# AiRyunn/BoT

Hardware: AMD Instinct MI355X
Metric: edges/sec full-batch GAT fwd+bwd on ogbn-arxiv; achieved HBM GB/s vs peak (higher is better)
Workload: dtype f32

## Files before the change

### bot_amd/_C.py

```python
from __future__ import annotations

import ctypes
import os
from ctypes import c_char_p, c_double, c_float, c_int32, c_int64, c_uint64, c_void_p

import torch

_HERE = os.path.dirname(os.path.abspath(__file__))
LIB_PATH = os.environ.get("BOT_AMD_LIB") or os.path.join(_HERE, "lib", "libbot_gnn.so")
ABI_VERSION = 19

if not os.path.exists(LIB_PATH):
    raise ImportError(
        f"{LIB_PATH} is missing: build the gfx950 kernels first "
        "(`make -C bot_amd/csrc` or `python -c 'import __graft_entry__ as g; g.build()'`). "
        "bot_amd has no CPU / PyTorch fallback."
    )
_lib = ctypes.CDLL(LIB_PATH)

_P = c_void_p
_SIGS = {
    "bot_abi_version": (ctypes.c_int, []),
    "bot_last_error": (c_char_p, []),
    "bot_last_kernel": (c_char_p, []),
    "bot_debug_abort_trace": (ctypes.c_int, [c_char_p]),
    "bot_row_plan_default_chunk": (c_int32, [c_int64]),
    "bot_row_plan_size_host": (ctypes.c_int, [_P, c_int64, c_int32, _P, _P, _P]),
    "bot_row_plan_fill_host": (ctypes.c_int, [_P, c_int64, c_int32, _P, _P, _P]),
    "bot_degrees_i64": (ctypes.c_int, [_P, c_int64, _P, _P]),
    "bot_spmm_workspace_floats": (c_int64, [c_int64, c_int32, c_int32]),
    "bot_spmm_set_layout": (ctypes.c_int, [c_int32]),
    "bot_spmm_set_zero_skip": (ctypes.c_int, [c_int32]),
    "bot_spmm_f32": (ctypes.c_int, [_P, _P, c_int64, c_int64, _P, c_int64, _P, _P, c_int64, _P, c_int64, c_int64, _P, _P,
                                    c_int32, c_int32, _P, c_int64, c_int64, _P, c_int64, c_int64, _P, _P]),
    "bot_spmm_blocked_f32": (ctypes.c_int, [_P, _P, _P, _P, _P, c_int32, c_int32, c_int32, c_int32, c_int32, c_int32, _P, c_int64, _P,
                                            c_int32, c_int32, _P, c_int64, _P, c_int64, _P]),
    "bot_spmm_dot_f32": (ctypes.c_int, [_P, _P, c_int64, c_int64, _P, c_int64, _P, _P, c_int64, _P, c_int64, c_int64, _P, _P,
                                        _P, c_int64, c_int64, c_int32, c_int32, _P, c_int64, c_int64, _P, _P, _P, _P]),
    "bot_spmm_bcast_f32": (ctypes.c_int, [_P, _P, c_int64, c_int64, _P, c_int64, _P, _P, c_int64, _P, c_int64, _P, _P, c_int32,
                                          c_int32, _P, c_int64, c_int64, _P, _P]),
    "bot_spmm_bcast_halves_f16": (ctypes.c_int, [_P, _P, c_int64, c_int64, _P, c_int64, _P, _P, c_int64, _P, c_int64, _P, _P, c_int32, c_int32, _P, _P,
                                                 c_int64, c_int64, c_int32, c_int32, _P, _P]),
    "bot_spmm_dot_bcast_f32": (ctypes.c_int, [_P, _P, c_int64, c_int64, _P, c_int64, _P, _P, c_int64, _P, c_int64, c_int64, _P,
                                              _P, _P, c_int64, c_int32, c_int32, _P, c_int64, _P, _P, _P]),
    "bot_sddmm_dot_f32": (ctypes.c_int, [_P, _P, c_int64, c_int64, _P, c_int64, _P, c_int64, c_int64, _P, c_int64, c_int64,
                                         c_int32, c_int32, _P, _P, c_int32, _P]),
    "bot_sddmm_dot_bcast_f32": (ctypes.c_int, [_P, _P, c_int64, c_int64, _P, c_int64, _P, c_int64, _P, c_int64, c_int64, c_int32,
                                               c_int32, _P, _P, _P]),
    "bot_sddmm_u_add_v_f32": (ctypes.c_int, [_P, _P, c_int64, _P, _P, c_int32, _P, _P]),
    "bot_gat_attn_fwd_f32": (ctypes.c_int, [_P, _P, c_int64, c_int64, _P, c_int64, c_int32, _P, _P, _P, _P, _P, c_float,
                                            c_int32, _P, _P, _P, c_float, c_uint64, _P, _P, _P]),
    "bot_gat_attn_bwd_f32": (ctypes.c_int, [_P, _P, c_int64, c_int64, _P, c_int64, c_int32, _P, _P, _P, _P, c_float, c_int32,
                                            _P, _P, _P, _P, _P, _P, _P, c_float, c_uint64, _P, _P]),
    "bot_gat_infer_workspace_floats": (c_int64, [c_int64, c_int32, c_int32]),
    "bot_gat_infer_f32": (ctypes.c_int, [_P, _P, c_int64, c_int64, _P, c_int64, _P, _P, c_int64, c_int64, _P, c_int64, c_int64,
                                         _P, c_int64, _P, c_int64, _P, _P, c_float, c_int32, c_int32, _P, c_int64, c_int64, _P, _P,
                                         c_int32, _P, c_int64, c_int64, _P, _P, _P]),
    "bot_segment_sum_f32": (ctypes.c_int, [_P, c_int64, c_int64, _P, c_int64, c_int32, _P, _P, c_int32, _P, _P]),
    "bot_gather_rows_f32": (ctypes.c_int, [_P, c_int64, _P, c_int64, c_int32, _P, c_int64, _P]),
    "bot_scatter_add_rows_f32": (ctypes.c_int, [_P, c_int64, _P, c_int64, c_int32, _P, c_int64, _P]),
    "bot_merge_weight_fwd_f32": (ctypes.c_int, [_P, _P, _P, _P, c_int32, c_int32, c_int32, c_int32, c_int32, c_int32, _P, _P]),
    "bot_merge_weight_bwd_f32": (ctypes.c_int, [_P, _P, _P, c_int32, c_int32, c_int32, c_int32, c_int32, c_int32, _P, _P, _P, _P, _P, _P]),
    "bot_edge_mlp_workspace_floats": (c_int64, []),
    "bot_edge_mlp_fwd_f32": (ctypes.c_int, [_P, c_int32, _P, _P, c_int32, _P, c_int32, c_int64, _P, _P]),
    "bot_edge_mlp_bwd_f32": (ctypes.c_int, [_P, c_int32, _P, _P, c_int32, _P, c_int32, _P, c_int64, _P, _P, _P, _P, _P]),
    "bot_random_keep_workspace_bytes": (c_int64, []),
    "bot_random_keep_u8": (ctypes.c_int, [c_int64, c_int64, c_uint64, _P, _P, _P]),
    "bot_halves_workspace_floats": (c_int64, []),
    "bot_halves_scale_f32": (ctypes.c_int, [_P, c_int64, c_int64, c_int32, _P, _P, _P]),
    "bot_halves_split_f16": (ctypes.c_int, [_P, c_int64, c_int64, c_int32, _P, c_int32, _P, c_int64, c_int32, _P]),
    "bot_halves_split_cols_f16": (ctypes.c_int, [_P, c_int64, c_int64, c_int32, _P, c_int32, _P, c_int64, c_int32, c_int32, _P]),
    "bot_halves_split_heads_f16": (ctypes.c_int, [_P, c_int64, c_int64, c_int32, c_int32, _P, _P, c_int64, c_int32, c_int32, _P]),
    "bot_gemm_halves_f32": (ctypes.c_int, [c_int32, c_int32, c_int64, c_int64, c_int64, _P, _P, c_int64, _P, c_int64, _P, c_int64,
                                           c_int32, c_int64, c_int64, c_int64, c_float, _P, c_int64, c_int32, c_int32, _P]),
    "bot_gemm_halves3_nt_f32": (ctypes.c_int, [c_int64, c_int64, c_int64, _P, _P, _P, c_int64, c_int64, _P, c_int64, c_int64, _P, c_int64,
                                               c_int32, _P]),
    "bot_gemm_halves3_tn_workspace_floats": (c_int64, [c_int64, c_int64, c_int64]),
    "bot_gemm_halves3_tn_f32": (ctypes.c_int, [c_int64, c_int64, c_int64, c_int64, c_int64, _P, _P, _P, c_int64, c_int64, _P, c_int64, c_int64, _P,
                                               c_int64, _P, c_int32, _P]),
    "bot_gemm_halves3_nt_grouped_f32": (ctypes.c_int, [c_int64, c_int64, _P, _P, _P, c_int64, c_int64, _P, c_int64, c_int64, _P, c_int64, c_int32, _P,
                                                       c_int32, _P, _P, c_int32, _P, c_int32, _P]),
    "bot_gemm_halves3_tn_grouped_workspace_floats": (c_int64, [c_int64, c_int32]),
    "bot_gemm_halves3_tn_grouped_f32": (ctypes.c_int, [c_int64, _P, _P, _P, c_int64, c_int64, _P, c_int64, c_int64, _P, c_int32, _P, _P, c_int32, _P]),
    "bot_tn_narrow_workspace_floats": (c_int64, [c_int64, c_int32, c_int32]),
    "bot_tn_narrow_f32": (ctypes.c_int, [_P, c_int64, _P, c_int64, c_int64, c_int32, c_int32, _P, c_int64, c_int32, _P, _P]),
    "bot_bn_act_bwd_reduce_max_f32": (ctypes.c_int, [_P, c_int64, _P, c_int64, c_int64, c_int32, _P, _P, _P, _P, c_int32, c_float, c_uint64, _P, _P, _P, _P, _P]),
    "bot_bn_bwd_bound_f32": (ctypes.c_int, [c_int32, c_int64, _P, _P, _P, c_double, _P, _P, _P, _P]),
    "bot_bn_act_bwd_apply_halves_f32": (ctypes.c_int, [_P, c_int64, _P, c_int64, c_int64, c_int32, _P, _P, _P, _P, c_int32, c_float, c_uint64, _P, _P, _P, c_double,
                                                       _P, c_int64, _P, _P, c_int64, c_int32, c_int32, c_int32, _P]),
    "bot_label_split_f32": (ctypes.c_int, [_P, c_int64, _P, c_int64, _P, c_float, c_uint64, _P, c_int32, _P, _P, _P, _P, _P]),
    "bot_build_input_f32": (ctypes.c_int, [_P, c_int64, c_int64, c_int32, c_int32, _P, c_float, c_uint64, _P, _P, c_int64, _P]),
    "bot_build_input_reuse_f32": (ctypes.c_int, [_P, c_int64, c_int64, c_int32, c_int32, _P, _P, _P, c_int64, c_float, c_uint64, _P, _P, c_int64, _P]),
    "bot_node_loss_f32": (ctypes.c_int, [_P, c_int64, c_int64, c_int32, _P, c_int64, _P, _P, c_int32, c_float, _P, c_int64, _P, c_int64, _P]),
    "bot_rmsprop_step_f32": (ctypes.c_int, [c_int32, _P, _P, _P, _P, c_float, _P, c_float, c_float, c_float, _P]),
    "bot_gemm_halves_last_algo": (ctypes.c_int, [_P, _P]),
    "bot_gemm_halves_library_version": (ctypes.c_int, [_P, _P]),
    "bot_tn_gemm_workspace_floats": (c_int64, [c_int64, c_int32, c_int32, c_int32]),
    "bot_tn_gemm_f32": (ctypes.c_int, [_P, c_int64, _P, c_int64, c_int64, c_int32, c_int32, _P, c_int64, c_int32, c_int32, c_int64, c_int64,
                                       c_int64, _P, _P]),
    "bot_skinny_gemm_f32": (ctypes.c_int, [_P, c_int64, _P, c_int64, c_int32, _P, c_int64, c_int64, c_int32, c_int32, c_int32, c_int32,
                                           c_int64, c_int64, c_int64, _P]),
    "bot_bn_workspace_floats": (c_int64, [c_int32]),
    "bot_colstats_f32": (ctypes.c_int, [_P, c_int64, c_int64, c_int32, _P, _P, _P, _P]),
    "bot_colsum_f32": (ctypes.c_int, [_P, c_int64, c_int64, c_int32, _P, _P, _P]),
    "bot_bn_stats_f32": (ctypes.c_int, [_P, c_int64, c_int64, c_int32, c_float, c_float, _P, _P, _P, _P, _P, _P, _P]),
    "bot_bn_stats_halves_f32": (ctypes.c_int, [_P, c_int64, c_int64, c_int32, c_float, c_float, _P, _P, _P, _P, _P, _P, _P, c_float, _P, _P, _P]),
    "bot_bn_act_fwd_halves_f32": (ctypes.c_int, [_P, c_int64, c_int64, c_int32, _P, _P, _P, _P, c_int32, c_float, c_uint64, _P, _P, c_int64,
                                                 _P, _P, c_int64, c_int32, c_int32, _P]),
    "bot_bn_act_fwd_f32": (ctypes.c_int, [_P, c_int64, c_int64, c_int32, _P, _P, _P, _P, c_int32, c_float, c_uint64, _P, _P, c_int64, _P]),
    "bot_bn_act_bwd_reduce_f32": (ctypes.c_int, [_P, c_int64, _P, c_int64, c_int64, c_int32, _P, _P, _P, _P, c_int32, c_float,
                                                 c_uint64, _P, _P, _P, _P, _P]),
    "bot_bn_act_bwd_apply_f32": (ctypes.c_int, [_P, c_int64, _P, c_int64, c_int64, c_int32, _P, _P, _P, _P, c_int32, c_float,
                                                c_uint64, _P, _P, _P, c_double, _P, c_int64, _P, _P]),
    "bot_halves_tn_combine_f32": (ctypes.c_int, [_P, _P, c_int32, c_int32, c_int32, c_int32, _P, _P, _P, c_int64, _P]),
    "bot_halves_scale_from_slots2_f32": (ctypes.c_int, [_P, c_float, _P, c_float, _P, _P]),
    "bot_halves_tail_f16": (ctypes.c_int, [c_int64, c_int32, _P, _P, _P, _P, _P, c_int64, c_int32, _P]),
    "bot_spmm_dot_halves_fits": (ctypes.c_int, [_P, c_int64, c_int64, _P, c_int64, c_int64, c_int32, c_int32, _P, c_int64, c_int64, c_int32]),
    "bot_spmm_dot_halves_f16": (ctypes.c_int, [_P, _P, c_int64, c_int64, _P, c_int64, _P, _P, c_int64, _P, c_int64, c_int64, _P, _P, _P, c_int64, c_int64,
                                               c_int32, c_int32, _P, _P, c_int64, c_int64, c_int32, _P, _P, _P]),
    "bot_gemm_halves3_nt_bn_rows": (c_int32, [c_int64]),
    "bot_gemm_halves3_nt3_f32": (ctypes.c_int, [c_int64, c_int64, c_int64, _P, _P, c_int64, _P, _P, c_int64, c_int64, _P, c_int64, c_int64, c_int32, _P, c_int64,
                                                _P, c_int32, _P]),
    "bot_gemm_halves3_nt_bn_deferred_max_k": (c_int32, []),
    "bot_gemm_halves3_nt_bn_reduce_f32": (ctypes.c_int, [c_int64, c_int64, c_int64, _P, _P, c_int64, _P, _P, c_int64, c_int64, _P, c_int64, c_int64, c_int32, _P, c_int64,
                                                         _P, _P]),
    "bot_gemm_halves3_nt_bn_apply_f32": (ctypes.c_int, [c_int64, c_int64, c_int64, _P, _P, c_int64, _P, _P, c_int64, c_int64, _P, c_int64, c_int64, c_int32, _P,
                                                        _P, _P, c_double, _P, c_int64, _P, _P, c_int64, c_int32, c_int32, c_int32, _P, _P]),
    "bot_bn_act_bwd_reduce_partials_f32": (ctypes.c_int, [_P, c_int32, c_int32, _P, _P, _P]),
    "bot_bn_bwd_bound_partials_f32": (ctypes.c_int, [c_int32, _P, c_int32, _P, _P, c_double, _P, _P, _P, _P]),
    "bot_bn_bwd_partials_finish_f32": (ctypes.c_int, [_P, _P, c_int32, c_int32, _P, _P, c_int32, c_double, _P, _P, _P, _P]),
    "bot_gemm_halves3_nt2_f32": (ctypes.c_int, [c_int64, c_int64, c_int64, _P, _P, c_int64, _P, _P, c_int64, c_int64, _P, c_int64, c_int64, c_int32, _P, c_int64,
                                                c_int32, _P]),
    "bot_halves_split_frag_f16": (ctypes.c_int, [_P, c_int64, c_int64, c_int32, _P, _P, c_int32, _P]),
    "bot_gemm_halves3_tn2_f32": (ctypes.c_int, [c_int64, c_int64, c_int64, c_int64, c_int64, _P, _P, _P, c_int64, _P, c_int64, c_int64, _P, c_int64, c_int64, _P,
                                                c_int64, _P, c_int32, _P]),
    "bot_stream_create": (ctypes.c_int, [c_int32, _P]),
    "bot_gemm_halves3_nt_grouped2_f32": (ctypes.c_int, [c_int64, c_int64, _P, _P, _P, c_int64, c_int64, _P, c_int64, c_int64, _P, c_int64, c_int32, _P,
                                                        c_int32, _P, _P, c_int32, _P, _P, _P, _P, c_int32, c_int32, _P]),
    "bot_bn_stats_halves_partials_f32": (ctypes.c_int, [_P, _P, c_int32, _P, c_int64, c_int32, c_float, c_float, _P, _P, _P, _P, _P, _P, _P, c_float, _P, _P, _P]),
    "bot_absmax_slots": (c_int32, []),
    "bot_absmax_slots_f32": (ctypes.c_int, [_P, c_int64, c_int64, c_int32, _P, _P]),
    "bot_halves_scale_from_slots_f32": (ctypes.c_int, [_P, _P, _P]),
    "bot_sample_neighbors_count_i32": (ctypes.c_int, [_P, c_int64, _P, c_int64, c_int32, _P, _P]),
    "bot_sample_neighbors_i32": (ctypes.c_int, [_P, c_int64, _P, c_int64, c_int32, c_uint64, _P, _P, _P]),
# ... 303 lines not shown

def spmm_dot(d, x, w, wperm, y, out=None, dot=None, absmax=None):
    _dev(x, w, y, d.indptr)
    x, ldx, hsx = _slab(x, "x")
    y, ldy, hsy = _slab(y, "y")
    H, D = x.shape[1], x.shape[2]
    w = _f32(w, "w").contiguous()
    if out is None:
        out = torch.empty((d.n_rows, H, D), dtype=torch.float32, device=x.device)
    out_, ldo, hso = _slab(out, "out")
    assert out_ is out
    if dot is None:
        dot = torch.empty((d.nnz, H), dtype=torch.float32, device=x.device)
    elif dot.dtype != torch.float32 or not dot.is_contiguous() or dot.dim() != 2 or dot.shape[1] != H:
        raise BotKernelError(f"spmm_dot: dot must be a contiguous float32 [E,{H}] array")
    partial = None
    if d.n_long:
        partial = torch.empty(int(_lib.bot_spmm_workspace_floats(d.n_slots, H, D)), dtype=torch.float32, device=x.device)
    _check(_timed("spmm_dot", (H, D), lambda: _lib.bot_spmm_dot_f32(
        d.indptr.data_ptr(), d.indices.data_ptr(), d.n_rows, d.nnz, d.items.data_ptr(), d.n_items, _ptr(d.long_rows),
        _ptr(d.long_ptr), d.n_long, x.data_ptr(), ldx, hsx, w.data_ptr(), _ptr(_i32(wperm, "wperm")), y.data_ptr(), ldy, hsy,
        H, D, out.data_ptr(), ldo, hso, dot.data_ptr(), _ptr(partial), _ptr(absmax), _stream())), "spmm_dot")
    return out, dot


def spmm_dot_halves_fits(x, y, hout, hsh, h2_off) -> bool:
    x, ldx, hsx = _slab(x, "x")
    y, ldy, hsy = _slab(y, "y")
    return bool(_lib.bot_spmm_dot_halves_fits(x.data_ptr(), ldx, hsx, y.data_ptr(), ldy, hsy, x.shape[1], x.shape[2], hout.data_ptr(), hout.stride(0),
                                              int(hsh), int(h2_off)))


def spmm_dot_halves(d, x, w, wperm, y, hscale, hout, hsh, h2_off, dot=None):
    _dev(x, w, y, d.indptr, hout, hscale)
    x, ldx, hsx = _slab(x, "x")
    y, ldy, hsy = _slab(y, "y")
    H, D = x.shape[1], x.shape[2]
    w = _f32(w, "w").contiguous()
    assert hout.dtype == torch.float16 and hout.stride(1) == 1 and hout.shape[0] == d.n_rows
    if dot is None:
        dot = torch.empty((d.nnz, H), dtype=torch.float32, device=x.device)
    elif dot.dtype != torch.float32 or not dot.is_contiguous() or dot.dim() != 2 or dot.shape[1] != H:
        raise BotKernelError(f"spmm_dot_halves: dot must be a contiguous float32 [E,{H}] array")
    partial = None
    if d.n_long:
        partial = torch.empty(int(_lib.bot_spmm_workspace_floats(d.n_slots, H, D)), dtype=torch.float32, device=x.device)
    _check(_timed("spmm_dot", (H, D), lambda: _lib.bot_spmm_dot_halves_f16(
        d.indptr.data_ptr(), d.indices.data_ptr(), d.n_rows, d.nnz, d.items.data_ptr(), d.n_items, _ptr(d.long_rows),
        _ptr(d.long_ptr), d.n_long, x.data_ptr(), ldx, hsx, w.data_ptr(), _ptr(_i32(wperm, "wperm")), y.data_ptr(), ldy, hsy,
        H, D, hscale.data_ptr(), hout.data_ptr(), hout.stride(0), int(hsh), int(h2_off), dot.data_ptr(), _ptr(partial), _stream())), "spmm_dot_halves")
    return dot


def spmm_bcast(d, x, w, wperm=None, head_outer=True):
    _dev(x, w, d.indptr)
    _f32(x, "x")
    if x.stride(1) != 1:
        x = x.contiguous()
    w = _f32(w, "w").contiguous()
    H, D = w.shape[1], x.shape[1]
    if head_outer:
        out = torch.empty((H, d.n_rows, D), dtype=torch.float32, device=x.device)
        ldo, hso = D, d.n_rows * D
    else:
        out = torch.empty((d.n_rows, H, D), dtype=torch.float32, device=x.device)
        ldo, hso = H * D, D
    partial = None
    if d.n_long:
        partial = torch.empty(int(_lib.bot_spmm_workspace_floats(d.n_slots, H, D)), dtype=torch.float32, device=x.device)
    _check(_timed("spmm_bcast", (H, D), lambda: _lib.bot_spmm_bcast_f32(
        d.indptr.data_ptr(), d.indices.data_ptr(), d.n_rows, d.nnz, d.items.data_ptr(), d.n_items, _ptr(d.long_rows),
        _ptr(d.long_ptr), d.n_long, x.data_ptr(), x.stride(0), w.data_ptr(), _ptr(_i32(wperm, "wperm")), H, D, out.data_ptr(),
        ldo, hso, _ptr(partial), _stream())), "spmm_bcast")
    return out


def spmm_bcast_halves(d, x, w, wperm, hscale, hout, col0, hsh, h2_off, hpiece):
    _dev(x, w, d.indptr, hout, hscale)
    _f32(x, "x")
    if x.stride(1) != 1:
        x = x.contiguous()
    w = _f32(w, "w").contiguous()
    H, D = w.shape[1], x.shape[1]
    assert hout.dtype == torch.float16 and hout.dim() == 2 and hout.shape[0] == d.n_rows and hout.stride(1) == 1 and col0 % 4 == 0
    assert col0 + h2_off + (H - 1) * hsh + hpiece <= hout.shape[1]
    partial = None
    if d.n_long:
        partial = torch.empty(int(_lib.bot_spmm_workspace_floats(d.n_slots, H, D)), dtype=torch.float32, device=x.device)
    _check(_timed("spmm_bcast", (H, D), lambda: _lib.bot_spmm_bcast_halves_f16(
        d.indptr.data_ptr(), d.indices.data_ptr(), d.n_rows, d.nnz, d.items.data_ptr(), d.n_items, _ptr(d.long_rows),
        _ptr(d.long_ptr), d.n_long, x.data_ptr(), x.stride(0), w.data_ptr(), _ptr(_i32(wperm, "wperm")), H, D, hscale.data_ptr(),
        hout.data_ptr() + 2 * col0, hout.stride(0), hsh, h2_off, hpiece, _ptr(partial), _stream())), "spmm_bcast_halves")
    return hout


def spmm_dot_bcast(d, x, w, wperm, y, out=None):
    _dev(x, w, y, d.indptr)
    _f32(x, "x"), _f32(y, "y")
    assert x.dim() == 3 and x.is_contiguous()
    if y.stride(1) != 1:
        y = y.contiguous()
    H, n, D = x.shape
    w = _f32(w, "w").contiguous()
    if out is None:
        out = torch.empty((d.n_rows, D), dtype=torch.float32, device=x.device)
    assert out.stride(1) == 1 and out.shape == (d.n_rows, D)
    dot = torch.empty((d.nnz, H), dtype=torch.float32, device=x.device)
    partial = None
    if d.n_long:
        partial = torch.empty(int(_lib.bot_spmm_workspace_floats(d.n_slots, 1, D)), dtype=torch.float32, device=x.device)
    _check(_timed("spmm_dot_bcast", (H, D), lambda: _lib.bot_spmm_dot_bcast_f32(
        d.indptr.data_ptr(), d.indices.data_ptr(), d.n_rows, d.nnz, d.items.data_ptr(), d.n_items, _ptr(d.long_rows),
        _ptr(d.long_ptr), d.n_long, x.data_ptr(), D, n * D, w.data_ptr(), _ptr(_i32(wperm, "wperm")), y.data_ptr(), y.stride(0),
        H, D, out.data_ptr(), out.stride(0), dot.data_ptr(), _ptr(partial), _stream())), "spmm_dot_bcast")
    return out, dot


def sddmm_dot(d, x, y, operm=None, out=None):
    _dev(x, y, d.indptr)
    x, ldx, hsx = _slab(x, "x")
    y, ldy, hsy = _slab(y, "y")
    H, D = x.shape[1], x.shape[2]
    if out is None:
        out = torch.empty((d.nnz, H), dtype=torch.float32, device=x.device)
    _check(_timed("sddmm_dot", (H, D), lambda: _lib.bot_sddmm_dot_f32(
        d.indptr.data_ptr(), d.indices.data_ptr(), d.n_rows, d.nnz, d.items.data_ptr(), d.n_items, x.data_ptr(), ldx, hsx,
        y.data_ptr(), ldy, hsy, H, D, out.data_ptr(), _ptr(_i32(operm, "operm")), 0, _stream())), "sddmm_dot")
    return out


def sddmm_dot_bcast(d, x, y, operm=None):
    _dev(x, y, d.indptr)
    _f32(x, "x"), _f32(y, "y")
    if x.stride(1) != 1:
        x = x.contiguous()
    assert y.dim() == 3 and y.is_contiguous()
    H, n, D = y.shape
    out = torch.empty((d.nnz, H), dtype=torch.float32, device=x.device)
    _check(_timed("sddmm_dot_bcast", (H, D), lambda: _lib.bot_sddmm_dot_bcast_f32(
        d.indptr.data_ptr(), d.indices.data_ptr(), d.n_rows, d.nnz, d.items.data_ptr(), d.n_items, x.data_ptr(), x.stride(0),
        y.data_ptr(), D, n * D, H, D, out.data_ptr(), _ptr(_i32(operm, "operm")), _stream())), "sddmm_dot_bcast")
    return out


def u_add_v(src, dst, x, y=None):
    _dev(x, y, src)
    x = _f32(x, "x").contiguous()
    y = None if y is None else _f32(y, "y").contiguous()
    E, W = src.numel(), x.shape[1]
    out = torch.empty((E, W), dtype=torch.float32, device=x.device)
    _check(_lib.bot_sddmm_u_add_v_f32(_i32(src, "src").data_ptr(), _ptr(_i32(dst, "dst")), E, x.data_ptr(), _ptr(y), W,
                                      out.data_ptr(), _stream()), "u_add_v")
    return out


def zsign_buffer(d, H, slope):
    if os.environ.get("BOT_NO_ZSIGN"):
        return None
    return torch.empty(d.nnz, dtype=torch.uint8, device=d.indptr.device) if (H <= 8 and slope != 1.0 and d.indptr.is_cuda) else None


def gat_attn_fwd(d, el, er, ee, eperm, keep, slope, H, aperm, zsign=None, drop=None):
    _dev(el, er, ee, d.indptr)
    el = None if el is None else _f32(el, "el").contiguous()
    er = None if er is None else _f32(er, "er").contiguous()
    ee = None if ee is None else _f32(ee, "ee").contiguous()
    if keep is not None and (keep.dtype != torch.uint8 or not keep.is_contiguous()):
        raise BotKernelError("keep must be contiguous uint8")
    a = torch.empty((d.nnz, H), dtype=torch.float32, device=d.indptr.device)
    p, seed = drop if drop is not None else (0.0, 0)
    a_drop = torch.empty_like(a) if p > 0 else None
    _check(_lib.bot_gat_attn_fwd_f32(d.indptr.data_ptr(), d.indices.data_ptr(), d.n_rows, d.nnz, _ptr(d.long_rows), d.n_long,
                                     d.chunk, _ptr(el), _ptr(er), _ptr(ee), _ptr(_i32(eperm, "eperm")), _ptr(keep),
                                     float(slope), H, a.data_ptr(), _ptr(_i32(aperm, "aperm")), _ptr(zsign), float(p),
                                     int(seed) & 0xFFFFFFFFFFFFFFFF, _seed_off(p), _ptr(a_drop), _stream()), "gat_attn_fwd")
    return a if drop is None else (a, a_drop if a_drop is not None else a)


def gat_attn_bwd(d, el, er, ee, eperm, slope, H, a, da, aperm, zperm, want_der, zsign=None, drop=None):
    _dev(a, da, d.indptr)
    el = None if el is None else _f32(el, "el").contiguous()
    er = None if er is None else _f32(er, "er").contiguous()
    ee = None if ee is None else _f32(ee, "ee").contiguous()
    a = _f32(a, "a").contiguous()
    da = _f32(da, "da").contiguous()
    dz = torch.empty((d.nnz, H), dtype=torch.float32, device=a.device)
    der = torch.empty((d.n_rows, H), dtype=torch.float32, device=a.device) if want_der else None
    _check(_lib.bot_gat_attn_bwd_f32(d.indptr.data_ptr(), d.indices.data_ptr(), d.n_rows, d.nnz, _ptr(d.long_rows), d.n_long,
                                     d.chunk, _ptr(el), _ptr(er), _ptr(ee), _ptr(_i32(eperm, "eperm")), float(slope), H,
                                     a.data_ptr(), da.data_ptr(), _ptr(_i32(aperm, "aperm")), dz.data_ptr(),
                                     _ptr(_i32(zperm, "zperm")), _ptr(der), _ptr(zsign), float(drop[0]) if drop else 0.0,
                                     (int(drop[1]) & 0xFFFFFFFFFFFFFFFF) if drop else 0, _seed_off(drop[0]) if drop else None,
                                     _stream()), "gat_attn_bwd")
    return dz, der
# ... 466 lines not shown
    n = x.shape[0]
    out = torch.empty((k, p), dtype=torch.float32, device=x.device)
    ws = torch.empty(int(_lib.bot_gemm_halves3_tn_workspace_floats(n, piece_x, piece_d)), dtype=torch.float32, device=x.device)
    _check(_timed("gemm_halves", (k, p, 3 * n, 1), lambda: _lib.bot_gemm_halves3_tn2_f32(
        n, k, p, piece_x, piece_d, scale_x.data_ptr(), scale_d.data_ptr(), _ptr(scale_d2), int(p_split), x.data_ptr(), _ld(x),
        2 * piece_x if x2_off is None else x2_off, d.data_ptr(), _ld(d), 2 * piece_d if d2_off is None else d2_off,
        out.data_ptr(), _ld(out), ws.data_ptr(), int(mode), _stream())), "gemm_halves3_tn")
    return out


def _idx64(t, name):
    if t.dtype != torch.int64 or not t.is_contiguous() or t.dim() != 1:
        raise BotKernelError(f"{name} must be a contiguous 1-D int64 tensor (got {t.dtype}, stride {tuple(t.stride())})")


def _labels64(labels):
    if labels.dtype != torch.int64:
        raise BotKernelError(f"labels must be int64 (got {labels.dtype})")
    lab = labels.reshape(labels.shape[0], -1)
    if lab.shape[1] > 1 and lab.stride(1) != 1:
        lab = lab.contiguous()
    return lab


def label_split(train_idx, labels, mask, mask_rate, seed, use_labels, code, wn):
    _dev(train_idx, labels, wn)
    _idx64(train_idx, "train_idx")
    count = torch.empty(1, dtype=torch.float32, device=wn.device)
    ws = torch.empty(128, dtype=torch.int32, device=wn.device)
    lab = _labels64(labels)
    if wn.dtype != torch.float32 or not wn.is_contiguous() or (code is not None and (code.dtype != torch.int32 or not code.is_contiguous())):
        raise BotKernelError("label_split: wn must be contiguous float32, code contiguous int32")
    m = None
    if mask is not None:
        _dev(mask)
        m = mask.to(torch.bool).contiguous().view(torch.uint8)
        if m.numel() != train_idx.numel():
            raise BotKernelError("label_split: mask must have one entry per training node")
    _check(_lib.bot_label_split_f32(train_idx.data_ptr(), train_idx.numel(), lab.data_ptr(), lab.stride(0), _ptr(m), float(mask_rate), int(seed),
                                    _seed_off(1.0), int(bool(use_labels)), _ptr(code), wn.data_ptr(), count.data_ptr(), ws.data_ptr(), _stream()), "label_split")
    return count


def build_input(feat, code, n_classes, p, seed):
    _dev(feat)
    _f32(feat, "feat")
    n, F = feat.shape
    out = torch.empty((n, F + n_classes), dtype=torch.float32, device=feat.device)
    _check(_lib.bot_build_input_f32(feat.data_ptr(), _ld(feat), n, F, n_classes, _ptr(code), float(p), int(seed), _seed_off(p), out.data_ptr(), _ld(out),
                                    _stream()), "build_input")
    return out


REUSE_CALLS = 0


def build_input_reuse(feat, code, reuse, pred, n_classes, p, seed, out=None):
    global REUSE_CALLS
    _dev(feat, code, reuse, pred, out)
    _f32(feat, "feat"), _f32(pred, "pred"), _f32(out, "out")
    n, F = feat.shape
    if feat.stride(1) != 1 and F > 1:
        feat = feat.contiguous()
    if pred.dim() != 2 or pred.shape[0] != n or pred.shape[1] < n_classes or (pred.stride(1) != 1 and pred.shape[1] > 1):
        raise BotKernelError(f"build_input_reuse: pred must be [{n}, >= {n_classes}] with unit column stride, got {tuple(pred.shape)}")
    if code is None or code.dtype != torch.int32 or not code.is_contiguous() or code.numel() != n:
        raise BotKernelError(f"build_input_reuse: code must be contiguous int32 [{n}]")
    if reuse is not None and (reuse.dtype != torch.uint8 or not reuse.is_contiguous() or reuse.numel() != n):
        raise BotKernelError(f"build_input_reuse: reuse must be contiguous uint8 [{n}]")
    if out is None:
        out = torch.empty((n, F + n_classes), dtype=torch.float32, device=feat.device)
    elif out.shape != (n, F + n_classes) or out.stride(1) != 1:
        raise BotKernelError(f"build_input_reuse: out must be [{n}, {F + n_classes}] with unit column stride")
    _check(_lib.bot_build_input_reuse_f32(feat.data_ptr(), _ld(feat), n, F, n_classes, code.data_ptr(), _ptr(reuse), pred.data_ptr(), _ld(pred), float(p),
                                          int(seed), _seed_off(p), out.data_ptr(), _ld(out), _stream()), "build_input_reuse")
    REUSE_CALLS += 1
    torch.autograd.graph.increment_version(out)
    return out


LOSS_KINDS = {"logit": 0, "loge": 1, "savage": 2}


def node_loss(x, labels, wn, count, kind, eps, want_grad=True):
    _dev(x, labels, wn, count)
    _f32(x, "x")
    n, C = x.shape
    n_pad = (n + 63) // 64 * 64
    y = torch.empty(n_pad, dtype=torch.float32, device=x.device)
    dx = torch.empty((n, C), dtype=torch.float32, device=x.device) if want_grad else None
    lab = _labels64(labels)
    if wn.dtype != torch.float32 or not wn.is_contiguous() or count.dtype != torch.float32:
        raise BotKernelError("node_loss: wn / count must be contiguous float32")
    _check(_lib.bot_node_loss_f32(x.data_ptr(), _ld(x), n, C, lab.data_ptr(), lab.stride(0), wn.data_ptr(), count.data_ptr(), LOSS_KINDS[kind], float(eps),
                                  y.data_ptr(), n_pad, _ptr(dx), C, _stream()), "node_loss")
    return y, dx


def node_loss_weighted(x, labels, wn, lw, wsum, kind, eps, want_grad=True):
    _dev(x, labels, wn, lw, wsum)
    _f32(x, "x")
    n, C = x.shape
    n_pad = (n + 63) // 64 * 64
    y = torch.empty(n_pad, dtype=torch.float32, device=x.device)
    dx = torch.empty((n, C), dtype=torch.float32, device=x.device) if want_grad else None
    lab = _labels64(labels)
# ... 922 lines not shown
```

### bot_amd/csrc/common.h

```cpp
#pragma once
#include <hip/hip_runtime.h>
#include <stdint.h>
#include <stdio.h>

#include "../../include/bot_gnn.h"

namespace bot {

void set_error(const char* fmt, ...);
void set_kernel(const char* fmt, ...);
void launch_halves_scale(const float* part, int n, float* scale, hipStream_t st);

inline int hip_status(const char* what) {
    hipError_t e = hipGetLastError();
    if (e != hipSuccess) {
        set_error("%s: %s", what, hipGetErrorString(e));
        return (int)e;
    }
    return 0;
}

#define BOT_REQUIRE(cond, code, ...)    \
    do {                                \
        if (!(cond)) {                  \
            bot::set_error(__VA_ARGS__); \
            return (code);              \
        }                               \
    } while (0)

inline bool aligned(const void* p, size_t a) { return (reinterpret_cast<uintptr_t>(p) % a) == 0; }

inline unsigned launch_grid(int64_t n, int64_t per_block, int64_t cap = 4096) {
    int64_t b = (n + per_block - 1) / per_block;
    return (unsigned)(b < 1 ? 1 : (b > cap ? cap : b));
}

constexpr int kBlock = 256;
constexpr int kWave = 64;

template <int VEC> struct Vec;
template <> struct Vec<1> { using type = float; };
template <> struct Vec<2> { using type = float2; };
template <> struct Vec<4> { using type = float4; };

template <int VEC>
__device__ __forceinline__ void vload(float (&r)[VEC], const float* p) {
    using T = typename Vec<VEC>::type;
    T v = *reinterpret_cast<const T*>(p);
    if constexpr (VEC == 1) { r[0] = v; }
    if constexpr (VEC == 2) { r[0] = v.x; r[1] = v.y; }
    if constexpr (VEC == 4) { r[0] = v.x; r[1] = v.y; r[2] = v.z; r[3] = v.w; }
}

template <int VEC>
__device__ __forceinline__ void vstore_nt(float* p, const float (&r)[VEC]) {
    typedef float nv __attribute__((ext_vector_type(VEC)));
    nv v;
#pragma unroll
    for (int t = 0; t < VEC; ++t) v[t] = r[t];
    __builtin_nontemporal_store(v, reinterpret_cast<nv*>(p));
}

template <int VEC>
__device__ __forceinline__ void vstore(float* p, const float (&r)[VEC]) {
    using T = typename Vec<VEC>::type;
    T v;
    if constexpr (VEC == 1) { v = r[0]; }
    if constexpr (VEC == 2) { v.x = r[0]; v.y = r[1]; }
    if constexpr (VEC == 4) { v.x = r[0]; v.y = r[1]; v.z = r[2]; v.w = r[3]; }
    *reinterpret_cast<T*>(p) = v;
}

template <int LANES>
__device__ __forceinline__ int group_bcast(int v, int j) {
    if constexpr (LANES == 64) return __builtin_amdgcn_readlane(v, j);
    else return __shfl(v, j, LANES);
}
template <int LANES>
__device__ __forceinline__ float group_bcast(float v, int j) {
    return __int_as_float(group_bcast<LANES>(__float_as_int(v), j));
}

template <int LANES>
// ... 114 lines not shown
```

### bot_amd/csrc/halves.hip

```cpp
#include <hip/hip_fp16.h>

#include "common.h"

namespace bot {

constexpr int kMaxBlocks = 1024;

__global__ __launch_bounds__(kBlock) void absmax_partial_kernel(const float* x, int64_t ldx, int64_t n, int32_t F, float* part) {
    __shared__ float lds[kBlock / kWave];
    float m = 0.f;
    const int64_t total = n * (int64_t)F;
    if (ldx == F && (reinterpret_cast<uintptr_t>(x) & 15) == 0) {
        const int64_t nq = total >> 2;
        const float4* x4 = reinterpret_cast<const float4*>(x);
        const int64_t stride = (int64_t)gridDim.x * kBlock;
        int64_t i = (int64_t)blockIdx.x * kBlock + threadIdx.x;
        for (; i + 3 * stride < nq; i += 4 * stride) {
            const float4 a = x4[i], b = x4[i + stride], c = x4[i + 2 * stride], d = x4[i + 3 * stride];
            m = fmaxf(m, fmaxf(fmaxf(fmaxf(fabsf(a.x), fabsf(a.y)), fmaxf(fabsf(a.z), fabsf(a.w))),
                               fmaxf(fmaxf(fabsf(b.x), fabsf(b.y)), fmaxf(fabsf(b.z), fabsf(b.w)))));
            m = fmaxf(m, fmaxf(fmaxf(fmaxf(fabsf(c.x), fabsf(c.y)), fmaxf(fabsf(c.z), fabsf(c.w))),
                               fmaxf(fmaxf(fabsf(d.x), fabsf(d.y)), fmaxf(fabsf(d.z), fabsf(d.w)))));
        }
        for (; i < nq; i += stride) {
            const float4 a = x4[i];
            m = fmaxf(m, fmaxf(fmaxf(fabsf(a.x), fabsf(a.y)), fmaxf(fabsf(a.z), fabsf(a.w))));
        }
        for (int64_t j = (nq << 2) + (int64_t)blockIdx.x * kBlock + threadIdx.x; j < total; j += stride) m = fmaxf(m, fabsf(x[j]));
    } else if (ldx == F) {
        for (int64_t i = (int64_t)blockIdx.x * kBlock + threadIdx.x; i < total; i += (int64_t)gridDim.x * kBlock) m = fmaxf(m, fabsf(x[i]));
    } else {
        for (int64_t i = (int64_t)blockIdx.x * kBlock + threadIdx.x; i < total; i += (int64_t)gridDim.x * kBlock) {
            const int64_t r = i / F;
            m = fmaxf(m, fabsf(x[r * ldx + (i - r * F)]));
        }
    }
#pragma unroll
    for (int o = 32; o > 0; o >>= 1) m = fmaxf(m, __shfl_xor(m, o));
    if ((threadIdx.x & 63) == 0) lds[threadIdx.x >> 6] = m;
    __syncthreads();
    if (threadIdx.x == 0) {
        for (int w = 1; w < kBlock / kWave; ++w) m = fmaxf(m, lds[w]);
        part[blockIdx.x] = m;
    }
}

__global__ __launch_bounds__(kWave) void halves_scale_kernel(const float* part, int nblk, float* scale) {
    float m = 0.f;
    for (int i = threadIdx.x; i < nblk; i += kWave) m = fmaxf(m, part[i]);
#pragma unroll
    for (int o = 32; o > 0; o >>= 1) m = fmaxf(m, __shfl_xor(m, o));
    if (threadIdx.x == 0) {
        float s = 1.f;
        if (m > 0.f && m < INFINITY) {
            int e;
            const float f = frexpf(m, &e);
            if (f == 0.5f) e -= 1;
            s = ldexpf(1.f, min(60, 14 - e));
        }
        scale[0] = s;
        scale[1] = 1.f / s;
    }
}

template <int ORDER>
__global__ __launch_bounds__(128) void halves_split_kernel(const float* x, int64_t ldx, int32_t F, const float* scale, __half* out,
                                                           int64_t ldo, int32_t piece, bool wide, int32_t width) {
    const int64_t r = blockIdx.x;
    const int c = (blockIdx.y * 128 + threadIdx.x) * 2;
    if (c >= width) return;
    const float s = scale ? scale[0] : 1.f;
    float v0 = 0.f, v1 = 0.f;
    const float* xr = x + r * ldx;
    if (c + 1 < F) {
        if (wide) {
            const float2 v = *reinterpret_cast<const float2*>(xr + c);
            v0 = v.x * s, v1 = v.y * s;
        } else {
            v0 = xr[c] * s, v1 = xr[c + 1] * s;
        }
    } else if (c < F) {
        v0 = xr[c] * s;
    }
// ... 304 lines not shown
```

### bot_amd/csrc/sddmm.hip

```cpp
#include "common.h"

namespace bot {

struct DotArgs {
    const int32_t* indices;
    const int4* items;
    int64_t n_items;
    const float* x;
    int64_t ldx, hsx;
    const float* y;
    int64_t ldy, hsy;
    int32_t H, D;
    float* out;
    const int32_t* operm;
    int32_t accumulate;
};

template <int LANES, int U>
__device__ __forceinline__ float transpose_reduce(float (&p)[U], int lane) {
    static_assert(U == 4 || U == 8, "U");
    if constexpr (U == 8) {
        const bool hi = lane & 4;
        float q[4];
#pragma unroll
        for (int i = 0; i < 4; ++i) {
            const float keep = hi ? p[i + 4] : p[i];
            const float send = hi ? p[i] : p[i + 4];
            q[i] = keep + __shfl_xor(send, 4, LANES);
        }
        const bool h2 = lane & 2;
        float r[2];
#pragma unroll
        for (int i = 0; i < 2; ++i) {
            const float keep = h2 ? q[i + 2] : q[i];
            const float send = h2 ? q[i] : q[i + 2];
            r[i] = keep + __shfl_xor(send, 2, LANES);
        }
        const bool h1 = lane & 1;
        float s = (h1 ? r[1] : r[0]) + __shfl_xor(h1 ? r[0] : r[1], 1, LANES);
#pragma unroll
        for (int m = 8; m < LANES; m <<= 1) s += __shfl_xor(s, m, LANES);
        return s;
    } else {
        const bool h2 = lane & 2;
        float r[2];
#pragma unroll
        for (int i = 0; i < 2; ++i) {
            const float keep = h2 ? p[i + 2] : p[i];
            const float send = h2 ? p[i] : p[i + 2];
            r[i] = keep + __shfl_xor(send, 2, LANES);
        }
        const bool h1 = lane & 1;
        float s = (h1 ? r[1] : r[0]) + __shfl_xor(h1 ? r[0] : r[1], 1, LANES);
#pragma unroll
        for (int m = 4; m < LANES; m <<= 1) s += __shfl_xor(s, m, LANES);
        return s;
    }
}

template <int VEC, int LANES, int NCHUNK>
__global__ __launch_bounds__(kBlock) void sddmm_dot_kernel(DotArgs a) {
    constexpr int U = 8;
    const int lane = threadIdx.x % LANES;
    const int64_t gid = ((int64_t)blockIdx.x * kBlock + threadIdx.x) / LANES;
    if (gid >= a.n_items * a.H) return;
    int head = (int)(gid / a.n_items);
    const int64_t item = gid - (int64_t)head * a.n_items;
    const int4 it = a.items[item];
// ... 24 lines not shown
    for (int k0 = beg; k0 < end; k0 += LANES) {
        const int k = k0 + lane;
        const int idx = k < end ? a.indices[k] : 0;
        const int cnt = min(LANES, end - k0);
        for (int i = 0; i < cnt; i += U) {
            float p[U];
            float v[U][NCHUNK][VEC];
#pragma unroll
            for (int u = 0; u < U; ++u) {
                const int s = group_bcast<LANES>(idx, min(i + u, cnt - 1));
                const float* px = xb + (int64_t)s * a.ldx;
#pragma unroll
                for (int c = 0; c < NCHUNK; ++c) vload<VEC>(v[u][c], px + off[c]);
            }
#pragma unroll
            for (int u = 0; u < U; ++u) {
                float s = 0.f;
#pragma unroll
                for (int c = 0; c < NCHUNK; ++c)
#pragma unroll
                    for (int t = 0; t < VEC; ++t) s = fmaf(v[u][c][t], yv[c][t], s);
                p[u] = s;
            }
            const float tot = transpose_reduce<LANES, U>(p, lane);
            if (lane < U && i + lane < cnt) {
                const int pos = k0 + i + lane;
                const int64_t o = (int64_t)(a.operm ? a.operm[pos] : pos) * a.H + head;
                a.out[o] = a.accumulate ? a.out[o] + tot : tot;
            }
        }
    }
}

template <int VEC, int LANES, int NCHUNK>
static void launch_dot(const DotArgs& a, hipStream_t st) {
    const int64_t groups = a.n_items * a.H;
    const int64_t blocks = (groups * LANES + kBlock - 1) / kBlock;
    if (blocks == 0) return;
    hipLaunchKernelGGL((sddmm_dot_kernel<VEC, LANES, NCHUNK>), dim3((unsigned)blocks), dim3(kBlock), 0, st, a);
}

template <int VEC>
static void dispatch_dot(const DotArgs& a, hipStream_t st) {
    const int L = (a.D + VEC - 1) / VEC;
    if (L <= 8) launch_dot<VEC, 8, 1>(a, st);
    else if (L <= 16) launch_dot<VEC, 16, 1>(a, st);
    else if (L <= 32) launch_dot<VEC, 32, 1>(a, st);
    else if (L <= 64) launch_dot<VEC, 64, 1>(a, st);
    else if (L <= 128) launch_dot<VEC, 64, 2>(a, st);
    else if (L <= 192) launch_dot<VEC, 64, 3>(a, st);
    else launch_dot<VEC, 64, 4>(a, st);
}

template <int VEC, int LANES, int NCHUNK, int HB>
__global__ __launch_bounds__(kBlock) void sddmm_dot_bcast_kernel(DotArgs a) {
    static_assert(LANES >= 16 && HB <= 4, "butterfly layout");
    constexpr int U = 4;
    const int lane = threadIdx.x % LANES;
    const int64_t item = ((int64_t)blockIdx.x * kBlock + threadIdx.x) / LANES;
    if (item >= a.n_items) return;
    const int4 it = a.items[item];
    int row = it.x, beg = it.y, end = it.z;
    if constexpr (LANES == 64) {
        row = __builtin_amdgcn_readfirstlane(row);
        beg = __builtin_amdgcn_readfirstlane(beg);
        end = __builtin_amdgcn_readfirstlane(end);
    }
    int off[NCHUNK];
    float yv[HB][NCHUNK][VEC];
#pragma unroll
    for (int c = 0; c < NCHUNK; ++c) {
        const int e = (c * LANES + lane) * VEC;
        const bool act = e < a.D;
        off[c] = act ? e : 0;
#pragma unroll
        for (int h = 0; h < HB; ++h) {
            vload<VEC>(yv[h][c], a.y + (int64_t)row * a.ldy + (int64_t)h * a.hsy + off[c]);
            if (!act) {
#pragma unroll
                for (int t = 0; t < VEC; ++t) yv[h][c][t] = 0.f;
            }
        }
    }
    for (int k0 = beg; k0 < end; k0 += LANES) {
        const int k = k0 + lane;
        const int idx = k < end ? a.indices[k] : 0;
        const int cnt = min(LANES, end - k0);
        for (int i = 0; i < cnt; i += U) {
            float p[16], v[U][NCHUNK][VEC];
#pragma unroll
            for (int q = 0; q < 16; ++q) p[q] = 0.f;
#pragma unroll
            for (int u = 0; u < U; ++u) {
                const int s = group_bcast<LANES>(idx, min(i + u, cnt - 1));
                const float* px = a.x + (int64_t)s * a.ldx;
#pragma unroll
                for (int c = 0; c < NCHUNK; ++c) vload<VEC>(v[u][c], px + off[c]);
            }
#pragma unroll
            for (int u = 0; u < U; ++u)
#pragma unroll
                for (int h = 0; h < HB; ++h) {
                    float d = 0.f;
#pragma unroll
                    for (int c = 0; c < NCHUNK; ++c)
#pragma unroll
                        for (int t = 0; t < VEC; ++t) d = fmaf(v[u][c][t], yv[h][c][t], d);
                    p[u * 4 + h] = d;
                }
            const float tot = transpose_reduce16<LANES>(p, lane);
            const int slot16 = lane & 15, u = slot16 >> 2, h = slot16 & 3;
            if (lane < 16 && h < HB && i + u < cnt) {
                const int pos = k0 + i + u;
                a.out[(int64_t)(a.operm ? a.operm[pos] : pos) * HB + h] = tot;
            }
        }
    }
}

template <int VEC, int HB>
static void dispatch_dot_bcast(const DotArgs& a, hipStream_t st) {
    const int L = (a.D + VEC - 1) / VEC;
#define BOT_DOTB(LN, NC)                                                                                                    \
    do {                                                                                                                    \
        const int64_t blocks = (a.n_items * LN + kBlock - 1) / kBlock;                                                      \
        if (blocks == 0) break;                                                                                             \
        set_kernel("bot::sddmm_dot_bcast_kernel<%d,%d,%d,%d>", VEC, LN, NC, HB);                                           \
        hipLaunchKernelGGL((sddmm_dot_bcast_kernel<VEC, LN, NC, HB>), dim3((unsigned)blocks), dim3(kBlock), 0, st, a);      \
    } while (0)
    if (L <= 16) BOT_DOTB(16, 1);
    else if (L <= 32) BOT_DOTB(32, 1);
    else if (L <= 64) BOT_DOTB(64, 1);
    else if (L <= 128) BOT_DOTB(64, 2);
    else BOT_DOTB(64, 4);
#undef BOT_DOTB
}

__global__ __launch_bounds__(kBlock) void u_add_v_kernel(const int32_t* src, const int32_t* dst, int64_t n_edges,
                                                        const float* x, const float* y, int32_t W, float* out) {
    const int64_t total = n_edges * W;
    for (int64_t g = (int64_t)blockIdx.x * kBlock + threadIdx.x; g < total; g += (int64_t)gridDim.x * kBlock) {
        const int64_t e = g / W;
        const int j = (int)(g - e * W);
        float v = x[(int64_t)src[e] * W + j];
        if (y) v += y[(int64_t)dst[e] * W + j];
        out[g] = v;
    }
}

}

extern "C" {

int bot_sddmm_dot_f32(const int32_t* indptr, const int32_t* indices, int64_t n_rows, int64_t nnz, const int32_t* items,
                      int64_t n_items, const float* x, int64_t ldx, int64_t hsx, const float* y, int64_t ldy, int64_t hsy,
                      int32_t H, int32_t D, float* out, const int32_t* operm, int32_t accumulate, bot_stream_t stream) {
    using namespace bot;
    (void)indptr;
    BOT_REQUIRE(n_rows >= 0 && nnz >= 0 && n_items >= 0, BOT_E_RANGE, "sddmm_dot: negative size");
    BOT_REQUIRE(nnz < INT32_MAX && n_rows < INT32_MAX, BOT_E_RANGE, "sddmm_dot: int32 index range exceeded");
    BOT_REQUIRE(H >= 1 && D >= 1, BOT_E_RANGE, "sddmm_dot: H=%d D=%d must be >= 1", H, D);
    if (nnz == 0 || n_rows == 0) return 0;
    BOT_REQUIRE(indices && items && x && y && out, BOT_E_NULL, "sddmm_dot: NULL pointer");
    BOT_REQUIRE(hsx >= D && hsy >= D && ldx >= (int64_t)(H - 1) * hsx + D && ldy >= (int64_t)(H - 1) * hsy + D, BOT_E_RANGE,
                "sddmm_dot: strides smaller than the slab");
    hipStream_t st = (hipStream_t)stream;
    const int vec = pick_vec(D, {ldx, hsx, ldy, hsy}, {x, y});
    const int cap = vec * 256;
    for (int d0 = 0; d0 < D; d0 += cap) {
        DotArgs a{indices, reinterpret_cast<const int4*>(items), n_items, x + d0, ldx, hsx, y + d0, ldy, hsy, H,
                  (int32_t)(D - d0 < cap ? D - d0 : cap), out, operm, (d0 > 0 || accumulate) ? 1 : 0};
        if (vec == 4) dispatch_dot<4>(a, st);
        else if (vec == 2) dispatch_dot<2>(a, st);
        else dispatch_dot<1>(a, st);
    }
    return hip_status("sddmm_dot launch");
}

int bot_sddmm_dot_bcast_f32(const int32_t* indptr, const int32_t* indices, int64_t n_rows, int64_t nnz, const int32_t* items,
                            int64_t n_items, const float* x, int64_t ldx, const float* y, int64_t ldy, int64_t hsy, int32_t H,
                            int32_t D, float* out, const int32_t* operm, bot_stream_t stream) {
    using namespace bot;
    (void)indptr;
    BOT_REQUIRE(n_rows >= 0 && nnz >= 0 && n_items >= 0 && nnz < INT32_MAX && n_rows < INT32_MAX, BOT_E_RANGE, "sddmm_dot_bcast: bad size");
    BOT_REQUIRE(H >= 1 && H <= 4 && D >= 1 && D <= 1024, BOT_E_RANGE, "sddmm_dot_bcast: H=%d (1..4) D=%d (1..1024)", H, D);
    if (nnz == 0 || n_rows == 0) return 0;
    BOT_REQUIRE(indices && items && x && y && out, BOT_E_NULL, "sddmm_dot_bcast: NULL pointer");
    BOT_REQUIRE(ldx >= D && ldy >= D && (hsy >= D || H == 1), BOT_E_RANGE, "sddmm_dot_bcast: strides smaller than the slab");
    hipStream_t st = (hipStream_t)stream;
    const int vec = pick_vec(D, {ldx, ldy, H > 1 ? hsy : 0}, {x, y});
    BOT_REQUIRE(D <= vec * 256, BOT_E_RANGE, "sddmm_dot_bcast: D=%d exceeds one launch tile", D);
    DotArgs a{indices, reinterpret_cast<const int4*>(items), n_items, x, ldx, 0, y, ldy, hsy, H, D, out, operm, 0};
#define BOT_DOTB_H(V)                                       \
    switch (H) {                                            \
        case 1: dispatch_dot_bcast<V, 1>(a, st); break;     \
        case 2: dispatch_dot_bcast<V, 2>(a, st); break;     \
        case 3: dispatch_dot_bcast<V, 3>(a, st); break;     \
        default: dispatch_dot_bcast<V, 4>(a, st); break;    \
    }
    if (vec == 4) { BOT_DOTB_H(4) } else if (vec == 2) { BOT_DOTB_H(2) } else { BOT_DOTB_H(1) }
#undef BOT_DOTB_H
    return hip_status("sddmm_dot_bcast launch");
}

int bot_sddmm_u_add_v_f32(const int32_t* src, const int32_t* dst, int64_t n_edges, const float* x, const float* y,
                          int32_t W, float* out, bot_stream_t stream) {
    using namespace bot;
    BOT_REQUIRE(n_edges >= 0 && W >= 1, BOT_E_RANGE, "u_add_v: n_edges=%lld W=%d", (long long)n_edges, W);
    if (n_edges == 0) return 0;
    BOT_REQUIRE(src && x && out && (y == nullptr || dst), BOT_E_NULL, "u_add_v: NULL pointer");
    const int64_t total = n_edges * W;
    int64_t blocks = (total + kBlock - 1) / kBlock;
    if (blocks > 256 * 8) blocks = 256 * 8;
    hipLaunchKernelGGL(u_add_v_kernel, dim3((unsigned)blocks), dim3(kBlock), 0, (hipStream_t)stream, src, dst, n_edges, x, y,
                       W, out);
    return hip_status("u_add_v launch");
}

}
```

### bot_amd/csrc/spmm.hip

```cpp
#include <hip/hip_fp16.h>

#include "sweep.h"

#include <stdlib.h>
#include <algorithm>
#include <atomic>
#include <string.h>

namespace bot {

struct SpmmArgs {
    const int32_t* indices;
    const int4* items;
    int64_t n_items;
    const float* x;
    int64_t ldx, hsx;
    const float* w;
    const int32_t* wperm;
    int32_t H, D, n_tiles;
    float* out;
    int64_t ldo, hso;
    float* partial;
    int64_t ldp;
    const float* y;
    int64_t ldy, hsy;
    float* dot_out;
    const float* addend;
    int64_t lda, hsa;
    uint32_t* absmax;
    __half* hout;
    int64_t ldh, hsh;
    int32_t h2_off, hpiece;
    const float* hscale;
    int32_t skip;
};

__device__ __forceinline__ bool is_zero_weight(float w) { return (__float_as_uint(w) << 1) == 0u; }
__device__ __forceinline__ bool wants_row(float w, uint32_t force) { return ((__float_as_uint(w) << 1) | force) != 0u; }
__device__ __forceinline__ void settle(float& v) { asm volatile("" : "+v"(v)); }
__device__ __forceinline__ void settle(int& v) { asm volatile("" : "+v"(v)); }

template <int VEC>
__device__ __forceinline__ void store_halves(__half* p, int32_t h2_off, const float (&v)[VEC], float s) {
    __half a[VEC], b[VEC];
#pragma unroll
    for (int t = 0; t < VEC; ++t) {
        const float z = v[t] * s;
        a[t] = __float2half_rn(z);
        b[t] = __float2half_rn((z - __half2float(a[t])) * 2048.0f);
    }
    if constexpr (VEC == 4) {
        *reinterpret_cast<uint2*>(p) = *reinterpret_cast<const uint2*>(a);
        *reinterpret_cast<uint2*>(p + h2_off) = *reinterpret_cast<const uint2*>(b);
    } else if constexpr (VEC == 2) {
        *reinterpret_cast<uint32_t*>(p) = *reinterpret_cast<const uint32_t*>(a);
        *reinterpret_cast<uint32_t*>(p + h2_off) = *reinterpret_cast<const uint32_t*>(b);
    } else {
        p[0] = a[0], p[h2_off] = b[0];
    }
}

template <int VEC, int LANES, int NCHUNK>
__global__ __launch_bounds__(kBlock) void spmm_dot_kernel(SpmmArgs a) {
    constexpr int U = 4;
    const int lane = threadIdx.x % LANES;
    const int64_t gid = ((int64_t)blockIdx.x * kBlock + threadIdx.x) / LANES;
    if (gid >= a.n_items * a.H) return;
    int head = (int)(gid / a.n_items);
    const int64_t item = gid - (int64_t)head * a.n_items;
    const int4 it = a.items[item];
    int row = it.x, beg = it.y, end = it.z, slot = it.w;
    if constexpr (LANES == 64) {
        row = __builtin_amdgcn_readfirstlane(row);
        beg = __builtin_amdgcn_readfirstlane(beg);
        end = __builtin_amdgcn_readfirstlane(end);
        slot = __builtin_amdgcn_readfirstlane(slot);
        head = __builtin_amdgcn_readfirstlane(head);
    }
    const float* xb = a.x + (int64_t)head * a.hsx;
    const float* yb = a.y + (int64_t)row * a.ldy + (int64_t)head * a.hsy;
    int off[NCHUNK];
    bool act[NCHUNK];
    float acc[NCHUNK][VEC], yv[NCHUNK][VEC];
#pragma unroll
    for (int c = 0; c < NCHUNK; ++c) {
        const int e = (c * LANES + lane) * VEC;
        act[c] = e < a.D;
        off[c] = act[c] ? e : 0;
        vload<VEC>(yv[c], yb + off[c]);
// ... 543 lines not shown
#pragma unroll
        for (int h = 0; h < HB; ++h) wv[h] = 0.f;
        if (k < end) {
            idx = a.indices[k];
            const int wp = a.wperm ? a.wperm[k] : k;
#pragma unroll
            for (int h = 0; h < HB; ++h) wv[h] = a.w[(int64_t)wp * HB + h];
        }
        const int cnt = min(LANES, end - k0);
        for (int i = 0; i < cnt; i += U) {
            float v[U][NCHUNK][VEC], ww[U][HB];
#pragma unroll
            for (int u = 0; u < U; ++u) {
                const int j = min(i + u, cnt - 1);
                const int s = group_bcast<LANES>(idx, j);
#pragma unroll
                for (int h = 0; h < HB; ++h) ww[u][h] = i + u < cnt ? group_bcast<LANES>(wv[h], j) : 0.f;
                const float* px = a.x + (int64_t)s * a.ldx;
#pragma unroll
                for (int c = 0; c < NCHUNK; ++c) vload<VEC>(v[u][c], px + off[c]);
            }
#pragma unroll
            for (int u = 0; u < U; ++u)
#pragma unroll
                for (int h = 0; h < HB; ++h)
#pragma unroll
                    for (int c = 0; c < NCHUNK; ++c)
#pragma unroll
                        for (int t = 0; t < VEC; ++t) acc[h][c][t] = fmaf(ww[u][h], v[u][c][t], acc[h][c][t]);
        }
    }
    if (a.hout && slot < 0) {
        const float s = a.hscale[0];
#pragma unroll
        for (int h = 0; h < HB; ++h) {
            __half* ob = a.hout + (int64_t)row * a.ldh + (int64_t)h * a.hsh;
#pragma unroll
            for (int c = 0; c < NCHUNK; ++c) {
                const int e = (c * LANES + lane) * VEC;
                if (e < a.hpiece) store_halves<VEC>(ob + e, a.h2_off, acc[h][c], act[c] ? s : 0.f);
            }
        }
        return;
    }
#pragma unroll
    for (int h = 0; h < HB; ++h) {
        float* ob = slot < 0 ? a.out + (int64_t)row * a.ldo + (int64_t)h * a.hso : a.partial + (int64_t)slot * a.ldp + (int64_t)h * a.D;
#pragma unroll
        for (int c = 0; c < NCHUNK; ++c)
            if (act[c]) vstore<VEC>(ob + off[c], acc[h][c]);
    }
}

__global__ __launch_bounds__(kBlock) void spmm_combine_halves_kernel(const int32_t* long_rows, const int32_t* long_ptr, int64_t n_long, int32_t H,
                                                                    int32_t D, const float* partial, int64_t ldp, __half* hout, int64_t ldh,
                                                                    int64_t hsh, int32_t h2_off, int32_t hpiece, const float* hscale) {
    const int64_t gid = (int64_t)blockIdx.x * kBlock + threadIdx.x;
    const int64_t hp = (int64_t)H * hpiece;
    if (gid >= n_long * hp) return;
    const int64_t i = gid / hp;
    const int e2 = (int)(gid - i * hp);
    const int h = e2 / hpiece, d = e2 - h * hpiece;
    float v[1] = {0.f};
    if (d < D) {
        const int e = h * D + d;
        for (int p = long_ptr[i]; p < long_ptr[i + 1]; ++p) v[0] += partial[(int64_t)p * ldp + e];
    }
    store_halves<1>(hout + (int64_t)long_rows[i] * ldh + (int64_t)h * hsh + d, h2_off, v, hscale[0]);
}

template <int VEC, int LANES, int NCHUNK, int HB>
__global__ __launch_bounds__(kBlock) void spmm_dot_bcast_kernel(SpmmArgs a) {
    static_assert(LANES >= 16 && HB <= 4, "butterfly layout");
    constexpr int U = 4;
    const int lane = threadIdx.x % LANES;
    const int64_t item = ((int64_t)blockIdx.x * kBlock + threadIdx.x) / LANES;
    if (item >= a.n_items) return;
    const int4 it = a.items[item];
    int row = it.x, beg = it.y, end = it.z, slot = it.w;
    if constexpr (LANES == 64) {
        row = __builtin_amdgcn_readfirstlane(row);
        beg = __builtin_amdgcn_readfirstlane(beg);
        end = __builtin_amdgcn_readfirstlane(end);
        slot = __builtin_amdgcn_readfirstlane(slot);
    }
    const float* yb = a.y + (int64_t)row * a.ldy;
    int off[NCHUNK];
    bool act[NCHUNK];
    float acc[NCHUNK][VEC], yv[NCHUNK][VEC];
#pragma unroll
    for (int c = 0; c < NCHUNK; ++c) {
        const int e = (c * LANES + lane) * VEC;
        act[c] = e < a.D;
        off[c] = act[c] ? e : 0;
        vload<VEC>(yv[c], yb + off[c]);
#pragma unroll
        for (int t = 0; t < VEC; ++t) {
            acc[c][t] = 0.f;
            if (!act[c]) yv[c][t] = 0.f;
        }
    }
    for (int k0 = beg; k0 < end; k0 += LANES) {
        const int k = k0 + lane;
        int idx = 0, wp = 0;
        float wv[HB];
#pragma unroll
        for (int h = 0; h < HB; ++h) wv[h] = 0.f;
        if (k < end) {
            idx = a.indices[k];
            wp = a.wperm ? a.wperm[k] : k;
#pragma unroll
            for (int h = 0; h < HB; ++h) wv[h] = a.w[(int64_t)wp * HB + h];
        }
        const int cnt = min(LANES, end - k0);
        for (int i = 0; i < cnt; i += U) {
            float p[16];
#pragma unroll
            for (int q = 0; q < 16; ++q) p[q] = 0.f;
#pragma unroll
            for (int u = 0; u < U; ++u) {
                const int j = min(i + u, cnt - 1);
                const int s = group_bcast<LANES>(idx, j);
                const float* px = a.x + (int64_t)s * a.ldx;
                float v[HB][NCHUNK][VEC];
#pragma unroll
                for (int h = 0; h < HB; ++h)
#pragma unroll
                    for (int c = 0; c < NCHUNK; ++c) vload<VEC>(v[h][c], px + (int64_t)h * a.hsx + off[c]);
#pragma unroll
                for (int h = 0; h < HB; ++h) {
                    const float ww = i + u < cnt ? group_bcast<LANES>(wv[h], j) : 0.f;
                    float d = 0.f;
#pragma unroll
                    for (int c = 0; c < NCHUNK; ++c)
#pragma unroll
                        for (int t = 0; t < VEC; ++t) {
                            acc[c][t] = fmaf(ww, v[h][c][t], acc[c][t]);
                            d = fmaf(v[h][c][t], yv[c][t], d);
                        }
                    p[u * 4 + h] = d;
                }
            }
            const float tot = transpose_reduce16<LANES>(p, lane);
            const int slot16 = lane & 15, u = slot16 >> 2, h = slot16 & 3;
            const int mywp = __shfl(wp, min(i + u, LANES - 1), LANES);
            if (lane < 16 && h < HB && i + u < cnt) a.dot_out[(int64_t)mywp * HB + h] = tot;
        }
    }
    float* ob = slot < 0 ? a.out + (int64_t)row * a.ldo : a.partial + (int64_t)slot * a.ldp;
#pragma unroll
    for (int c = 0; c < NCHUNK; ++c)
        if (act[c]) vstore<VEC>(ob + off[c], acc[c]);
}

template <int VEC, int HB, bool DOT>
static void dispatch_bcast(SpmmArgs& a, hipStream_t st) {
    const int L = (std::max(a.D, a.hout ? a.hpiece : 0) + VEC - 1) / VEC;
#define BOT_BCAST(LN, NC)                                                                                                     \
    do {                                                                                                                      \
        const int64_t blocks = (a.n_items * LN + kBlock - 1) / kBlock;                                                        \
        if (blocks == 0) break;                                                                                               \
        set_kernel(DOT ? "bot::spmm_dot_bcast_kernel<%d,%d,%d,%d>" : "bot::spmm_bcast_kernel<%d,%d,%d,%d>", VEC, LN, NC, HB);        \
        if constexpr (DOT) hipLaunchKernelGGL((spmm_dot_bcast_kernel<VEC, LN, NC, HB>), dim3((unsigned)blocks), dim3(kBlock), 0, st, a); \
        else hipLaunchKernelGGL((spmm_bcast_kernel<VEC, LN, NC, HB>), dim3((unsigned)blocks), dim3(kBlock), 0, st, a);        \
    } while (0)
    if (L <= 16) BOT_BCAST(16, 1);
    else if (L <= 32) BOT_BCAST(32, 1);
    else if (L <= 64) BOT_BCAST(64, 1);
    else if (L <= 128) BOT_BCAST(64, 2);
    else BOT_BCAST(64, 4);
#undef BOT_BCAST
}

template <bool DOT>
static int run_bcast(SpmmArgs& a, int vec, int H, hipStream_t st) {
#define BOT_BCAST_H(V)                                \
    switch (H) {                                      \
        case 1: dispatch_bcast<V, 1, DOT>(a, st); break; \
        case 2: dispatch_bcast<V, 2, DOT>(a, st); break; \
        case 3: dispatch_bcast<V, 3, DOT>(a, st); break; \
        default: dispatch_bcast<V, 4, DOT>(a, st); break; \
    }
    if (vec == 4) { BOT_BCAST_H(4) } else if (vec == 2) { BOT_BCAST_H(2) } else { BOT_BCAST_H(1) }
#undef BOT_BCAST_H
    return hip_status(DOT ? "spmm_dot_bcast launch" : "spmm_bcast launch");
}

template <int VEC, int LANES, int NCHUNK>
static void launch_spmm(const SpmmArgs& a, hipStream_t st) {
    const int64_t groups = a.n_items * a.H * a.n_tiles;
    const int64_t blocks = (groups * LANES + kBlock - 1) / kBlock;
    if (blocks == 0) return;
    set_kernel("bot::spmm_kernel<%d,%d,%d,%s>", VEC, LANES, NCHUNK, a.w ? "true" : "false");
    if (a.w) hipLaunchKernelGGL((spmm_kernel<VEC, LANES, NCHUNK, true>), dim3((unsigned)blocks), dim3(kBlock), 0, st, a);
    else hipLaunchKernelGGL((spmm_kernel<VEC, LANES, NCHUNK, false>), dim3((unsigned)blocks), dim3(kBlock), 0, st, a);
}

template <int VEC, int LANES, int NCHUNK>
static void launch_spmm_dot(const SpmmArgs& a, hipStream_t st) {
    const int64_t groups = a.n_items * a.H;
    const int64_t blocks = (groups * LANES + kBlock - 1) / kBlock;
    if (blocks == 0) return;
    set_kernel("bot::spmm_dot_kernel<%d,%d,%d>", VEC, LANES, NCHUNK);
    hipLaunchKernelGGL((spmm_dot_kernel<VEC, LANES, NCHUNK>), dim3((unsigned)blocks), dim3(kBlock), 0, st, a);
}

template <int VEC>
static void dispatch_spmm_dot(SpmmArgs& a, hipStream_t st) {
    const int L = (a.D + VEC - 1) / VEC;
    if (L <= 8) launch_spmm_dot<VEC, 8, 1>(a, st);
    else if (L <= 16) launch_spmm_dot<VEC, 16, 1>(a, st);
    else if (L <= 32) launch_spmm_dot<VEC, 32, 1>(a, st);
    else if (L <= 64) launch_spmm_dot<VEC, 64, 1>(a, st);
    else if (L <= 128) launch_spmm_dot<VEC, 64, 2>(a, st);
    else if (L <= 192) launch_spmm_dot<VEC, 64, 3>(a, st);
    else launch_spmm_dot<VEC, 64, 4>(a, st);
}

static bool spmm_dot_rows_wanted() {
    static const bool wanted = [] {
        const char* e = getenv("BOT_SPMM_DOT_LAYOUT");
        return !(e && !strcmp(e, "heads"));
    }();
    return wanted;
}

static bool spmm_rows_wanted() {
    static const bool wanted = [] {
        const char* e = getenv("BOT_SPMM_LAYOUT");
        return !(e && !strcmp(e, "heads"));
    }();
    return wanted;
}

// ... 173 lines not shown
    if (n_long > 0) {
        const int64_t n = n_long * H * D;
        hipLaunchKernelGGL(spmm_combine_kernel, dim3((unsigned)((n + kBlock - 1) / kBlock)), dim3(kBlock), 0, st, long_rows,
                           long_ptr, n_long, H, D, partial, (int64_t)H * D, out, ldo, hso, addend, lda, hsa);
        if (int rc = hip_status("spmm combine launch")) return rc;
    }
    return 0;
}

int bot_spmm_dot_f32(const int32_t* indptr, const int32_t* indices, int64_t n_rows, int64_t nnz, const int32_t* items,
                     int64_t n_items, const int32_t* long_rows, const int32_t* long_ptr, int64_t n_long, const float* x,
                     int64_t ldx, int64_t hsx, const float* w, const int32_t* wperm, const float* y, int64_t ldy, int64_t hsy,
                     int32_t H, int32_t D, float* out, int64_t ldo, int64_t hso, float* dot_out, float* partial,
                     uint32_t* absmax_slots, bot_stream_t stream) {
    using namespace bot;
    (void)indptr;
    BOT_REQUIRE(n_rows >= 0 && nnz >= 0 && n_items >= 0 && n_long >= 0, BOT_E_RANGE, "spmm_dot: negative size");
    BOT_REQUIRE(nnz < INT32_MAX && n_rows < INT32_MAX, BOT_E_RANGE, "spmm_dot: int32 index range exceeded");
    BOT_REQUIRE(H >= 1 && D >= 1, BOT_E_RANGE, "spmm_dot: H=%d D=%d must be >= 1", H, D);
    if (n_rows == 0) return 0;
    BOT_REQUIRE(items && x && out && y && (nnz == 0 || (indices && w && dot_out)), BOT_E_NULL, "spmm_dot: NULL pointer");
    BOT_REQUIRE(n_long == 0 || (long_rows && long_ptr && partial), BOT_E_NULL, "spmm_dot: long rows need long_rows/long_ptr/partial");
    BOT_REQUIRE(hsx >= D && hso >= D && hsy >= D && ldx >= (int64_t)(H - 1) * hsx + D && ldo >= (int64_t)(H - 1) * hso + D &&
                    ldy >= (int64_t)(H - 1) * hsy + D, BOT_E_RANGE, "spmm_dot: strides smaller than the slab");
    hipStream_t st = (hipStream_t)stream;
    SpmmArgs a{indices, reinterpret_cast<const int4*>(items), n_items, x, ldx, hsx, w, wperm, H, D, 1, out, ldo, hso, partial,
               (int64_t)H * D, y, ldy, hsy, dot_out, nullptr, 0, 0};
    const int vec = pick_vec(D, {ldx, hsx, ldo, hso, ldy, hsy}, {x, out, partial, y});
    BOT_REQUIRE(D <= vec * 256, BOT_E_RANGE, "spmm_dot: D=%d exceeds the %d floats one launch tile covers (use bot_spmm_f32 + bot_sddmm_dot_f32)",
                D, vec * 256);
    a.absmax = absmax_slots;
    a.skip = g_zero_skip.load(std::memory_order_relaxed);
    const bool rows = vec == 4 ? dispatch_spmm_dot_rows<4>(a, st) : (vec == 2 ? dispatch_spmm_dot_rows<2>(a, st) : dispatch_spmm_dot_rows<1>(a, st));
    if (!rows) {
        if (vec == 4) dispatch_spmm_dot<4>(a, st);
        else if (vec == 2) dispatch_spmm_dot<2>(a, st);
        else dispatch_spmm_dot<1>(a, st);
    }
    if (int rc = hip_status("spmm_dot launch")) return rc;
    if (n_long > 0) {
        const int64_t n = n_long * H * D;
        hipLaunchKernelGGL(spmm_combine_kernel, dim3((unsigned)((n + kBlock - 1) / kBlock)), dim3(kBlock), 0, st, long_rows,
                           long_ptr, n_long, H, D, partial, (int64_t)H * D, out, ldo, hso, (const float*)nullptr, (int64_t)0, (int64_t)0,
                           rows ? absmax_slots : (uint32_t*)nullptr);
        if (int rc = hip_status("spmm_dot combine launch")) return rc;
    }
    if (absmax_slots && !rows) {
        for (int h = 0; h < H; ++h) launch_absmax_slots(out + (int64_t)h * hso, ldo, n_rows, D, absmax_slots, st);
        if (int rc = hip_status("spmm_dot absmax launch")) return rc;
    }
    return 0;
}

int bot_spmm_bcast_f32(const int32_t* indptr, const int32_t* indices, int64_t n_rows, int64_t nnz, const int32_t* items,
                       int64_t n_items, const int32_t* long_rows, const int32_t* long_ptr, int64_t n_long, const float* x,
                       int64_t ldx, const float* w, const int32_t* wperm, int32_t H, int32_t D, float* out, int64_t ldo,
                       int64_t hso, float* partial, bot_stream_t stream) {
    using namespace bot;
    (void)indptr;
    BOT_REQUIRE(n_rows >= 0 && nnz >= 0 && n_items >= 0 && n_long >= 0 && nnz < INT32_MAX, BOT_E_RANGE, "spmm_bcast: bad size");
    BOT_REQUIRE(H >= 1 && H <= 4 && D >= 1 && D <= 1024, BOT_E_RANGE, "spmm_bcast: H=%d (1..4) D=%d (1..1024)", H, D);
    if (n_rows == 0) return 0;
    BOT_REQUIRE(items && x && out && (nnz == 0 || (indices && w)), BOT_E_NULL, "spmm_bcast: NULL pointer");
    BOT_REQUIRE(n_long == 0 || (long_rows && long_ptr && partial), BOT_E_NULL, "spmm_bcast: long rows need long_rows/long_ptr/partial");
    BOT_REQUIRE(ldx >= D && (hso >= D || H == 1) && ldo >= D, BOT_E_RANGE, "spmm_bcast: strides smaller than the slab");
    hipStream_t st = (hipStream_t)stream;
    SpmmArgs a{indices, reinterpret_cast<const int4*>(items), n_items, x, ldx, 0, w, wperm, H, D, 1, out, ldo, hso, partial,
               (int64_t)H * D, nullptr, 0, 0, nullptr, nullptr, 0, 0};
    const int vec = pick_vec(D, {ldx, ldo, hso}, {x, out, partial});
    BOT_REQUIRE(D <= vec * 256, BOT_E_RANGE, "spmm_bcast: D=%d exceeds one launch tile", D);
    if (int rc = run_bcast<false>(a, vec, H, st)) return rc;
    if (n_long > 0) {
        const int64_t n = n_long * H * D;
        hipLaunchKernelGGL(spmm_combine_kernel, dim3((unsigned)((n + kBlock - 1) / kBlock)), dim3(kBlock), 0, st, long_rows,
                           long_ptr, n_long, H, D, partial, (int64_t)H * D, out, ldo, hso, (const float*)nullptr, (int64_t)0, (int64_t)0);
        if (int rc = hip_status("spmm_bcast combine launch")) return rc;
    }
    return 0;
}

int bot_spmm_bcast_halves_f16(const int32_t* indptr, const int32_t* indices, int64_t n_rows, int64_t nnz, const int32_t* items, int64_t n_items,
                              const int32_t* long_rows, const int32_t* long_ptr, int64_t n_long, const float* x, int64_t ldx, const float* w,
                              const int32_t* wperm, int32_t H, int32_t D, const float* hscale, uint16_t* hout, int64_t ldh, int64_t hsh, int32_t h2_off,
                              int32_t hpiece, float* partial, bot_stream_t stream) {
    using namespace bot;
    (void)indptr;
    BOT_REQUIRE(n_rows >= 0 && nnz >= 0 && n_items >= 0 && n_long >= 0 && nnz < INT32_MAX, BOT_E_RANGE, "spmm_bcast_halves: bad size");
    BOT_REQUIRE(H >= 1 && H <= 4 && D >= 1 && D <= 1024, BOT_E_RANGE, "spmm_bcast_halves: H=%d (1..4) D=%d (1..1024)", H, D);
    if (n_rows == 0) return 0;
    BOT_REQUIRE(items && x && hout && hscale && (nnz == 0 || (indices && w)), BOT_E_NULL, "spmm_bcast_halves: NULL pointer");
    BOT_REQUIRE(n_long == 0 || (long_rows && long_ptr && partial), BOT_E_NULL, "spmm_bcast_halves: long rows need long_rows/long_ptr/partial");
    BOT_REQUIRE(ldx >= D && hpiece >= D && hpiece % 4 == 0 && (hsh >= hpiece || H == 1) && h2_off % 4 == 0 && hsh % 4 == 0 && ldh % 4 == 0 &&
                    h2_off >= (int64_t)(H - 1) * hsh + hpiece && ldh >= h2_off + (int64_t)(H - 1) * hsh + hpiece && aligned(hout, 8),
                BOT_E_RANGE, "spmm_bcast_halves: D=%d hpiece=%d hsh=%lld h2_off=%d ldh=%lld", D, hpiece, (long long)hsh, h2_off, (long long)ldh);
    hipStream_t st = (hipStream_t)stream;
    SpmmArgs a{indices, reinterpret_cast<const int4*>(items), n_items, x, ldx, 0, w, wperm, H, D, 1, nullptr, 0, 0, partial,
               (int64_t)H * D, nullptr, 0, 0, nullptr, nullptr, 0, 0};
    a.hout = reinterpret_cast<__half*>(hout), a.ldh = ldh, a.hsh = hsh, a.h2_off = h2_off, a.hpiece = hpiece, a.hscale = hscale;
    const int vec = pick_vec(D, {ldx}, {x, partial});
    BOT_REQUIRE(hpiece <= vec * 256, BOT_E_RANGE, "spmm_bcast_halves: hpiece=%d exceeds one launch tile", hpiece);
    a.D = D;
    if (int rc = run_bcast<false>(a, vec, H, st)) return rc;
    if (n_long > 0) {
        const int64_t n = n_long * H * hpiece;
        hipLaunchKernelGGL(spmm_combine_halves_kernel, dim3((unsigned)((n + kBlock - 1) / kBlock)), dim3(kBlock), 0, st, long_rows, long_ptr, n_long, H, D,
                           (const float*)partial, (int64_t)H * D, a.hout, ldh, hsh, h2_off, hpiece, hscale);
        if (int rc = hip_status("spmm_bcast_halves combine launch")) return rc;
    }
    return 0;
}

int bot_spmm_dot_halves_fits(const float* x, int64_t ldx, int64_t hsx, const float* y, int64_t ldy, int64_t hsy, int32_t H, int32_t D, const uint16_t* hout,
                             int64_t ldh, int64_t hsh, int32_t h2_off) {
    using namespace bot;
    if (H < 2 || D < 1 || !spmm_dot_rows_wanted()) return 0;
    const int vec = pick_vec(D, {ldx, hsx, ldy, hsy}, {x, y});
    if (!(hsh >= D && h2_off >= (int64_t)(H - 1) * hsh + D && ldh >= h2_off + (int64_t)(H - 1) * hsh + D && hsh % vec == 0 && h2_off % vec == 0 && ldh % vec == 0 &&
          aligned(hout, 2 * vec) && D <= vec * 256))
        return 0;
    const int L = (D + vec - 1) / vec;
    if (L <= 8) return 0;
    if (L > 64) return (L <= 128 && vec != 4 && H <= 3) ? 1 : 0;
    const int HL = L <= 16 ? 16 : (L <= 32 ? 32 : 64);
    return (H * HL + 63) / 64 <= 4 ? 1 : 0;
}

int bot_spmm_dot_halves_f16(const int32_t* indptr, const int32_t* indices, int64_t n_rows, int64_t nnz, const int32_t* items,
                            int64_t n_items, const int32_t* long_rows, const int32_t* long_ptr, int64_t n_long, const float* x,
                            int64_t ldx, int64_t hsx, const float* w, const int32_t* wperm, const float* y, int64_t ldy, int64_t hsy,
                            int32_t H, int32_t D, const float* hscale, uint16_t* hout, int64_t ldh, int64_t hsh, int32_t h2_off, float* dot_out,
                            float* partial, bot_stream_t stream) {
    using namespace bot;
    (void)indptr;
    BOT_REQUIRE(n_rows >= 0 && nnz >= 0 && n_items >= 0 && n_long >= 0 && nnz < INT32_MAX && n_rows < INT32_MAX, BOT_E_RANGE, "spmm_dot_halves: bad size");
    BOT_REQUIRE(H >= 2 && D >= 1, BOT_E_RANGE, "spmm_dot_halves: H=%d D=%d (the all-heads layout needs H >= 2)", H, D);
    if (n_rows == 0) return 0;
    BOT_REQUIRE(items && x && hout && hscale && y && (nnz == 0 || (indices && w && dot_out)), BOT_E_NULL, "spmm_dot_halves: NULL pointer");
    BOT_REQUIRE(n_long == 0 || (long_rows && long_ptr && partial), BOT_E_NULL, "spmm_dot_halves: long rows need long_rows/long_ptr/partial");
    BOT_REQUIRE(hsx >= D && hsy >= D && ldx >= (int64_t)(H - 1) * hsx + D && ldy >= (int64_t)(H - 1) * hsy + D, BOT_E_RANGE,
                "spmm_dot_halves: strides smaller than the slab");
    hipStream_t st = (hipStream_t)stream;
    SpmmArgs a{indices, reinterpret_cast<const int4*>(items), n_items, x, ldx, hsx, w, wperm, H, D, 1, nullptr, 0, 0, partial,
               (int64_t)H * D, y, ldy, hsy, dot_out, nullptr, 0, 0};
    const int vec = pick_vec(D, {ldx, hsx, ldy, hsy}, {x, partial, y});
    BOT_REQUIRE(hsh >= D && h2_off >= (int64_t)(H - 1) * hsh + D && ldh >= h2_off + (int64_t)(H - 1) * hsh + D && hsh % vec == 0 && h2_off % vec == 0 &&
                    ldh % vec == 0 && aligned(hout, 2 * vec), BOT_E_RANGE, "spmm_dot_halves: D=%d hsh=%lld h2_off=%d ldh=%lld vec=%d", D, (long long)hsh, h2_off,
                (long long)ldh, vec);
    BOT_REQUIRE(D <= vec * 256, BOT_E_RANGE, "spmm_dot_halves: D=%d exceeds one launch tile", D);
    a.hout = reinterpret_cast<__half*>(hout), a.ldh = ldh, a.hsh = hsh, a.h2_off = h2_off, a.hpiece = D, a.hscale = hscale;
    a.skip = g_zero_skip.load(std::memory_order_relaxed);
    const bool rows = vec == 4 ? dispatch_spmm_dot_rows<4>(a, st) : (vec == 2 ? dispatch_spmm_dot_rows<2>(a, st) : dispatch_spmm_dot_rows<1>(a, st));
    BOT_REQUIRE(rows, BOT_E_RANGE, "spmm_dot_halves: H=%d D=%d does not fit the all-heads layout", H, D);
    if (int rc = hip_status("spmm_dot_halves launch")) return rc;
    if (n_long > 0) {
        const int64_t n = n_long * H * D;
        hipLaunchKernelGGL(spmm_combine_halves_kernel, dim3((unsigned)((n + kBlock - 1) / kBlock)), dim3(kBlock), 0, st, long_rows, long_ptr, n_long, H, D,
                           (const float*)partial, (int64_t)H * D, a.hout, ldh, hsh, h2_off, D, hscale);
        if (int rc = hip_status("spmm_dot_halves combine launch")) return rc;
    }
    return 0;
}

// ... 30 lines not shown
```

### bot_amd/csrc/step.hip

```cpp
#include <algorithm>

#include "common.h"

namespace bot {
namespace {

__device__ __forceinline__ uint64_t eff_seed(uint64_t seed, const uint64_t* off) {
    return off ? seed + off[0] * 0x9E3779B97F4A7C15ull : seed;
}

__device__ __forceinline__ float uniform01(uint32_t w) { return (w >> 8) * (1.0f / 16777216.0f); }

constexpr int kSplitBlocks = 128;
__global__ __launch_bounds__(256) void label_split_kernel(const int64_t* train_idx, int64_t n_train, const int64_t* labels, int64_t ldl, const uint8_t* mask,
                                                          float mask_rate, uint64_t seed, const uint64_t* seed_offset, int use_labels, int32_t* code,
                                                          float* wn, int32_t* partial) {
    __shared__ int part[4];
    const uint64_t s = eff_seed(seed, seed_offset);
    int mine = 0;
    for (int64_t i = (int64_t)blockIdx.x * 256 + threadIdx.x; i < n_train; i += (int64_t)gridDim.x * 256) {
        bool keep;
        if (mask) {
            keep = mask[i] != 0;
        } else {
            uint32_t w[4];
            Philox::gen(s, (uint64_t)(i >> 2), w);
            keep = uniform01(w[i & 3]) < mask_rate;
        }
        const int64_t n = train_idx[i];
        const bool pred = use_labels ? !keep : keep;
        if (code) code[n] = (use_labels && keep) ? (int32_t)labels[n * ldl] : -1;
        wn[n] = pred ? 1.f : 0.f;
        mine += pred ? 1 : 0;
    }
#pragma unroll
    for (int o = 32; o > 0; o >>= 1) mine += __shfl_xor(mine, o);
    if ((threadIdx.x & 63) == 0) part[threadIdx.x >> 6] = mine;
    __syncthreads();
    if (threadIdx.x == 0) partial[blockIdx.x] = part[0] + part[1] + part[2] + part[3];
}

__global__ __launch_bounds__(64) void label_count_kernel(const int32_t* partial, int nb, float* count) {
    int t = 0;
    for (int i = threadIdx.x; i < nb; i += 64) t += partial[i];
#pragma unroll
    for (int o = 32; o > 0; o >>= 1) t += __shfl_xor(t, o);
    if (threadIdx.x == 0) count[0] = (float)t;
}

__global__ __launch_bounds__(256) void build_input_kernel(const float* feat, int64_t ldf, int64_t n, int F, int C, const int32_t* code, float p,
                                                          uint64_t seed, const uint64_t* seed_offset, float* out, int64_t ldo) {
    const int W = F + C, nquad = (W + 3) >> 2;
    const uint64_t s = eff_seed(seed, seed_offset);
    const float scale = p > 0.f ? 1.f / (1.f - p) : 1.f;
    const int64_t total = n * (int64_t)nquad;
    for (int64_t q = (int64_t)blockIdx.x * 256 + threadIdx.x; q < total; q += (int64_t)gridDim.x * 256) {
        const int64_t r = q / nquad;
        const int c0 = (int)(q - r * nquad) * 4;
        const int lab = code ? code[r] : -1;
        uint32_t w[4] = {0u, 0u, 0u, 0u};
        if (p > 0.f) Philox::gen(s, (uint64_t)q, w);
        float v[4];
#pragma unroll
        for (int t = 0; t < 4; ++t) {
            const int c = c0 + t;
            float x = 0.f;
            if (c < F) x = feat[r * ldf + c];
            else if (c < W) x = (c - F == lab) ? 1.f : 0.f;
            v[t] = (p > 0.f && uniform01(w[t]) < p) ? 0.f : x * scale;
        }
        float* o = out + r * ldo + c0;
        if (c0 + 3 < W && (ldo & 3) == 0 && (reinterpret_cast<uintptr_t>(out) & 15) == 0) {
            *reinterpret_cast<float4*>(o) = make_float4(v[0], v[1], v[2], v[3]);
        } else {
#pragma unroll
            for (int t = 0; t < 4; ++t)
                if (c0 + t < W) o[t] = v[t];
        }
    }
}

constexpr int kReuseMaxPerLane = 8;
__global__ __launch_bounds__(256) void build_input_reuse_kernel(const float* feat, int64_t ldf, int64_t n, int F, int C, const int32_t* code,
                                                                const uint8_t* reuse, const float* pred, int64_t ldp, float p, uint64_t seed,
                                                                const uint64_t* seed_offset, float* out, int64_t ldo) {
    __shared__ float prob[16][16 * kReuseMaxPerLane + 16];
    const int W = F + C, nquad = (W + 3) >> 2;
    const uint64_t s = eff_seed(seed, seed_offset);
    const float scale = p > 0.f ? 1.f / (1.f - p) : 1.f;
    const int l16 = threadIdx.x & 15, g = threadIdx.x >> 4;
    const bool vec_out = (ldo & 3) == 0 && (reinterpret_cast<uintptr_t>(out) & 15) == 0;
    const bool vec_in = (ldf & 3) == 0 && (reinterpret_cast<uintptr_t>(feat) & 15) == 0;
    for (int64_t base = (int64_t)blockIdx.x * 16; base < n; base += (int64_t)gridDim.x * 16) {
        const int64_t r = base + g;
        const bool live = r < n;
        const int lab = live ? code[r] : 0;
        const bool soft = live && lab < 0 && (!reuse || reuse[r] != 0);
        const float* xr = pred + (soft ? r : 0) * ldp;
        float v[kReuseMaxPerLane];
        float m = -INFINITY;
#pragma unroll
        for (int k = 0; k < kReuseMaxPerLane; ++k) {
            const int c = l16 + 16 * k;
            v[k] = (soft && c < C) ? xr[c] : -INFINITY;
            m = fmaxf(m, v[k]);
        }
#pragma unroll
        for (int o = 8; o > 0; o >>= 1) m = fmaxf(m, __shfl_xor(m, o, 16));
        float se = 0.f;
#pragma unroll
        for (int k = 0; k < kReuseMaxPerLane; ++k) {
            v[k] = (soft && l16 + 16 * k < C) ? expf(v[k] - m) : 0.f;
            se += v[k];
        }
#pragma unroll
        for (int o = 8; o > 0; o >>= 1) se += __shfl_xor(se, o, 16);
        if (soft) {
            const float inv = 1.f / se;
#pragma unroll
            for (int k = 0; k < kReuseMaxPerLane; ++k) {
                const int c = l16 + 16 * k;
                if (c < C) prob[g][c] = v[k] * inv;
            }
        }
        __syncthreads();
        if (live) {
            const float* fr = feat + r * ldf;
            float* orow = out + r * ldo;
            for (int quad = l16; quad < nquad; quad += 16) {
                const int c0 = quad * 4;
                uint32_t w[4] = {0u, 0u, 0u, 0u};
                if (p > 0.f) Philox::gen(s, (uint64_t)(r * nquad + quad), w);
// ... 102 lines not shown
    int n_tensors;
    float lr, alpha, eps, weight_decay;
    const float* lr_dev;
};

__global__ __launch_bounds__(256) void rmsprop_kernel(RmsArgs a) {
    int t = 0;
    while (t + 1 < a.n_tensors && (int)blockIdx.x >= a.first_block[t + 1]) ++t;
    const int64_t i0 = ((int64_t)(blockIdx.x - a.first_block[t]) * 256 + threadIdx.x) * 4;
    const float lr = a.lr_dev ? a.lr_dev[0] : a.lr;
    float* p = a.p[t];
    const float* g = a.g[t];
    float* sq = a.sq[t];
#pragma unroll
    for (int e = 0; e < 4; ++e) {
        const int64_t i = i0 + e;
        if (i < a.numel[t]) {
            float gi = g[i];
            if (a.weight_decay != 0.f) gi = fmaf(a.weight_decay, p[i], gi);
            const float s = a.alpha * sq[i] + (1.f - a.alpha) * gi * gi;
            sq[i] = s;
            p[i] = p[i] - lr * (gi / (sqrtf(s) + a.eps));
        }
    }
}

}
}

extern "C" int bot_label_split_f32(const int64_t* train_idx, int64_t n_train, const int64_t* labels, int64_t ldl, const uint8_t* mask, float mask_rate,
                                   uint64_t seed, const uint64_t* seed_offset, int32_t use_labels, int32_t* code, float* wn, float* count,
                                   int32_t* workspace, bot_stream_t stream) {
    using namespace bot;
    BOT_REQUIRE(n_train >= 0 && train_idx && wn && count && workspace && (!use_labels || (code && labels)), -1, "label_split: null pointer");
    const int nb = (int)std::max<int64_t>(1, std::min<int64_t>(kSplitBlocks, (n_train + 255) / 256));
    hipLaunchKernelGGL(label_split_kernel, dim3(nb), dim3(256), 0, (hipStream_t)stream, train_idx, n_train, labels, ldl, mask, mask_rate, seed, seed_offset,
                       (int)use_labels, code, wn, workspace);
    hipLaunchKernelGGL(label_count_kernel, dim3(1), dim3(64), 0, (hipStream_t)stream, workspace, nb, count);
    return hip_status("label_split");
}

extern "C" int bot_build_input_f32(const float* feat, int64_t ldf, int64_t n, int32_t F, int32_t C, const int32_t* code, float p, uint64_t seed,
                                   const uint64_t* seed_offset, float* out, int64_t ldo, bot_stream_t stream) {
    using namespace bot;
    BOT_REQUIRE(n >= 0 && F >= 0 && C >= 0 && F + C > 0 && feat && out && ldo >= F + C && ldf >= F && p >= 0.f && p < 1.f && (C == 0 || code), -1,
                "build_input: bad arguments");
    if (n == 0) return 0;
    const int64_t total = n * (int64_t)((F + C + 3) / 4);
    hipLaunchKernelGGL(build_input_kernel, dim3((unsigned)std::min<int64_t>((total + 255) / 256, 65536)), dim3(256), 0, (hipStream_t)stream, feat, ldf, n, (int)F,
                       (int)C, code, p, seed, seed_offset, out, ldo);
    return hip_status("build_input");
}

extern "C" int bot_build_input_reuse_f32(const float* feat, int64_t ldf, int64_t n, int32_t F, int32_t C, const int32_t* code, const uint8_t* reuse,
                                         const float* pred, int64_t ldp, float p, uint64_t seed, const uint64_t* seed_offset, float* out, int64_t ldo,
                                         bot_stream_t stream) {
    using namespace bot;
    BOT_REQUIRE(C >= 1 && C <= 16 * kReuseMaxPerLane, BOT_E_RANGE, "build_input_reuse: C=%d (1 <= C <= %d)", (int)C, 16 * kReuseMaxPerLane);
    BOT_REQUIRE(n >= 0 && F >= 0 && ldo >= F + C && ldf >= F && ldp >= C && p >= 0.f && p < 1.f, BOT_E_RANGE,
                "build_input_reuse: n=%lld F=%d ldf=%lld ldp=%lld ldo=%lld p=%f", (long long)n, (int)F, (long long)ldf, (long long)ldp, (long long)ldo, (double)p);
    BOT_REQUIRE(out && code && pred && (F == 0 || feat), BOT_E_NULL, "build_input_reuse: NULL pointer (feat, code, pred, out)");
    if (n == 0) return 0;
    hipLaunchKernelGGL(build_input_reuse_kernel, dim3((unsigned)std::min<int64_t>((n + 15) / 16, 65536)), dim3(256), 0, (hipStream_t)stream, feat, ldf, n, (int)F,
                       (int)C, code, reuse, pred, ldp, p, seed, seed_offset, out, ldo);
    return hip_status("build_input_reuse");
}

extern "C" int bot_node_loss_f32(const float* x, int64_t ldx, int64_t n, int32_t C, const int64_t* labels, int64_t ldl, const float* wn, const float* count,
                                 int32_t kind, float eps, float* y, int64_t n_pad, float* dx, int64_t lddx, bot_stream_t stream) {
    using namespace bot;
    BOT_REQUIRE(n >= 0 && C > 0 && C <= 16 * kLossMaxPerLane && x && labels && wn && count && y && n_pad >= n && kind >= 0 && kind <= 2 && (!dx || lddx >= C),
                -1, "node_loss: bad arguments (1 <= C <= %d)", 16 * kLossMaxPerLane);
    if (n_pad == 0) return 0;
    hipLaunchKernelGGL(node_loss_kernel<false>, dim3((unsigned)((n_pad * 16 + 255) / 256)), dim3(256), 0, (hipStream_t)stream, x, ldx, n, (int)C, labels, ldl,
                       wn, nullptr, count, (int)kind, eps, y, dx, lddx, n_pad);
    return hip_status("node_loss");
}

extern "C" int bot_node_loss_weighted_f32(const float* x, int64_t ldx, int64_t n, int32_t C, const int64_t* labels, int64_t ldl, const float* wn,
                                          const float* lw, const float* wsum, int32_t kind, float eps, float* y, int64_t n_pad, float* dx, int64_t lddx,
                                          bot_stream_t stream) {
    using namespace bot;
    BOT_REQUIRE(n >= 0 && C > 0 && C <= 16 * kLossMaxPerLane && n_pad >= n && kind >= 0 && kind <= 2 && (!dx || lddx >= C) && ldx >= C, BOT_E_RANGE,
                "node_loss_weighted: n=%lld n_pad=%lld C=%d kind=%d ldx=%lld lddx=%lld (1 <= C <= %d)", (long long)n, (long long)n_pad, (int)C, (int)kind,
                (long long)ldx, (long long)lddx, 16 * kLossMaxPerLane);
    BOT_REQUIRE(x && labels && wn && lw && wsum && y, BOT_E_NULL, "node_loss_weighted: NULL pointer (x, labels, wn, lw, wsum, y)");
    if (n_pad == 0) return 0;
    hipLaunchKernelGGL(node_loss_kernel<true>, dim3((unsigned)((n_pad * 16 + 255) / 256)), dim3(256), 0, (hipStream_t)stream, x, ldx, n, (int)C, labels, ldl,
                       wn, lw, wsum, (int)kind, eps, y, dx, lddx, n_pad);
    return hip_status("node_loss_weighted");
}

extern "C" int bot_rmsprop_step_f32(int32_t n_tensors, float* const* params, const float* const* grads, float* const* square_avg, const int64_t* numel,
                                    float lr, const float* lr_dev, float alpha, float eps, float weight_decay, bot_stream_t stream) {
    using namespace bot;
    BOT_REQUIRE(n_tensors >= 0 && n_tensors <= kMaxTensors, -1, "rmsprop_step: at most %d tensors per call (got %d)", kMaxTensors, n_tensors);
    if (n_tensors == 0) return 0;
    RmsArgs a;
    int blocks = 0;
    for (int t = 0; t < n_tensors; ++t) {
        BOT_REQUIRE(params[t] && grads[t] && square_avg[t] && numel[t] >= 0, -1, "rmsprop_step: null pointer in tensor %d", t);
        a.p[t] = params[t], a.g[t] = grads[t], a.sq[t] = square_avg[t], a.numel[t] = numel[t];
        a.first_block[t] = blocks;
        blocks += (int)((numel[t] + 1023) / 1024);
    }
    a.first_block[n_tensors] = blocks;
// ... 6 lines not shown
```

### bot_amd/nn/fused.py

```python
from __future__ import annotations

import os
from types import SimpleNamespace

import torch
import torch.nn as nn
import torch.nn.functional as F

from .. import _C, gemm, halo, side
from ..graph import take_rows
from ..ops import bn_epilogue_forward, bn_epilogue_sums, new_dropout_seed, stats_partials_for


ABSMAX_BYPRODUCT = os.environ.get("BOT_ABSMAX_BYPRODUCT", "1") != "0"
SKIP_Y = os.environ.get("BOT_SKIP_Y", "1") != "0"
HANDLES = 0
SKINNY = os.environ.get("BOT_SKINNY", "1") != "0"
FORCE = False
CALLS = 0
AGG_CALLS = 0
L0_CALLS = 0


def can_fuse(conv, norm, activation, graph, training, stack_residual) -> bool:
# ... 477 lines not shown


def _small_mm(a, b, b_is_kn, out):
    if a.is_cuda and SKINNY:
        return _C.skinny_gemm(a, b, b_is_kn=b_is_kn, out=out)
    out.copy_(a @ (b if b_is_kn else b.t()))
    return out


def use_agg_first(conv) -> bool:
    return AGG_FIRST and conv._in_src_feats <= conv._out_feats and conv._num_heads <= 4 and conv._in_src_feats <= 256


class _GATHiddenAggFirst(torch.autograd.Function):

    @staticmethod
    def forward(ctx, h, W, Wr, bn_w, bn_b, graph, bn, H, D, has_res, has_er, slope, attn_p, drop_p, bn_training, kp, sym, y_needed=True):
        N, Fin, HD = h.shape[0], h.shape[1], H * D
        Nd = graph.number_of_dst_nodes()
        csc = graph.csc
        ctx.cfg, ctx.graph = (H, D, has_res, has_er, slope), graph
        ctx.sym = sym
        ctx.kp = kp
        skinny = SKINNY and h.is_cuda and Fin <= 256 and N >= 4096
        l0h = _l0_halves_ok(h, H, D, Fin, has_res, sym, attn_p, graph) and not ctx.needs_input_grad[0]
        ctx.l0h = l0h
        if l0h:
            P2 = Wr.shape[1 if kp else 0]
            out2 = torch.empty((N, P2), dtype=h.dtype, device=h.device)
            _small_mm(h, Wr[:, HD:] if kp else Wr[HD:], kp, out2[:, HD:])
        elif skinny:
            out2 = _C.skinny_gemm(h, Wr, b_is_kn=kp, out=torch.empty((N, Wr.shape[1 if kp else 0]), dtype=h.dtype, device=h.device))
        else:
            out2 = torch.mm(h, Wr) if kp else torch.mm(h, Wr.t())
        ctx.skinny = skinny
        c = HD if has_res else 0
        ext = None
        if graph.halo is not None:
            import torch.distributed as dist
            plan = graph.halo
            Wd = _ext_width(Fin, H)
            ext = torch.empty((N + plan.n_halo, Wd), dtype=h.dtype, device=h.device)
            ext[:N, :Fin] = h
            ext[:N, Fin:Fin + H] = out2[:, c:c + H]
            if Wd > Fin + H:
                ext[:N, Fin + H:].zero_()
            send = _C.gather_rows(ext[:N], plan.send_rows) if plan.n_send else ext.new_empty((0, Wd))
            halo.a2a(ext[N:], send, plan.recv_splits, plan.send_splits, plan.group)
            xsrc = ext[:, :Fin]
            el = ext[:, Fin:Fin + H].contiguous()
        else:
            xsrc = h
            el = out2[:, c:c + H].contiguous()
        er = out2[:Nd, c + H:c + 2 * H].contiguous() if has_er else None
        if sym:
            s_out, w_e = sym_scales(graph)
            el = el * s_out.unsqueeze(1)
        ctx.zs = _C.zsign_buffer(csc, H, slope)
        ctx.adrop = (attn_p, new_dropout_seed(attn_p)) if attn_p > 0 else None
        a, a_d = _C.gat_attn_fwd(csc, el, er, None, None, None, slope, H, None, ctx.zs, drop=ctx.adrop or (0.0, 0))
        if sym:
            a_d = a_d * w_e
        if l0h:
            global L0_CALLS
            L0_CALLS += 1
            FP, DP, g_fwd, _, _ = _l0_tables(H, D, Fin, out2.shape[1], kp, Nd)
            KA = (1 + H) * FP
            xscale = _C.halves_scale(h) if ext is None else _C.halves_scale_from_slots(_C.absmax_into(xsrc, _C.absmax_slots(h.device)))
            A = torch.empty((Nd, 2 * KA), dtype=torch.float16, device=h.device)
            _C.halves_split_cols(h if Nd == N else h[:Nd], xscale, 2, A, KA, 0, FP)
            _C.spmm_bcast_halves(csc, xsrc, a_d, None, xscale, A, FP, FP, KA, FP)
            Wres = (Wr.t()[:HD] if kp else Wr[:HD]).contiguous()
            slots = _C.absmax_slots(h.device)
            _C.absmax_into(Wres, slots)
            _C.absmax_into(W, slots)
            wscale = _C.halves_scale_from_slots(slots)
            B = torch.empty((HD, 6 * FP), dtype=torch.float16, device=h.device)
            _C.halves_split_cols(Wres, wscale, 1, B, 2 * FP, 0, FP)
            _C.halves_split_cols(W, wscale, 1, B, 2 * FP, FP, FP)
            x = out2[:Nd, :HD]
            partials = None
            if bn is not None and h.is_cuda | FORCE:
                carries = int(_C._lib.bot_gemm_halves3_nt_bn_rows(2 * FP)) == 256
                partials = stats_partials_for(bn, bn_training, Nd, HD, h.device, carries and gemm.epilogue_piece(HD, x) is not None)
            _C.gemm_halves3_nt_grouped(A, B, xscale, wscale, KA, 2 * FP, out2, g_fwd, FP // 32, stats=partials)
            return _finish_forward(ctx, x, bn, bn_w, bn_b, bn_training, drop_p, y_needed, partials, h=h, W=W, Wr=Wr, z=A,
                                   table=ext if ext is not None else h, el=el, er=er, a=a, a_d=a_d, xscale=xscale)
        z = _C.spmm_bcast(csc, xsrc, a_d, None, head_outer=True)
        Wh = W.view(H, D, Fin)
        if has_res and skinny:
            _C.skinny_gemm(z, Wh, b_is_kn=False, out=out2, accumulate=True, batch=H, strides=(Nd * Fin, D * Fin, D), m=Nd, n=D, k=Fin)
            x = out2[:Nd, :HD]
        elif has_res:
            for i in range(H):
                out2[:Nd, i * D:(i + 1) * D].addmm_(z[i], Wh[i].t())
            x = out2[:Nd, :HD]
        elif skinny:
            agg = _C.skinny_gemm(z, Wh, b_is_kn=False, out=torch.empty((H, Nd, D), dtype=h.dtype, device=h.device), batch=H,
                                 strides=(Nd * Fin, D * Fin, Nd * D), m=Nd, n=D, k=Fin)
            x = agg.permute(1, 0, 2).reshape(Nd, HD)
        else:
            agg = torch.empty((H, Nd, D), dtype=h.dtype, device=h.device)
            for i in range(H):
                torch.mm(z[i], Wh[i].t(), out=agg[i])
            x = agg.permute(1, 0, 2).reshape(Nd, HD)
        return _finish_forward(ctx, x, bn, bn_w, bn_b, bn_training, drop_p, y_needed, h=h, W=W, Wr=Wr, z=z,
                               table=ext if ext is not None else h, el=el, er=er, a=a, a_d=a_d)

    @staticmethod
    def backward(ctx, dy):
        H, D, has_res, has_er, slope = ctx.cfg
        g, epi, s = ctx.graph, ctx.epi, _saved(ctx)
        h, W, Wr, z, table, el, er, a, a_d = s.h, s.W, s.Wr, s.z, s.table, s.el, s.er, s.a, s.a_d
        if epi is not None and epi.out_link is not None:
            dy = epi.out_link.stored(dy)
        dy = dy.contiguous()
        d_bn_w = d_bn_b = None
        l0h, kp = ctx.l0h, ctx.kp
        N, Fin, HD, P2 = h.shape[0], h.shape[1], H * D, Wr.shape[1 if kp else 0]
        Nd = g.number_of_dst_nodes()
        dout2 = torch.empty((N, P2), dtype=h.dtype, device=h.device)
        dx = dout2[:Nd, :HD] if has_res else torch.empty((Nd, HD), dtype=h.dtype, device=h.device)
        if has_res and Nd < N:
            dout2[Nd:, :HD].zero_()
        direct = l0h and L0_DIRECT and epi is not None and D % 2 == 0
        slots = _C.absmax_slots(dy.device) if l0h and (ABSMAX_BYPRODUCT or direct) and epi is not None else None
        Dh = dscale = None
        if epi is None:
            dx.copy_(dy)
        else:
            (sg, sgx), (d_bn_b, d_bn_w) = bn_epilogue_sums(epi, dy, s.x, s.mean, s.invstd, s.bn_w, s.bn_b, True, epi.bn_training and epi.sync,
                                                           slots if direct else None)
            if direct:
                DP = (D + 63) // 64 * 64
                dscale = _C.halves_scale_from_slots(slots)
                Dh = _C.bn_act_bwd_apply_halves(dy, s.x, s.mean, s.invstd, s.bn_w, s.bn_b, True, epi.drop_p, epi.seed, sg, sgx, epi.total,
                                                dscale, _l0_dh(dy.device, Nd, H, D, DP), D, DP)
            else:
                _C.bn_act_bwd_apply(dy, s.x, s.mean, s.invstd, s.bn_w, s.bn_b, True, epi.drop_p, epi.seed, sg, sgx, epi.total, out=dx, absmax=slots)
        Wh = W.view(H, D, Fin)
        dz = torch.empty((H, Nd, Fin), dtype=h.dtype, device=h.device)
        dW3 = torch.empty((H, D, Fin), dtype=h.dtype, device=h.device) if ctx.needs_input_grad[1] and not l0h else None
        if l0h:
            FP, DP, _, g_dz, t_tn = _l0_tables(H, D, Fin, P2, kp, Nd)
            if Dh is None:
                dscale = _C.halves_scale_from_slots(slots) if slots is not None else _C.halves_scale(dx)
                Dh = _C.halves_split_heads(dx, dscale, H, D, DP)
            Wt = gemm.split(Wh.transpose(1, 2).reshape(H * Fin, D), 1)
            _C.gemm_halves3_nt_grouped(Dh, Wt.buf, dscale, Wt.scale, H * DP, Wt.piece, dz[0], g_dz, 0)
            flat = torch.empty(HD * Fin + P2 * Fin, dtype=h.dtype, device=h.device)

            def wgrad():
                _C.gemm_halves3_tn_grouped(z, Dh, s.xscale, dscale, (1 + H) * FP, H * DP, flat, t_tn)
                return flat
            if side.usable(flat):
                side.run(wgrad, z, Dh, s.xscale, dscale, flat)
            else:
                wgrad()
        elif ctx.skinny and D <= 256:
            _C.skinny_gemm(dx, Wh, b_is_kn=True, out=dz, batch=H, strides=(D, D * Fin, Nd * Fin), m=Nd, n=Fin, k=D)
        if ctx.skinny and dW3 is not None:
            _C.tn_gemm(dx, z, out=dW3, batch=H, strides=(D, Nd * Fin, 0), n=Nd, kx=D, ky=Fin)
        for i in range(H if not l0h else 0):
            dxi = dx[:, i * D:(i + 1) * D]
            if not (ctx.skinny and D <= 256):
                torch.mm(dxi, Wh[i], out=dz[i])
            if dW3 is not None and not ctx.skinny:
                torch.mm(dxi.t(), z[i], out=dW3[i])
        dW = dW3.view(HD, Fin) if dW3 is not None else None
        halo = g.halo is not None
        c = HD if has_res else 0
        need_dh = ctx.needs_input_grad[0]
        if not need_dh:
            xsrc = table[:, :Fin] if halo else h
            da = _C.sddmm_dot_bcast(g.csc, xsrc, dz)
            dh_g = None
        elif halo:
            dext = torch.empty_like(table)
            _, da = _C.spmm_dot_bcast(g.csr, dz, a_d, g.csr2csc, table[:, :Fin], out=dext[:, :Fin])
        else:
            dh_g, da = _C.spmm_dot_bcast(g.csr, dz, a_d, g.csr2csc, h)
        d_el, der = _attn_backward(ctx, da, el, er, a)
        if halo and not need_dh:
            dsm = d_el.new_zeros((d_el.shape[0], (H + 3) // 4 * 4))
            dsm[:, :H] = d_el
            d_el = _extend_backward(g, dsm, N)[:, :H]
        elif halo:
            _score_columns(dext, Fin, d_el)
            own = _extend_backward(g, dext, N)
            dh_g, d_el = own[:, :Fin], own[:, Fin:Fin + H]
        _score_columns(dout2, c, d_el, der)
        dWr = None
        if l0h:
            dW = flat[:HD * Fin].view(HD, Fin)
            dWr = flat[HD * Fin:].view((Fin, P2) if kp else (P2, Fin))
            tail = dout2[:, HD:]
            if h.is_cuda and tail.shape[1] <= 32:
                _C.tn_narrow(tail, h, dWr[:, HD:] if kp else dWr[HD:], transpose_out=kp)
            elif h.is_cuda:
                _C.tn_gemm(tail, h, out=dWr[:, HD:] if kp else dWr[HD:], transpose_out=kp)
            elif kp:
                dWr[:, HD:] = h.t() @ tail
            else:
                dWr[HD:] = tail.t() @ h
            side.join()
            if not ctx.needs_input_grad[1]:
                dW = None
            if not ctx.needs_input_grad[2]:
                dWr = None
        elif ctx.needs_input_grad[2]:
            dWr = torch.mm(h.t(), dout2) if kp else torch.mm(dout2.t(), h)
        dh = None
        if need_dh:
            dh = torch.addmm(dh_g, dout2, Wr.t() if kp else Wr)
        return (dh, dW, dWr, d_bn_w if ctx.needs_input_grad[3] else None, d_bn_b if ctx.needs_input_grad[4] else None,
                None, None, None, None, None, None, None, None, None, None, None, None, None)


def halves_only_consumer(conv, norm, activation, graph, training, stack_residual, n_rows, on_device) -> bool:
    return (SKIP_Y and (on_device or FORCE) and can_fuse(conv, norm, activation, graph, training, stack_residual) and not use_agg_first(conv)
            and gemm.MODE == "halves" and (gemm.FORCE or (on_device and n_rows >= gemm.MIN_ROWS)))


_INPUT_DROPPED = [False]


class input_already_dropped:

    def __init__(self, on=True):
        self.on = bool(on)

    def __enter__(self):
        _INPUT_DROPPED[0] = self.on
        return self

    def __exit__(self, *exc):
        _INPUT_DROPPED[0] = False
        return False


def take_input_dropped() -> bool:
    v = _INPUT_DROPPED[0]
    _INPUT_DROPPED[0] = False
    return v


def gat_hidden_layer(conv, bn, graph, h, dropout_p, training, y_needed=True):
    from . import has_zero_in_degree
    if not conv._allow_zero_in_degree:
        assert not has_zero_in_degree(graph), "0-in-degree nodes (models.py:477-479)"
    global CALLS
    CALLS += 1
    H, D = conv._num_heads, conv._out_feats
    attn_p = conv.attn_drop.p if training else 0.0
    bn_w = bn.weight if bn is not None and bn.affine else None
    bn_b = bn.bias if bn is not None and bn.affine else None
    bn_training = bn is not None and (bn.training or not bn.track_running_stats)
    if use_agg_first(conv):
        global AGG_CALLS
        AGG_CALLS += 1
        return _GATHiddenAggFirst.apply(h, conv.fc.weight, merged_weight(conv, with_fc=False), bn_w, bn_b, graph, bn, H, D,
                                        conv.res_fc is not None, conv.attn_r is not None, conv.leaky_relu.negative_slope,
                                        attn_p, dropout_p if training and bn is not None else 0.0, bn_training, WEIGHT_KP,
                                        conv._use_symmetric_norm, y_needed)
    if bn is None:
        return _GATHidden.apply(h, merged_weight(conv), None, None, graph, None, H, D, conv.res_fc is not None,
                                conv.attn_r is not None, conv.leaky_relu.negative_slope, attn_p, 0.0, False, WEIGHT_KP,
                                conv._use_symmetric_norm)
    return _GATHidden.apply(h, merged_weight(conv), bn.weight if bn.affine else None, bn.bias if bn.affine else None, graph, bn,
                            H, D, conv.res_fc is not None, conv.attn_r is not None, conv.leaky_relu.negative_slope,
                            conv.attn_drop.p if training else 0.0, dropout_p if training else 0.0, bn_training, WEIGHT_KP,
                            conv._use_symmetric_norm, y_needed)



_GENERATION = [0]


def bump_generation():
    _GENERATION[0] += 1


def _versions(*ts):
    return (_GENERATION[0],) + tuple((t.data_ptr(), t._version) for t in ts if t is not None)


def _cached(owner, slot, key, make):
    c = owner.__dict__.setdefault("_bot_infer_cache", {})
    hit = c.get(slot)
    if hit is None or hit[0] != key:
        hit = c[slot] = (key, make())
    return hit[1]

# ... 67 lines not shown

def count_infer():
    global INFER_CALLS
    INFER_CALLS += 1


L0_INFER = os.environ.get("BOT_L0_INFER", "1") != "0"
L0_INFER_CALLS = 0


L0_INFER_OVER_LABEL_REUSE = os.environ.get("BOT_L0_INFER_LABEL_REUSE", "1") != "0"


def _infer_l0_ok(conv, graph, h, label_reuse_cols) -> bool:
    return (L0_INFER and L0_HALVES and use_agg_first(conv) and (not label_reuse_cols or L0_INFER_OVER_LABEL_REUSE) and graph.halo is None
            and conv.res_fc is not None
            and not conv._use_symmetric_norm and conv._out_feats <= 256 and h.shape[1] <= 192 and (h.is_cuda or FORCE)
            and gemm.MODE == "halves" and gemm.NT_KERNEL == "halves3" and (h.shape[0] >= gemm.MIN_ROWS or gemm.FORCE or FORCE))


def _infer_l0(conv, epi, graph, h, relu):
    global L0_INFER_CALLS
    L0_INFER_CALLS += 1
    H, D = conv._num_heads, conv._out_feats
    HD, N, Fin = H * D, graph.number_of_dst_nodes(), h.shape[1]
    has_er = conv.attn_r is not None
    csc = graph.csc
    Wr = _cached(conv, "wcat_agg", _infer_key(conv), lambda: merged_weight(conv, with_fc=False).detach())
    kp = WEIGHT_KP
    P2 = Wr.shape[1 if kp else 0]
    FP, _, g_fwd, _, _ = _l0_tables(H, D, Fin, P2, kp, N)
    KA = (1 + H) * FP

    def right_operand():
        Wres = (Wr.t()[:HD] if kp else Wr[:HD]).contiguous()
        W = conv.fc.weight.detach()
        slots = _C.absmax_slots(h.device)
        _C.absmax_into(Wres, slots)
        _C.absmax_into(W, slots)
        wscale = _C.halves_scale_from_slots(slots)
        B = torch.empty((HD, 6 * FP), dtype=torch.float16, device=h.device)
        _C.halves_split_cols(Wres, wscale, 1, B, 2 * FP, 0, FP)
        _C.halves_split_cols(W, wscale, 1, B, 2 * FP, FP, FP)
        return B, wscale
    B, wscale = _cached(conv, "infer_l0_halves", _infer_key(conv) + (str(h.device),), right_operand)
    tail = torch.empty((h.shape[0], P2 - HD), dtype=h.dtype, device=h.device)
    _small_mm(h, Wr[:, HD:] if kp else Wr[HD:], kp, tail)
    el = tail[:, :H]
    er = tail[:N, H:2 * H] if has_er else None
    a = _C.gat_attn_fwd(csc, el, er, None, None, None, conv.leaky_relu.negative_slope, H, None)
    xscale = _C.halves_scale(h)
    A = torch.empty((N, 2 * KA), dtype=torch.float16, device=h.device)
    _C.halves_split_cols(h if N == h.shape[0] else h[:N], xscale, 2, A, KA, 0, FP)
    _C.spmm_bcast_halves(csc, h, a, None, xscale, A, FP, FP, KA, FP)
    scale, shift = eval_affine(epi)
    y = torch.empty((N, HD), dtype=h.dtype, device=h.device)
    slots = _C.absmax_slots(h.device) if (relu and ABSMAX_BYPRODUCT and gemm.enabled(h)) else None
    _C.gemm_halves3_nt_grouped(A, B, xscale, wscale, KA, 2 * FP, y, g_fwd, FP // 32, col_scale=scale, col_shift=shift, relu=relu, absmax=slots)
    if slots is not None:
        gemm.stash_scale(y, _C.halves_scale_from_slots(slots))
    return y


@torch.no_grad()
def gat_infer_layer(conv, epi, graph, h, relu, first=False):
    from . import has_zero_in_degree
    if not conv._allow_zero_in_degree:
        assert not has_zero_in_degree(graph), "0-in-degree nodes (models.py:477-479)"
    global INFER_CALLS
    INFER_CALLS += 1
    H, D = conv._num_heads, conv._out_feats
    HD, N = H * D, graph.number_of_dst_nodes()
    has_res, has_er = conv.res_fc is not None, conv.attn_r is not None
    W = infer_weight(conv)
    ctx = _LabelReuse.active
    F0 = ctx.static_cols if (ctx is not None and first and 0 < ctx.static_cols < h.shape[1]) else 0
    if _infer_l0_ok(conv, graph, h, F0):
        return _infer_l0(conv, epi, graph, h, relu)
    if F0:
        Wk = W if WEIGHT_KP else W.t()
        key = (id(conv), h.data_ptr(), tuple(h.shape)) + _versions(W)
        if ctx.store.get("key") != key:
            ctx.store["key"], ctx.store["base"] = key, torch.mm(h[:, :F0], Wk[:F0])
        out = torch.addmm(ctx.store["base"], h[:, F0:], Wk[F0:])
    elif gemm.enabled(h):
        out = gemm.mm_nt(gemm.split_with_stash(h, 0), _cached(conv, "infer_halves", _infer_key(conv),
                                                   lambda: gemm.split_right(W.t().contiguous() if WEIGHT_KP else W)))
    else:
        out = torch.mm(h, W) if WEIGHT_KP else torch.mm(h, W.t())
    B = block_width(HD)
    c = 2 * B if has_res else B
    if graph.halo is not None:
        ext = _extend_forward(graph, out, HD, H, c)
        ft, el = ext[:, :HD], ext[:, HD:HD + H]
    else:
        ft, el = out[:, :HD], out[:, c:c + H]
    er = out[:N, c + H:c + 2 * H] if has_er else None
    ew = None
    if conv._use_symmetric_norm:
        s_out, w_e = sym_scales(graph)
        el = el * s_out.unsqueeze(1)
        ew = w_e
    scale, shift = eval_affine(epi)
    res = out[:N, B:B + HD].unflatten(1, (H, D)) if has_res else None
    slots = _C.absmax_slots(h.device) if (relu and ABSMAX_BYPRODUCT and gemm.enabled(h)) else None
    y = _C.gat_infer(graph.csc, ft.unflatten(1, (H, D)), el, er, None, ew, conv.leaky_relu.negative_slope, addend=res,
                     scale=scale, shift=shift, relu=relu, absmax=slots)
# ... 5 lines not shown
```

### bot_amd/train.py

```python
from __future__ import annotations

import math
import os
import weakref

import torch
import torch.nn.functional as F

EPSILON = 1 - math.log(2)
FUSED_STEP = os.environ.get("BOT_FUSED_STEP", "1") != "0"
FUSED_REUSE = os.environ.get("BOT_FUSED_REUSE", "1") != "0"
FORCE_REUSE = False
DEBUG_KEEP_PREDS = False
DEBUG_PREDS = []
_SPLIT = {}
_REUSE = {}


def _split_buffers(train_idx, n):
    key = (train_idx.device, n, id(train_idx))
    ent = _SPLIT.get(key)
    if ent is None or ent[0]() is not train_idx or ent[3] != train_idx._version:
        ent = (weakref.ref(train_idx), torch.full((n,), -1, dtype=torch.int32, device=train_idx.device),
               torch.zeros(n, dtype=torch.float32, device=train_idx.device), train_idx._version)
# ... 43 lines not shown
class _NodeLossWeighted(torch.autograd.Function):

    @staticmethod
    def forward(ctx, pred, labels, wn, lw, kind):
        from . import _C
        n = pred.shape[0]
        lwp = torch.zeros((n + 63) // 64 * 64, dtype=torch.float32, device=pred.device)
        lwp[:n] = torch.where(wn > 0, lw, torch.zeros_like(lw))
        wsum = _C.colsum(lwp.view(-1, 64)).sum().reshape(1)
        y, dx = _C.node_loss_weighted(pred, labels, wn, lw, wsum, kind, EPSILON, want_grad=pred.requires_grad)
        ctx.save_for_backward(dx)
        return _C.colsum(y.view(-1, 64)).sum() / wsum[0]

    @staticmethod
    def backward(ctx, g):
        (dx,) = ctx.saved_tensors
        return dx * g, None, None, None, None


def weighted_node_loss(pred, labels, wn, lw, kind="logit"):
    from .ops import sum_all
    y = per_node_loss(pred, labels.clamp(0, pred.shape[1] - 1), kind)
    lw = lw.to(y.dtype)
    on = wn > 0
    return sum_all(torch.where(on, lw * y, torch.zeros_like(y))) / sum_all(torch.where(on, lw, torch.zeros_like(lw)))


def _check_loss_weight(loss_weight, n):
    if loss_weight.shape != (n,) or not loss_weight.is_floating_point():
        raise ValueError(f"loss_weight holds one float per node of the graph the step runs on ({n}), got {tuple(loss_weight.shape)} "
                         f"{loss_weight.dtype}")


def _forward(model, graph, feat, edge_weight):
    return model(graph, feat) if edge_weight is None else model(graph, feat, edge_weight=edge_weight)


def _fused_forward_backward(model, graph, feat, labels, train_idx, *, use_labels, mask_rate, loss, n_classes, mask, count_reduce=None,
                            n_label_iters=0, val_idx=None, test_idx=None, loss_weight=None, edge_weight=None):
    from . import _C
    from .nn import fused
    from .ops import new_dropout_seed
    n = feat.shape[0]
    code, wn = _split_buffers(train_idx, n)
    count = _C.label_split(train_idx, labels, mask, mask_rate, new_dropout_seed(1.0) if mask is None else 0, use_labels,
                           code if use_labels else None, wn)
    if count_reduce is not None:
        count_reduce(count)
    from . import nn as bnn
    drop = getattr(model, "input_drop", None) if isinstance(model, (bnn.GAT, bnn.GCN)) else None
    if use_labels:
        p = float(drop.p) if (drop is not None and model.training) else 0.0
        static = feat
        feat = _C.build_input(static, code, n_classes, p, new_dropout_seed(p))
        if n_label_iters > 0:
            reuse = _reuse_members(n, train_idx, val_idx, test_idx)
            with torch.no_grad():
                for _ in range(n_label_iters):
                    with fused.input_already_dropped(drop is not None):
                        prev = _forward(model, graph, feat, edge_weight)
                    if DEBUG_KEEP_PREDS:
                        DEBUG_PREDS.append(prev)
                    feat = _C.build_input_reuse(static, code, reuse, prev, n_classes, p, new_dropout_seed(p), out=feat)
                    del prev
        with fused.input_already_dropped(drop is not None):
            pred = _forward(model, graph, feat, edge_weight)
    else:
        pred = _forward(model, graph, feat, edge_weight)
    if loss_weight is not None:
        _check_loss_weight(loss_weight, n)
        if pred.shape[1] <= 128:
            out = _NodeLossWeighted.apply(pred, labels, wn, loss_weight.to(torch.float32).contiguous(), loss)
        else:
            out = weighted_node_loss(pred, labels, wn, loss_weight, loss)
    elif pred.shape[1] <= 128:
        out = _NodeLoss.apply(pred, labels, wn, count, loss)
    else:
        from .ops import sum_all
        y = per_node_loss(pred, labels.clamp(0, pred.shape[1] - 1), loss)
        out = sum_all(torch.where(wn > 0, y, torch.zeros_like(y))) / count[0]
    out.backward()
    return out, pred, wn if (wn.is_cuda and torch.cuda.is_current_stream_capturing()) else wn.clone()


def add_labels(feat, labels, idx, n_classes):
    onehot = torch.zeros([feat.shape[0], n_classes], device=feat.device, dtype=feat.dtype)
    onehot[idx, labels[idx, 0]] = 1
    return torch.cat([feat, onehot], dim=-1)


def per_node_loss(x, labels, loss="logit"):
    y = F.cross_entropy(x, labels[:, 0], reduction="none")
    if loss == "loge":
        y = torch.log(EPSILON + y) - math.log(EPSILON)
    elif loss == "savage":
        y = (1 - torch.exp(-y)) ** 2
    elif loss != "logit":
        raise ValueError(f"unknown loss {loss!r}")
    return y


def compute_loss(x, labels, loss="logit"):
    return torch.mean(per_node_loss(x, labels, loss))


def adjust_learning_rate(optimizer, lr, epoch):
    if epoch <= 50:
        for group in optimizer.param_groups:
            group["lr"] = lr * epoch / 50


def compute_acc(pred, labels):
    return ((torch.argmax(pred, dim=1) == labels[:, 0]).float().sum() / len(pred)).item()


def forward_backward(model, graph, feat, labels, train_idx, val_idx, test_idx, *, use_labels=True, mask_rate=0.5,
                     n_label_iters=0, loss="logit", n_classes=None, mask=None, loss_weight=None, edge_weight=None):
    reuse = n_label_iters > 0 and use_labels and reuse_path_ok(feat, n_classes)
    if FUSED_STEP and (n_label_iters == 0 or reuse) and feat.dtype == torch.float32 and loss in ("logit", "loge", "savage"):
        return _fused_forward_backward(model, graph, feat, labels, train_idx, use_labels=use_labels, mask_rate=mask_rate, loss=loss,
                                       n_classes=n_classes, mask=mask, n_label_iters=n_label_iters if reuse else 0, val_idx=val_idx,
                                       test_idx=test_idx, loss_weight=loss_weight, edge_weight=edge_weight)
    if mask is None:
        mask = torch.rand(train_idx.shape, device=train_idx.device) < mask_rate
    if use_labels:
        onehot = torch.zeros([feat.shape[0], n_classes], device=feat.device, dtype=feat.dtype)
        onehot[train_idx, labels[train_idx, 0]] = mask.to(feat.dtype)
        feat = torch.cat([feat, onehot], dim=-1)
        w = (~mask).to(feat.dtype)
    else:
        w = mask.to(feat.dtype)
    pred = _forward(model, graph, feat, edge_weight)
    if n_label_iters > 0 and use_labels:
        m = mask.unsqueeze(1)
        for _ in range(n_label_iters):
            pred = pred.detach()
            prob = F.softmax(pred, dim=-1)
            feat[train_idx, -n_classes:] = torch.where(m, feat[train_idx, -n_classes:], prob[train_idx])
            for idx in (val_idx, test_idx):
                feat[idx, -n_classes:] = prob[idx]
            pred = _forward(model, graph, feat, edge_weight)
    wn = torch.zeros(pred.shape[0], device=pred.device, dtype=pred.dtype)
    wn[train_idx] = w
    if loss_weight is not None:
        _check_loss_weight(loss_weight, pred.shape[0])
        out = weighted_node_loss(pred, labels, wn, loss_weight, loss)
        out.backward()
        return out, pred, w
    y = per_node_loss(pred, labels.clamp(0, pred.shape[1] - 1), loss)
    from .ops import sum_all
    out = sum_all(torch.where(wn > 0, y, torch.zeros_like(y))) / sum_all(w)
    out.backward()
    return out, pred, w


def train_step(model, graph, feat, labels, train_idx, val_idx, test_idx, optimizer, **kw):
    model.train()
    optimizer.zero_grad()
    loss, pred, _ = forward_backward(model, graph, feat, labels, train_idx, val_idx, test_idx, **kw)
    optimizer.step()
    return loss, pred


@torch.no_grad()
def evaluate(model, graph, feat, labels, train_idx, val_idx, test_idx, *, use_labels=True, n_label_iters=0, loss="logit",
             n_classes=None):
    import contextlib
    from .nn import fused
    model.eval()
    n_static = feat.shape[1]
    if use_labels:
        feat = add_labels(feat, labels, train_idx, n_classes)
    with (fused.label_reuse(n_static) if (use_labels and n_label_iters > 0) else contextlib.nullcontext()):
        pred = model(graph, feat)
        if n_label_iters > 0:
            unlabel_idx = torch.cat([val_idx, test_idx])
            for _ in range(n_label_iters):
                feat[unlabel_idx, -n_classes:] = F.softmax(pred[unlabel_idx], dim=-1)
                pred = model(graph, feat)
    losses = tuple(compute_loss(pred[i], labels[i], loss) for i in (train_idx, val_idx, test_idx))
    accs = tuple(compute_acc(pred[i], labels[i]) for i in (train_idx, val_idx, test_idx))
    return accs + losses + (pred,)


CAPTURE_DRAIN_S = float(os.environ.get("BOT_CAPTURE_DRAIN_S", "1.0"))


def drain_rccl_watchdog(device=None) -> bool:
    import time
    import torch.distributed as dist
    if not (dist.is_available() and dist.is_initialized()) or not torch.cuda.is_available():
        return False
    if "nccl" not in str(dist.get_backend()).lower():
        return False
    torch.cuda.synchronize(device)
    time.sleep(CAPTURE_DRAIN_S)
    return True


class CapturedTrainStep:

    def __init__(self, step_fn, device, warmup: int = 3):
        from . import _C
        self.device = torch.device(device)
        if _C.SEED_OFFSET is None or _C.SEED_OFFSET.device != self.device:
            _C.SEED_OFFSET = torch.zeros(1, dtype=torch.int64, device=self.device)
        self._off = _C.SEED_OFFSET
        self._step_fn = step_fn

        def body():
            self._off.add_(1)
            return step_fn()

        side = torch.cuda.Stream(device=self.device)
        side.wait_stream(torch.cuda.current_stream(self.device))
        with torch.cuda.stream(side):
            for _ in range(warmup):
                body()
        torch.cuda.current_stream(self.device).wait_stream(side)
        self.graph = torch.cuda.CUDAGraph()
        import torch.distributed as dist
        mode = "thread_local" if dist.is_available() and dist.is_initialized() else "global"
        self.drained = drain_rccl_watchdog(self.device)
        with torch.cuda.graph(self.graph, capture_error_mode=mode):
            self.loss, self.pred = body()

# ... 19 lines not shown
```

### include/bot_gnn.h

```cpp
#ifndef BOT_GNN_H
#define BOT_GNN_H

#include <stdint.h>

#ifdef __cplusplus
extern "C" {
#endif

#define BOT_ABI_VERSION 19

#define BOT_E_NULL (-1)
#define BOT_E_RANGE (-2)
#define BOT_E_ALIGN (-3)
#define BOT_E_PLAN (-4)

typedef void* bot_stream_t;

int bot_abi_version(void);
const char* bot_last_error(void);
int bot_stream_create(int32_t high_priority, bot_stream_t* out);
const char* bot_last_kernel(void);
int bot_debug_abort_trace(const char* path_host);

int bot_row_plan_size_host(const int32_t* indptr_host, int64_t n_rows, int32_t chunk,
// ... 8 lines not shown
                             int64_t* sizes , bot_stream_t stream);
int bot_row_plan_fill_device(const int32_t* indptr, int64_t n_rows, int32_t chunk, const void* workspace, int64_t workspace_bytes,
                             int64_t n_items, int64_t n_long, int64_t n_slots, int32_t* items ,
                             int32_t* long_rows , int32_t* long_ptr , bot_stream_t stream);

int64_t bot_csc_transpose_workspace_bytes(int64_t nnz);
int bot_csc_transpose_i32(const int32_t* indptr, const int32_t* indices, int64_t n_dst, int64_t n_src, int64_t nnz, int32_t* indptr_r,
                          int32_t* indices_r, int32_t* eid_r, int64_t* n_bad, void* workspace, int64_t workspace_bytes,
                          bot_stream_t stream);

int bot_degrees_i64(const int32_t* indptr, int64_t n_rows, int64_t* deg, bot_stream_t stream);

int64_t bot_spmm_workspace_floats(int64_t n_slots, int32_t H, int32_t D);
int bot_spmm_set_layout(int32_t layout);
int bot_spmm_set_zero_skip(int32_t on);
int bot_spmm_f32(const int32_t* indptr, const int32_t* indices, int64_t n_rows, int64_t nnz,
                 const int32_t* items, int64_t n_items,
                 const int32_t* long_rows, const int32_t* long_ptr, int64_t n_long,
                 const float* x, int64_t ldx, int64_t hsx,
                 const float* w, const int32_t* wperm,
                 int32_t H, int32_t D,
                 float* out, int64_t ldo, int64_t hso,
                 const float* addend, int64_t lda, int64_t hsa,
                 float* partial, bot_stream_t stream);

int bot_spmm_blocked_f32(const int32_t* tile_rows, const int32_t* ptr, const int32_t* b_src, const uint8_t* b_lrow,
                         const int32_t* b_pos, int32_t n_tiles, int32_t nblk, int32_t block_rows, int32_t T, int32_t epi,
                         int32_t round_tiles, const float* x, int64_t ldx, const float* w, int32_t H, int32_t D, float* out,
                         int64_t ldo, const float* addend, int64_t lda, bot_stream_t stream);


int bot_spmm_dot_f32(const int32_t* indptr, const int32_t* indices, int64_t n_rows, int64_t nnz,
                     const int32_t* items, int64_t n_items,
                     const int32_t* long_rows, const int32_t* long_ptr, int64_t n_long,
                     const float* x, int64_t ldx, int64_t hsx,
                     const float* w, const int32_t* wperm,
                     const float* y, int64_t ldy, int64_t hsy,
                     int32_t H, int32_t D,
                     float* out, int64_t ldo, int64_t hso,
                     float* dot_out, float* partial, uint32_t* absmax_slots, bot_stream_t stream);

int bot_spmm_bcast_f32(const int32_t* indptr, const int32_t* indices, int64_t n_rows, int64_t nnz,
                       const int32_t* items, int64_t n_items,
                       const int32_t* long_rows, const int32_t* long_ptr, int64_t n_long,
                       const float* x, int64_t ldx, const float* w, const int32_t* wperm,
                       int32_t H, int32_t D, float* out, int64_t ldo, int64_t hso,
                       float* partial, bot_stream_t stream);
int bot_spmm_bcast_halves_f16(const int32_t* indptr, const int32_t* indices, int64_t n_rows, int64_t nnz,
                              const int32_t* items, int64_t n_items,
                              const int32_t* long_rows, const int32_t* long_ptr, int64_t n_long,
                              const float* x, int64_t ldx, const float* w, const int32_t* wperm,
                              int32_t H, int32_t D, const float* hscale, uint16_t* hout, int64_t ldh, int64_t hsh, int32_t h2_off,
                              int32_t hpiece, float* partial, bot_stream_t stream);
int bot_spmm_dot_bcast_f32(const int32_t* indptr, const int32_t* indices, int64_t n_rows, int64_t nnz,
                           const int32_t* items, int64_t n_items,
                           const int32_t* long_rows, const int32_t* long_ptr, int64_t n_long,
                           const float* x, int64_t ldx, int64_t hsx, const float* w, const int32_t* wperm,
                           const float* y, int64_t ldy, int32_t H, int32_t D,
                           float* out, int64_t ldo, float* dot_out, float* partial, bot_stream_t stream);

int bot_sddmm_dot_f32(const int32_t* indptr, const int32_t* indices, int64_t n_rows, int64_t nnz,
                      const int32_t* items, int64_t n_items,
                      const float* x, int64_t ldx, int64_t hsx,
                      const float* y, int64_t ldy, int64_t hsy,
                      int32_t H, int32_t D,
                      float* out, const int32_t* operm, int32_t accumulate, bot_stream_t stream);

int bot_sddmm_dot_bcast_f32(const int32_t* indptr, const int32_t* indices, int64_t n_rows, int64_t nnz,
                            const int32_t* items, int64_t n_items,
                            const float* x, int64_t ldx,
                            const float* y, int64_t ldy, int64_t hsy,
                            int32_t H, int32_t D,
                            float* out, const int32_t* operm, bot_stream_t stream);

int bot_sddmm_u_add_v_f32(const int32_t* src, const int32_t* dst, int64_t n_edges,
                          const float* x, const float* y, int32_t W, float* out, bot_stream_t stream);

int bot_gat_attn_fwd_f32(const int32_t* indptr, const int32_t* indices, int64_t n_rows, int64_t nnz,
                         const int32_t* long_rows, int64_t n_long, int32_t chunk,
                         const float* el, const float* er, const float* ee, const int32_t* eperm,
                         const uint8_t* keep, float slope, int32_t H,
                         float* a, const int32_t* aperm, uint8_t* zsign,
                         float attn_drop, uint64_t drop_seed, const uint64_t* seed_offset, float* a_drop,
                         bot_stream_t stream);

int bot_gat_attn_bwd_f32(const int32_t* indptr, const int32_t* indices, int64_t n_rows, int64_t nnz,
                         const int32_t* long_rows, int64_t n_long, int32_t chunk,
                         const float* el, const float* er, const float* ee, const int32_t* eperm,
                         float slope, int32_t H,
                         const float* a, const float* da, const int32_t* aperm,
                         float* dz, const int32_t* zperm, float* der, const uint8_t* zsign,
                         float attn_drop, uint64_t drop_seed, const uint64_t* seed_offset, bot_stream_t stream);

int64_t bot_gat_infer_workspace_floats(int64_t n_slots, int32_t H, int32_t D);
int bot_gat_infer_f32(const int32_t* indptr, const int32_t* indices, int64_t n_rows, int64_t nnz,
                      const int32_t* items, int64_t n_items,
                      const int32_t* long_rows, const int32_t* long_ptr, int64_t n_long, int64_t n_slots,
                      const float* x, int64_t ldx, int64_t hsx,
                      const float* el, int64_t ldel, const float* er, int64_t lder,
                      const float* ee, const float* ew, float slope, int32_t H, int32_t D,
                      const float* addend, int64_t lda, int64_t hsa,
                      const float* scale, const float* shift, int32_t relu,
                      float* out, int64_t ldo, int64_t hso,
                      float* workspace, uint32_t* absmax_slots , bot_stream_t stream);

int bot_segment_sum_f32(const int32_t* indptr, int64_t n_rows, int64_t nnz,
                        const int32_t* long_rows, int64_t n_long, int32_t chunk,
                        const float* vals, const int32_t* perm, int32_t W,
                        float* out, bot_stream_t stream);

int bot_gather_rows_f32(const float* x, int64_t ldx, const int32_t* rows, int64_t n_sel, int32_t F,
                        float* out, int64_t ldo, bot_stream_t stream);
int bot_scatter_add_rows_f32(float* x, int64_t ldx, const int32_t* rows, int64_t n_sel, int32_t F,
                             const float* vals, int64_t ldv, bot_stream_t stream);

int64_t bot_bn_workspace_floats(int32_t F);
int bot_colstats_f32(const float* x, int64_t ldx, int64_t n, int32_t F, float* mean, float* m2, float* workspace,
                     bot_stream_t stream);
int bot_colsum_f32(const float* x, int64_t ldx, int64_t n, int32_t F, float* sum, float* workspace, bot_stream_t stream);
int bot_bn_stats_f32(const float* x, int64_t ldx, int64_t n, int32_t F, float eps, float momentum, float* mean, float* invstd,
                     float* running_mean, float* running_var, int64_t* num_batches_tracked, float* workspace,
                     bot_stream_t stream);
int bot_bn_act_fwd_f32(const float* x, int64_t ldx, int64_t n, int32_t F, const float* mean, const float* invstd,
                       const float* weight, const float* bias, int32_t relu, float p, uint64_t seed,
                       const uint64_t* seed_offset, float* y, int64_t ldy, bot_stream_t stream);
int bot_bn_stats_halves_f32(const float* x, int64_t ldx, int64_t n, int32_t F, float eps, float momentum, float* mean, float* invstd,
// ... 202 lines not shown
    const float* bias;
    int32_t relu;
    float p;
    uint64_t seed;
    const uint64_t* seed_offset;
    float* part;
    float* pmax;
} bot_bn_bwd_stats_t;
int32_t bot_gemm_halves3_nt_bn_rows(int64_t k);
int bot_gemm_halves3_nt3_f32(int64_t m, int64_t n, int64_t k, const float* scale_a, const float* scale_a2, int64_t k_split, const float* scale_b,
                             const uint16_t* A, int64_t lda, int64_t a2_off, const uint16_t* B, int64_t ldb, int64_t b2_off, int32_t b_layout, float* C,
                             int64_t ldc, const bot_bn_bwd_stats_t* bn, int32_t mode, bot_stream_t stream);
int32_t bot_gemm_halves3_nt_bn_deferred_max_k(void);
int bot_gemm_halves3_nt_bn_reduce_f32(int64_t m, int64_t n, int64_t k, const float* scale_a, const float* scale_a2, int64_t k_split, const float* scale_b,
                                      const uint16_t* A, int64_t lda, int64_t a2_off, const uint16_t* B, int64_t ldb, int64_t b2_off, int32_t b_layout,
                                      float* C, int64_t ldc, const bot_bn_bwd_stats_t* bn, bot_stream_t stream);
int bot_gemm_halves3_nt_bn_apply_f32(int64_t m, int64_t n, int64_t k, const float* scale_a, const float* scale_a2, int64_t k_split, const float* scale_b,
                                     const uint16_t* A, int64_t lda, int64_t a2_off, const uint16_t* B, int64_t ldb, int64_t b2_off, int32_t b_layout,
                                     const bot_bn_bwd_stats_t* bn, const float* sum_g, const float* sum_gx, double total_count, float* dx, int64_t lddx,
                                     const float* hscale, uint16_t* hout, int64_t ldh, int32_t h2_off, int32_t hD, int32_t hDP, uint32_t* absmax_slots,
                                     bot_stream_t stream);
int bot_bn_act_bwd_reduce_partials_f32(const float* part, int32_t nblk, int32_t F, float* sum_g, float* sum_gx, bot_stream_t stream);
int bot_bn_bwd_bound_partials_f32(int32_t F, const float* pmax, int32_t nblk, const float* sum_g, const float* sum_gx, double total_count,
                                  const float* weight, const float* invstd, uint32_t* absmax_slots, bot_stream_t stream);
int bot_bn_bwd_partials_finish_f32(const float* part, const float* pmax, int32_t nblk, int32_t F, float* sum_g, float* sum_gx, int32_t batch_stats,
                                   double total_count, const float* weight, const float* invstd, uint32_t* absmax_slots, bot_stream_t stream);
int bot_halves_split_frag_f16(const float* x, int64_t ldx, int64_t n, int32_t F, const float* scale, uint16_t* out, int32_t piece, bot_stream_t stream);
int bot_gemm_halves3_tn2_f32(int64_t n_rows, int64_t k, int64_t p, int64_t kp, int64_t pp, const float* scale_x, const float* scale_d, const float* scale_d2,
                             int64_t p_split, const uint16_t* X, int64_t ldx, int64_t x2_off, const uint16_t* D, int64_t ldd, int64_t d2_off, float* out,
                             int64_t ldo, float* workspace, int32_t mode, bot_stream_t stream);

int bot_gemm_halves3_nt_grouped_f32(int64_t m, int64_t b_rows, const float* scale_a, const float* scale_b, const uint16_t* A, int64_t lda,
                                    int64_t a2_off, const uint16_t* B, int64_t ldb, int64_t b2_off, float* C, int64_t ldc, int32_t n_groups,
                                    const int64_t* groups, int32_t k_seg, const float* col_scale, const float* col_shift, int32_t relu,
                                    uint32_t* absmax_slots, int32_t mode, bot_stream_t stream);
int bot_gemm_halves3_nt_grouped2_f32(int64_t m, int64_t b_rows, const float* scale_a, const float* scale_b, const uint16_t* A, int64_t lda,
                                     int64_t a2_off, const uint16_t* B, int64_t ldb, int64_t b2_off, float* C, int64_t ldc, int32_t n_groups,
                                     const int64_t* groups, int32_t k_seg, const float* col_scale, const float* col_shift, int32_t relu,
                                     uint32_t* absmax_slots, float* stats_part, float* stats_minmax, float* stats_pivot, int32_t stats_F,
                                     int32_t mode, bot_stream_t stream);
int bot_bn_stats_halves_partials_f32(const float* part, const float* minmax, int32_t nblk, const float* pivot, int64_t n, int32_t F, float eps, float momentum,
                                     float* mean, float* invstd, float* running_mean, float* running_var, int64_t* num_batches_tracked,
                                     const float* weight, const float* bias, float p, float* hscale, float* bound_workspace, bot_stream_t stream);
int64_t bot_gemm_halves3_tn_grouped_workspace_floats(int64_t n_rows, int32_t n_tiles);
int bot_gemm_halves3_tn_grouped_f32(int64_t n_rows, const float* scale_x, const float* scale_d, const uint16_t* X, int64_t ldx, int64_t x2_off,
                                    const uint16_t* D, int64_t ldd, int64_t d2_off, float* out, int32_t n_tiles, const int64_t* tiles,
                                    float* workspace, int32_t mode, bot_stream_t stream);

int bot_label_split_f32(const int64_t* train_idx, int64_t n_train, const int64_t* labels, int64_t ldl, const uint8_t* mask, float mask_rate,
                        uint64_t seed, const uint64_t* seed_offset, int32_t use_labels, int32_t* code, float* wn, float* count, int32_t* workspace,
                        bot_stream_t stream);
int bot_build_input_f32(const float* feat, int64_t ldf, int64_t n, int32_t F, int32_t C, const int32_t* code, float p, uint64_t seed,
                        const uint64_t* seed_offset, float* out, int64_t ldo, bot_stream_t stream);
int bot_build_input_reuse_f32(const float* feat, int64_t ldf, int64_t n, int32_t F, int32_t C, const int32_t* code, const uint8_t* reuse,
                              const float* pred, int64_t ldp, float p, uint64_t seed, const uint64_t* seed_offset, float* out, int64_t ldo,
                              bot_stream_t stream);
int bot_node_loss_f32(const float* x, int64_t ldx, int64_t n, int32_t C, const int64_t* labels, int64_t ldl, const float* wn, const float* count,
                      int32_t kind, float eps, float* y, int64_t n_pad, float* dx, int64_t lddx, bot_stream_t stream);
int bot_node_loss_weighted_f32(const float* x, int64_t ldx, int64_t n, int32_t C, const int64_t* labels, int64_t ldl, const float* wn, const float* lw,
                               const float* wsum, int32_t kind, float eps, float* y, int64_t n_pad, float* dx, int64_t lddx, bot_stream_t stream);
int bot_rmsprop_step_f32(int32_t n_tensors, float* const* params, const float* const* grads, float* const* square_avg, const int64_t* numel,
                         float lr, const float* lr_dev, float alpha, float eps, float weight_decay, bot_stream_t stream);

int bot_gemm_halves_last_algo(int32_t* index, float* ms);
int bot_gemm_halves_library_version(int32_t* compiled, int32_t* runtime);

int bot_skinny_gemm_f32(const float* A, int64_t lda, const float* B, int64_t ldb, int32_t b_is_kn, float* C, int64_t ldc, int64_t m,
                        int32_t n, int32_t k, int32_t accumulate, int32_t batch, int64_t stride_a, int64_t stride_b, int64_t stride_c,
                        bot_stream_t stream);

int64_t bot_tn_narrow_workspace_floats(int64_t n, int32_t kx, int32_t ky);
int bot_tn_narrow_f32(const float* X, int64_t ldx, const float* Y, int64_t ldy, int64_t n, int32_t kx, int32_t ky, float* out, int64_t ldo,
                      int32_t transpose_out, float* workspace, bot_stream_t stream);
int64_t bot_tn_gemm_workspace_floats(int64_t n, int32_t kx, int32_t ky, int32_t batch);
int bot_tn_gemm_f32(const float* X, int64_t ldx, const float* Y, int64_t ldy, int64_t n, int32_t kx, int32_t ky, float* out, int64_t ldo,
                    int32_t transpose_out, int32_t batch, int64_t stride_x, int64_t stride_y, int64_t stride_out, float* workspace,
                    bot_stream_t stream);

#ifdef __cplusplus
}
#endif
#endif
```

Before: 249.1 million.

## Gather only feature columns plus a compact label pair in layer-0 sparse kernels

When labels are appended to input features, the new input builder also emits a per-node (class, value) pair table. The layer-0 SpMM and SDDMM kernels then read only the dense feature columns and rebuild the one-hot label part from that pair, instead of gathering the full one-hot label block for every edge. This cuts gather traffic on the widest input layer. In exchange it adds a context-managed pairing mechanism with version checks, extra kernel variants and a row pitch padded to 32 columns. It also adds a vectorised absmax path for strided inputs.

```diff
diff --git a/bot_amd/_C.py b/bot_amd/_C.py
--- a/bot_amd/_C.py
+++ b/bot_amd/_C.py
@@ -41,12 +41,18 @@
                                           c_int32, _P, c_int64, c_int64, _P, _P]),
     "bot_spmm_bcast_halves_f16": (ctypes.c_int, [_P, _P, c_int64, c_int64, _P, c_int64, _P, _P, c_int64, _P, c_int64, _P, _P, c_int32, c_int32, _P, _P,
                                                  c_int64, c_int64, c_int32, c_int32, _P, _P]),
+    "bot_spmm_bcast_pairs_f32": (ctypes.c_int, [_P, _P, c_int64, c_int64, _P, c_int64, _P, _P, c_int64, _P, c_int64, _P, c_int32, _P, _P, c_int32,
+                                                c_int32, _P, c_int64, c_int64, _P, _P]),
+    "bot_spmm_bcast_halves_pairs_f16": (ctypes.c_int, [_P, _P, c_int64, c_int64, _P, c_int64, _P, _P, c_int64, _P, c_int64, _P, c_int32, _P, _P, c_int32,
+                                                       c_int32, _P, _P, c_int64, c_int64, c_int32, c_int32, _P, _P]),
     "bot_spmm_dot_bcast_f32": (ctypes.c_int, [_P, _P, c_int64, c_int64, _P, c_int64, _P, _P, c_int64, _P, c_int64, c_int64, _P,
                                               _P, _P, c_int64, c_int32, c_int32, _P, c_int64, _P, _P, _P]),
     "bot_sddmm_dot_f32": (ctypes.c_int, [_P, _P, c_int64, c_int64, _P, c_int64, _P, c_int64, c_int64, _P, c_int64, c_int64,
                                          c_int32, c_int32, _P, _P, c_int32, _P]),
     "bot_sddmm_dot_bcast_f32": (ctypes.c_int, [_P, _P, c_int64, c_int64, _P, c_int64, _P, c_int64, _P, c_int64, c_int64, c_int32,
                                                c_int32, _P, _P, _P]),
+    "bot_sddmm_dot_bcast_pairs_f32": (ctypes.c_int, [_P, _P, c_int64, c_int64, _P, c_int64, _P, c_int64, _P, c_int32, _P, c_int64, c_int64, c_int32,
+                                                     c_int32, _P, _P, _P]),
     "bot_sddmm_u_add_v_f32": (ctypes.c_int, [_P, _P, c_int64, _P, _P, c_int32, _P, _P]),
     "bot_gat_attn_fwd_f32": (ctypes.c_int, [_P, _P, c_int64, c_int64, _P, c_int64, c_int32, _P, _P, _P, _P, _P, c_float,
                                             c_int32, _P, _P, _P, c_float, c_uint64, _P, _P, _P]),
@@ -90,6 +96,7 @@
                                                        _P, c_int64, _P, _P, c_int64, c_int32, c_int32, c_int32, _P]),
     "bot_label_split_f32": (ctypes.c_int, [_P, c_int64, _P, c_int64, _P, c_float, c_uint64, _P, c_int32, _P, _P, _P, _P, _P]),
     "bot_build_input_f32": (ctypes.c_int, [_P, c_int64, c_int64, c_int32, c_int32, _P, c_float, c_uint64, _P, _P, c_int64, _P]),
+    "bot_build_input_pairs_f32": (ctypes.c_int, [_P, c_int64, c_int64, c_int32, c_int32, _P, c_float, c_uint64, _P, _P, c_int64, _P, _P]),
     "bot_build_input_reuse_f32": (ctypes.c_int, [_P, c_int64, c_int64, c_int32, c_int32, _P, _P, _P, c_int64, c_float, c_uint64, _P, _P, c_int64, _P]),
     "bot_node_loss_f32": (ctypes.c_int, [_P, c_int64, c_int64, c_int32, _P, c_int64, _P, _P, c_int32, c_float, _P, c_int64, _P, c_int64, _P]),
     "bot_rmsprop_step_f32": (ctypes.c_int, [c_int32, _P, _P, _P, _P, c_float, _P, c_float, c_float, c_float, _P]),
@@ -499,7 +506,33 @@
     return dot
 
 
-def spmm_bcast(d, x, w, wperm=None, head_outer=True):
+PAIR_CALLS = 0
+PAIR_DECLINES = 0
+_E_RANGE = -2
+
+
+def _label_pairs(pairs, x, label_col):
+    if pairs is None:
+        return None
+    if pairs.dtype != torch.int32 or pairs.dim() != 2 or pairs.shape != (x.shape[0], 2) or not pairs.is_contiguous() or pairs.device != x.device:
+        raise BotKernelError(f"label pairs must be contiguous int32 [{x.shape[0]}, 2] on {x.device}, got {pairs.dtype} {tuple(pairs.shape)}")
+    if not 0 <= int(label_col) <= x.shape[1]:
+        raise BotKernelError(f"label_col={label_col} outside the {x.shape[1]} columns of x")
+    return pairs
+
+
+def _pairs_or_full(name, key, with_pairs, full, what):
+    global PAIR_CALLS, PAIR_DECLINES
+    if with_pairs is not None:
+        rc = _timed(name, key, with_pairs)
+        if rc != _E_RANGE:
+            PAIR_CALLS += 1
+            return _check(rc, what + "_pairs")
+        PAIR_DECLINES += 1
+    _check(_timed(name, key, full), what)
+
+
+def spmm_bcast(d, x, w, wperm=None, head_outer=True, pairs=None, label_col=0):
     _dev(x, w, d.indptr)
     _f32(x, "x")
     if x.stride(1) != 1:
@@ -515,14 +548,16 @@
     partial = None
     if d.n_long:
         partial = torch.empty(int(_lib.bot_spmm_workspace_floats(d.n_slots, H, D)), dtype=torch.float32, device=x.device)
-    _check(_timed("spmm_bcast", (H, D), lambda: _lib.bot_spmm_bcast_f32(
-        d.indptr.data_ptr(), d.indices.data_ptr(), d.n_rows, d.nnz, d.items.data_ptr(), d.n_items, _ptr(d.long_rows),
-        _ptr(d.long_ptr), d.n_long, x.data_ptr(), x.stride(0), w.data_ptr(), _ptr(_i32(wperm, "wperm")), H, D, out.data_ptr(),
-        ldo, hso, _ptr(partial), _stream())), "spmm_bcast")
-    return out
-
-
-def spmm_bcast_halves(d, x, w, wperm, hscale, hout, col0, hsh, h2_off, hpiece):
+    pairs = _label_pairs(pairs, x, label_col)
+    head = (d.indptr.data_ptr(), d.indices.data_ptr(), d.n_rows, d.nnz, d.items.data_ptr(), d.n_items, _ptr(d.long_rows), _ptr(d.long_ptr), d.n_long,
+            x.data_ptr(), x.stride(0))
+    tail = (w.data_ptr(), _ptr(_i32(wperm, "wperm")), H, D, out.data_ptr(), ldo, hso, _ptr(partial), _stream())
+    _pairs_or_full("spmm_bcast", (H, D), None if pairs is None else lambda: _lib.bot_spmm_bcast_pairs_f32(*head, pairs.data_ptr(), int(label_col), *tail),
+                   lambda: _lib.bot_spmm_bcast_f32(*head, *tail), "spmm_bcast")
+    return out
+
+
+def spmm_bcast_halves(d, x, w, wperm, hscale, hout, col0, hsh, h2_off, hpiece, pairs=None, label_col=0):
     _dev(x, w, d.indptr, hout, hscale)
     _f32(x, "x")
     if x.stride(1) != 1:
@@ -534,10 +569,14 @@
     partial = None
     if d.n_long:
         partial = torch.empty(int(_lib.bot_spmm_workspace_floats(d.n_slots, H, D)), dtype=torch.float32, device=x.device)
-    _check(_timed("spmm_bcast", (H, D), lambda: _lib.bot_spmm_bcast_halves_f16(
-        d.indptr.data_ptr(), d.indices.data_ptr(), d.n_rows, d.nnz, d.items.data_ptr(), d.n_items, _ptr(d.long_rows),
-        _ptr(d.long_ptr), d.n_long, x.data_ptr(), x.stride(0), w.data_ptr(), _ptr(_i32(wperm, "wperm")), H, D, hscale.data_ptr(),
-        hout.data_ptr() + 2 * col0, hout.stride(0), hsh, h2_off, hpiece, _ptr(partial), _stream())), "spmm_bcast_halves")
+    pairs = _label_pairs(pairs, x, label_col)
+    head = (d.indptr.data_ptr(), d.indices.data_ptr(), d.n_rows, d.nnz, d.items.data_ptr(), d.n_items, _ptr(d.long_rows), _ptr(d.long_ptr), d.n_long,
+            x.data_ptr(), x.stride(0))
+    tail = (w.data_ptr(), _ptr(_i32(wperm, "wperm")), H, D, hscale.data_ptr(), hout.data_ptr() + 2 * col0, hout.stride(0), hsh, h2_off, hpiece,
+            _ptr(partial), _stream())
+    _pairs_or_full("spmm_bcast", (H, D),
+                   None if pairs is None else lambda: _lib.bot_spmm_bcast_halves_pairs_f16(*head, pairs.data_ptr(), int(label_col), *tail),
+                   lambda: _lib.bot_spmm_bcast_halves_f16(*head, *tail), "spmm_bcast_halves")
     return hout
 
 
@@ -576,7 +615,7 @@
     return out
 
 
-def sddmm_dot_bcast(d, x, y, operm=None):
+def sddmm_dot_bcast(d, x, y, operm=None, pairs=None, label_col=0):
     _dev(x, y, d.indptr)
     _f32(x, "x"), _f32(y, "y")
     if x.stride(1) != 1:
@@ -584,9 +623,12 @@
     assert y.dim() == 3 and y.is_contiguous()
     H, n, D = y.shape
     out = torch.empty((d.nnz, H), dtype=torch.float32, device=x.device)
-    _check(_timed("sddmm_dot_bcast", (H, D), lambda: _lib.bot_sddmm_dot_bcast_f32(
-        d.indptr.data_ptr(), d.indices.data_ptr(), d.n_rows, d.nnz, d.items.data_ptr(), d.n_items, x.data_ptr(), x.stride(0),
-        y.data_ptr(), D, n * D, H, D, out.data_ptr(), _ptr(_i32(operm, "operm")), _stream())), "sddmm_dot_bcast")
+    pairs = _label_pairs(pairs, x, label_col)
+    head = (d.indptr.data_ptr(), d.indices.data_ptr(), d.n_rows, d.nnz, d.items.data_ptr(), d.n_items, x.data_ptr(), x.stride(0))
+    tail = (y.data_ptr(), D, n * D, H, D, out.data_ptr(), _ptr(_i32(operm, "operm")), _stream())
+    _pairs_or_full("sddmm_dot_bcast", (H, D),
+                   None if pairs is None else lambda: _lib.bot_sddmm_dot_bcast_pairs_f32(*head, pairs.data_ptr(), int(label_col), *tail),
+                   lambda: _lib.bot_sddmm_dot_bcast_f32(*head, *tail), "sddmm_dot_bcast")
     return out
 
 
@@ -1159,6 +1201,23 @@
     return out
 
 
+def build_input_pairs(feat, code, n_classes, p, seed, pitch=None):
+    _dev(feat, code)
+    _f32(feat, "feat")
+    n, F = feat.shape
+    W = F + n_classes
+    if code is None or code.dtype != torch.int32 or code.shape != (n,) or not code.is_contiguous():
+        raise BotKernelError(f"build_input_pairs: code must be contiguous int32 [{n}]")
+    pitch = W if pitch is None else int(pitch)
+    if pitch < W:
+        raise BotKernelError(f"build_input_pairs: pitch {pitch} below the {W} columns")
+    out = torch.empty((n, pitch), dtype=torch.float32, device=feat.device)[:, :W]
+    pairs = torch.empty((n, 2), dtype=torch.int32, device=feat.device)
+    _check(_lib.bot_build_input_pairs_f32(feat.data_ptr(), _ld(feat), n, F, n_classes, code.data_ptr(), float(p), int(seed), _seed_off(p), out.data_ptr(),
+                                          pitch, pairs.data_ptr(), _stream()), "build_input_pairs")
+    return out, pairs
+
+
 REUSE_CALLS = 0
 
 
diff --git a/bot_amd/csrc/common.h b/bot_amd/csrc/common.h
--- a/bot_amd/csrc/common.h
+++ b/bot_amd/csrc/common.h
@@ -29,6 +29,14 @@
     } while (0)
 
 inline bool aligned(const void* p, size_t a) { return (reinterpret_cast<uintptr_t>(p) % a) == 0; }
+
+#define BOT_REQUIRE_PAIRS(what)                                                                                                            \
+    do {                                                                                                                                   \
+        BOT_REQUIRE(F > 0 && F < D && F % 4 == 0, BOT_E_RANGE, what ": F=%d must be a multiple of 4 inside (0, D=%d): keep the full gather", \
+                    (int)F, (int)D);                                                                                                       \
+        BOT_REQUIRE(pairs, BOT_E_NULL, what ": NULL pair table");                                                                         \
+        BOT_REQUIRE(bot::aligned(pairs, 8), BOT_E_ALIGN, what ": pair table not 8-byte aligned");                                        \
+    } while (0)
 
 inline unsigned launch_grid(int64_t n, int64_t per_block, int64_t cap = 4096) {
     int64_t b = (n + per_block - 1) / per_block;
diff --git a/bot_amd/csrc/halves.hip b/bot_amd/csrc/halves.hip
--- a/bot_amd/csrc/halves.hip
+++ b/bot_amd/csrc/halves.hip
@@ -29,6 +29,15 @@
         for (int64_t j = (nq << 2) + (int64_t)blockIdx.x * kBlock + threadIdx.x; j < total; j += stride) m = fmaxf(m, fabsf(x[j]));
     } else if (ldx == F) {
         for (int64_t i = (int64_t)blockIdx.x * kBlock + threadIdx.x; i < total; i += (int64_t)gridDim.x * kBlock) m = fmaxf(m, fabsf(x[i]));
+    } else if (((F | ldx) & 3) == 0 && (reinterpret_cast<uintptr_t>(x) & 15) == 0) {
+        const int Fq = F >> 2;
+        const int64_t nq = n * (int64_t)Fq, ldq = ldx >> 2;
+        const float4* x4 = reinterpret_cast<const float4*>(x);
+        for (int64_t i = (int64_t)blockIdx.x * kBlock + threadIdx.x; i < nq; i += (int64_t)gridDim.x * kBlock) {
+            const int64_t r = i / Fq;
+            const float4 a = x4[r * ldq + (i - r * Fq)];
+            m = fmaxf(m, fmaxf(fmaxf(fabsf(a.x), fabsf(a.y)), fmaxf(fabsf(a.z), fabsf(a.w))));
+        }
     } else {
         for (int64_t i = (int64_t)blockIdx.x * kBlock + threadIdx.x; i < total; i += (int64_t)gridDim.x * kBlock) {
             const int64_t r = i / F;
diff --git a/bot_amd/csrc/sddmm.hip b/bot_amd/csrc/sddmm.hip
--- a/bot_amd/csrc/sddmm.hip
+++ b/bot_amd/csrc/sddmm.hip
@@ -14,6 +14,11 @@
     float* out;
     const int32_t* operm;
     int32_t accumulate;
+};
+
+struct DotLabelPairs {
+    const int2* pairs;
+    int32_t F;
 };
 
 template <int LANES, int U>
@@ -144,8 +149,8 @@
     else launch_dot<VEC, 64, 4>(a, st);
 }
 
-template <int VEC, int LANES, int NCHUNK, int HB>
-__global__ __launch_bounds__(kBlock) void sddmm_dot_bcast_kernel(DotArgs a) {
+template <int VEC, int LANES, int NCHUNK, int HB, bool PAIRS>
+__device__ __forceinline__ void sddmm_dot_bcast_sweep(const DotArgs& a, const DotLabelPairs& lp) {
     static_assert(LANES >= 16 && HB <= 4, "butterfly layout");
     constexpr int U = 4;
     const int lane = threadIdx.x % LANES;
@@ -158,13 +163,16 @@
         beg = __builtin_amdgcn_readfirstlane(beg);
         end = __builtin_amdgcn_readfirstlane(end);
     }
-    int off[NCHUNK];
+    int off[NCHUNK], rel[NCHUNK];
+    bool lab[NCHUNK];
     float yv[HB][NCHUNK][VEC];
 #pragma unroll
     for (int c = 0; c < NCHUNK; ++c) {
         const int e = (c * LANES + lane) * VEC;
         const bool act = e < a.D;
         off[c] = act ? e : 0;
+        lab[c] = PAIRS && act && e >= lp.F;
+        rel[c] = lab[c] ? e - lp.F : INT32_MIN / 2;
 #pragma unroll
         for (int h = 0; h < HB; ++h) {
             vload<VEC>(yv[h][c], a.y + (int64_t)row * a.ldy + (int64_t)h * a.hsy + off[c]);
@@ -177,6 +185,7 @@
     for (int k0 = beg; k0 < end; k0 += LANES) {
         const int k = k0 + lane;
         const int idx = k < end ? a.indices[k] : 0;
+        int2 pr = make_int2(-1, 0);
         const int cnt = min(LANES, end - k0);
         for (int i = 0; i < cnt; i += U) {
             float p[16], v[U][NCHUNK][VEC];
@@ -184,10 +193,33 @@
             for (int q = 0; q < 16; ++q) p[q] = 0.f;
 #pragma unroll
             for (int u = 0; u < U; ++u) {
-                const int s = group_bcast<LANES>(idx, min(i + u, cnt - 1));
+                const int j = min(i + u, cnt - 1);
+                const int s = group_bcast<LANES>(idx, j);
                 const float* px = a.x + (int64_t)s * a.ldx;
-#pragma unroll
-                for (int c = 0; c < NCHUNK; ++c) vload<VEC>(v[u][c], px + off[c]);
+                if constexpr (PAIRS) {
+#pragma unroll
+                    for (int c = 0; c < NCHUNK; ++c) {
+#pragma unroll
+                        for (int t = 0; t < VEC; ++t) v[u][c][t] = 0.f;
+                        if (!lab[c]) vload<VEC>(v[u][c], px + off[c]);
+                    }
+                } else {
+#pragma unroll
+                    for (int c = 0; c < NCHUNK; ++c) vload<VEC>(v[u][c], px + off[c]);
+                }
+            }
+            if constexpr (PAIRS) {
+                if (i == 0 && k < end) pr = lp.pairs[idx];
+#pragma unroll
+                for (int u = 0; u < U; ++u) {
+                    const int j = min(i + u, cnt - 1);
+                    const int cls = group_bcast<LANES>(pr.x, j);
+                    const float val = __int_as_float(group_bcast<LANES>(pr.y, j));
+#pragma unroll
+                    for (int c = 0; c < NCHUNK; ++c)
+#pragma unroll
+                        for (int t = 0; t < VEC; ++t) v[u][c][t] = rel[c] + t == cls ? val : v[u][c][t];
+                }
             }
 #pragma unroll
             for (int u = 0; u < U; ++u)
@@ -210,15 +242,30 @@
     }
 }
 
+template <int VEC, int LANES, int NCHUNK, int HB>
+__global__ __launch_bounds__(kBlock) void sddmm_dot_bcast_kernel(DotArgs a) {
+    sddmm_dot_bcast_sweep<VEC, LANES, NCHUNK, HB, false>(a, DotLabelPairs{nullptr, 0});
+}
+
+template <int VEC, int LANES, int NCHUNK, int HB>
+__global__ __launch_bounds__(kBlock) void sddmm_dot_bcast_pairs_kernel(DotArgs a, DotLabelPairs lp) {
+    sddmm_dot_bcast_sweep<VEC, LANES, NCHUNK, HB, true>(a, lp);
+}
+
 template <int VEC, int HB>
-static void dispatch_dot_bcast(const DotArgs& a, hipStream_t st) {
+static void dispatch_dot_bcast(const DotArgs& a, const DotLabelPairs& lp, hipStream_t st) {
     const int L = (a.D + VEC - 1) / VEC;
 #define BOT_DOTB(LN, NC)                                                                                                    \
     do {                                                                                                                    \
         const int64_t blocks = (a.n_items * LN + kBlock - 1) / kBlock;                                                      \
         if (blocks == 0) break;                                                                                             \
-        set_kernel("bot::sddmm_dot_bcast_kernel<%d,%d,%d,%d>", VEC, LN, NC, HB);                                           \
-        hipLaunchKernelGGL((sddmm_dot_bcast_kernel<VEC, LN, NC, HB>), dim3((unsigned)blocks), dim3(kBlock), 0, st, a);      \
+        if (lp.pairs) {                                                                                                     \
+            set_kernel("bot::sddmm_dot_bcast_pairs_kernel<%d,%d,%d,%d>", VEC, LN, NC, HB);                                  \
+            hipLaunchKernelGGL((sddmm_dot_bcast_pairs_kernel<VEC, LN, NC, HB>), dim3((unsigned)blocks), dim3(kBlock), 0, st, a, lp); \
+        } else {                                                                                                            \
+            set_kernel("bot::sddmm_dot_bcast_kernel<%d,%d,%d,%d>", VEC, LN, NC, HB);                                        \
+            hipLaunchKernelGGL((sddmm_dot_bcast_kernel<VEC, LN, NC, HB>), dim3((unsigned)blocks), dim3(kBlock), 0, st, a);  \
+        }                                                                                                                   \
     } while (0)
     if (L <= 16) BOT_DOTB(16, 1);
     else if (L <= 32) BOT_DOTB(32, 1);
@@ -269,11 +316,10 @@
     return hip_status("sddmm_dot launch");
 }
 
-int bot_sddmm_dot_bcast_f32(const int32_t* indptr, const int32_t* indices, int64_t n_rows, int64_t nnz, const int32_t* items,
-                            int64_t n_items, const float* x, int64_t ldx, const float* y, int64_t ldy, int64_t hsy, int32_t H,
-                            int32_t D, float* out, const int32_t* operm, bot_stream_t stream) {
+static int sddmm_dot_bcast_impl(const int32_t* indices, int64_t n_rows, int64_t nnz, const int32_t* items,
+                            int64_t n_items, const float* x, int64_t ldx, const int32_t* pairs, int32_t F, const float* y, int64_t ldy, int64_t hsy,
+                            int32_t H, int32_t D, float* out, const int32_t* operm, bot_stream_t stream) {
     using namespace bot;
-    (void)indptr;
     BOT_REQUIRE(n_rows >= 0 && nnz >= 0 && n_items >= 0 && nnz < INT32_MAX && n_rows < INT32_MAX, BOT_E_RANGE, "sddmm_dot_bcast: bad size");
     BOT_REQUIRE(H >= 1 && H <= 4 && D >= 1 && D <= 1024, BOT_E_RANGE, "sddmm_dot_bcast: H=%d (1..4) D=%d (1..1024)", H, D);
     if (nnz == 0 || n_rows == 0) return 0;
@@ -283,16 +329,32 @@
     const int vec = pick_vec(D, {ldx, ldy, H > 1 ? hsy : 0}, {x, y});
     BOT_REQUIRE(D <= vec * 256, BOT_E_RANGE, "sddmm_dot_bcast: D=%d exceeds one launch tile", D);
     DotArgs a{indices, reinterpret_cast<const int4*>(items), n_items, x, ldx, 0, y, ldy, hsy, H, D, out, operm, 0};
+    const DotLabelPairs lp{reinterpret_cast<const int2*>(pairs), F};
 #define BOT_DOTB_H(V)                                       \
     switch (H) {                                            \
-        case 1: dispatch_dot_bcast<V, 1>(a, st); break;     \
-        case 2: dispatch_dot_bcast<V, 2>(a, st); break;     \
-        case 3: dispatch_dot_bcast<V, 3>(a, st); break;     \
-        default: dispatch_dot_bcast<V, 4>(a, st); break;    \
+        case 1: dispatch_dot_bcast<V, 1>(a, lp, st); break;     \
+        case 2: dispatch_dot_bcast<V, 2>(a, lp, st); break;     \
+        case 3: dispatch_dot_bcast<V, 3>(a, lp, st); break;     \
+        default: dispatch_dot_bcast<V, 4>(a, lp, st); break;    \
     }
     if (vec == 4) { BOT_DOTB_H(4) } else if (vec == 2) { BOT_DOTB_H(2) } else { BOT_DOTB_H(1) }
 #undef BOT_DOTB_H
     return hip_status("sddmm_dot_bcast launch");
+}
+
+int bot_sddmm_dot_bcast_f32(const int32_t* indptr, const int32_t* indices, int64_t n_rows, int64_t nnz, const int32_t* items,
+                            int64_t n_items, const float* x, int64_t ldx, const float* y, int64_t ldy, int64_t hsy, int32_t H,
+                            int32_t D, float* out, const int32_t* operm, bot_stream_t stream) {
+    (void)indptr;
+    return sddmm_dot_bcast_impl(indices, n_rows, nnz, items, n_items, x, ldx, nullptr, 0, y, ldy, hsy, H, D, out, operm, stream);
+}
+
+int bot_sddmm_dot_bcast_pairs_f32(const int32_t* indptr, const int32_t* indices, int64_t n_rows, int64_t nnz, const int32_t* items,
+                                  int64_t n_items, const float* x, int64_t ldx, const int32_t* pairs, int32_t F, const float* y, int64_t ldy,
+                                  int64_t hsy, int32_t H, int32_t D, float* out, const int32_t* operm, bot_stream_t stream) {
+    (void)indptr;
+    BOT_REQUIRE_PAIRS("sddmm_dot_bcast_pairs");
+    return sddmm_dot_bcast_impl(indices, n_rows, nnz, items, n_items, x, ldx, pairs, F, y, ldy, hsy, H, D, out, operm, stream);
 }
 
 int bot_sddmm_u_add_v_f32(const int32_t* src, const int32_t* dst, int64_t n_edges, const float* x, const float* y,
diff --git a/bot_amd/csrc/spmm.hip b/bot_amd/csrc/spmm.hip
--- a/bot_amd/csrc/spmm.hip
+++ b/bot_amd/csrc/spmm.hip
@@ -35,6 +35,18 @@
     int32_t skip;
 };
 
+struct LabelPairs {
+    const int2* pairs;
+    int32_t F;
+};
+
+constexpr int kNoLabelLane = INT32_MIN / 2;
+template <int VEC>
+__device__ __forceinline__ void label_values(float (&v)[VEC], int rel, int cls, float val) {
+#pragma unroll
+    for (int t = 0; t < VEC; ++t) v[t] = rel + t == cls ? val : v[t];
+}
+
 __device__ __forceinline__ bool is_zero_weight(float w) { return (__float_as_uint(w) << 1) == 0u; }
 __device__ __forceinline__ bool wants_row(float w, uint32_t force) { return ((__float_as_uint(w) << 1) | force) != 0u; }
 __device__ __forceinline__ void settle(float& v) { asm volatile("" : "+v"(v)); }
@@ -684,6 +696,109 @@
     }
 }
 
+template <int VEC, int LANES, int NCHUNK, int HB>
+__global__ __launch_bounds__(kBlock) void spmm_bcast_pairs_kernel(SpmmArgs a, LabelPairs lp) {
+    constexpr int U = 4;
+    const int lane = threadIdx.x % LANES;
+    const int64_t item = ((int64_t)blockIdx.x * kBlock + threadIdx.x) / LANES;
+    if (item >= a.n_items) return;
+    const int4 it = a.items[item];
+    int row = it.x, beg = it.y, end = it.z, slot = it.w;
+    if constexpr (LANES == 64) {
+        row = __builtin_amdgcn_readfirstlane(row);
+        beg = __builtin_amdgcn_readfirstlane(beg);
+        end = __builtin_amdgcn_readfirstlane(end);
+        slot = __builtin_amdgcn_readfirstlane(slot);
+    }
+    int off[NCHUNK], rel[NCHUNK];
+    bool act[NCHUNK], lab[NCHUNK];
+    float acc[HB][NCHUNK][VEC];
+#pragma unroll
+    for (int c = 0; c < NCHUNK; ++c) {
+        const int e = (c * LANES + lane) * VEC;
+        act[c] = e < a.D;
+        off[c] = act[c] ? e : 0;
+        lab[c] = act[c] && e >= lp.F;
+        rel[c] = lab[c] ? e - lp.F : kNoLabelLane;
+#pragma unroll
+        for (int h = 0; h < HB; ++h)
+#pragma unroll
+            for (int t = 0; t < VEC; ++t) acc[h][c][t] = 0.f;
+    }
+    for (int k0 = beg; k0 < end; k0 += LANES) {
+        const int k = k0 + lane;
+        int idx = 0;
+        int2 pr = make_int2(-1, 0);
+        float wv[HB];
+#pragma unroll
+        for (int h = 0; h < HB; ++h) wv[h] = 0.f;
+        if (k < end) {
+            idx = a.indices[k];
+            const int wp = a.wperm ? a.wperm[k] : k;
+#pragma unroll
+            for (int h = 0; h < HB; ++h) wv[h] = a.w[(int64_t)wp * HB + h];
+            pr = lp.pairs[idx];
+        }
+#pragma unroll
+        for (int h = 0; h < HB; ++h) settle(wv[h]);
+        settle(pr.x), settle(pr.y);
+        const int cnt = min(LANES, end - k0);
+        for (int i = 0; i < cnt; i += U) {
+            float v[U][NCHUNK][VEC], ww[U][HB];
+#pragma unroll
+            for (int u = 0; u < U; ++u) {
+                const int j = min(i + u, cnt - 1);
+                const int s = group_bcast<LANES>(idx, j);
+#pragma unroll
+                for (int h = 0; h < HB; ++h) ww[u][h] = i + u < cnt ? group_bcast<LANES>(wv[h], j) : 0.f;
+                const float* px = a.x + (int64_t)s * a.ldx;
+#pragma unroll
+                for (int c = 0; c < NCHUNK; ++c) {
+#pragma unroll
+                    for (int t = 0; t < VEC; ++t) v[u][c][t] = 0.f;
+                    if (!lab[c]) vload<VEC>(v[u][c], px + off[c]);
+                }
+            }
+#pragma unroll
+            for (int u = 0; u < U; ++u) {
+                const int j = min(i + u, cnt - 1);
+                const int cls = group_bcast<LANES>(pr.x, j);
+                const float val = __int_as_float(group_bcast<LANES>(pr.y, j));
+#pragma unroll
+                for (int c = 0; c < NCHUNK; ++c) label_values<VEC>(v[u][c], rel[c], cls, val);
+            }
+#pragma unroll
+            for (int u = 0; u < U; ++u)
+#pragma unroll
+                for (int h = 0; h < HB; ++h)
+#pragma unroll
+                    for (int c = 0; c < NCHUNK; ++c)
+#pragma unroll
+                        for (int t = 0; t < VEC; ++t) acc[h][c][t] = fmaf(ww[u][h], v[u][c][t], acc[h][c][t]);
+        }
+    }
+    if (a.hout && slot < 0) {
+        const float s = a.hscale[0];
+#pragma unroll
+        for (int h = 0; h < HB; ++h) {
+            __half* ob = a.hout + (int64_t)row * a.ldh + (int64_t)h * a.hsh;
+#pragma unroll
+            for (int c = 0; c < NCHUNK; ++c) {
+                const int e = (c * LANES + lane) * VEC;
+                if (e < a.hpiece) store_halves<VEC>(ob + e, a.h2_off, acc[h][c], act[c] ? s : 0.f);
+            }
+        }
+        return;
+    }
+#pragma unroll
+    for (int h = 0; h < HB; ++h) {
+        float* ob = slot < 0 ? a.out + (int64_t)row * a.ldo + (int64_t)h * a.hso : a.partial + (int64_t)slot * a.ldp + (int64_t)h * a.D;
+#pragma unroll
+        for (int c = 0; c < NCHUNK; ++c)
+            if (act[c]) vstore<VEC>(ob + off[c], acc[h][c]);
+    }
+}
+
 __global__ __launch_bounds__(kBlock) void spmm_combine_halves_kernel(const int32_t* long_rows, const int32_t* long_ptr, int64_t n_long, int32_t H,
                                                                     int32_t D, const float* partial, int64_t ldp, __half* hout, int64_t ldh,
                                                                     int64_t hsh, int32_t h2_off, int32_t hpiece, const float* hscale) {
@@ -786,15 +901,22 @@
 }
 
 template <int VEC, int HB, bool DOT>
-static void dispatch_bcast(SpmmArgs& a, hipStream_t st) {
+static void dispatch_bcast(SpmmArgs& a, const LabelPairs& lp, hipStream_t st) {
     const int L = (std::max(a.D, a.hout ? a.hpiece : 0) + VEC - 1) / VEC;
 #define BOT_BCAST(LN, NC)                                                                                                     \
     do {                                                                                                                      \
         const int64_t blocks = (a.n_items * LN + kBlock - 1) / kBlock;                                                        \
         if (blocks == 0) break;                                                                                               \
-        set_kernel(DOT ? "bot::spmm_dot_bcast_kernel<%d,%d,%d,%d>" : "bot::spmm_bcast_kernel<%d,%d,%d,%d>", VEC, LN, NC, HB);        \
-        if constexpr (DOT) hipLaunchKernelGGL((spmm_dot_bcast_kernel<VEC, LN, NC, HB>), dim3((unsigned)blocks), dim3(kBlock), 0, st, a); \
-        else hipLaunchKernelGGL((spmm_bcast_kernel<VEC, LN, NC, HB>), dim3((unsigned)blocks), dim3(kBlock), 0, st, a);        \
+        if constexpr (DOT) {                                                                                                  \
+            set_kernel("bot::spmm_dot_bcast_kernel<%d,%d,%d,%d>", VEC, LN, NC, HB);                                           \
+            hipLaunchKernelGGL((spmm_dot_bcast_kernel<VEC, LN, NC, HB>), dim3((unsigned)blocks), dim3(kBlock), 0, st, a);     \
+        } else if (lp.pairs) {                                                                                                \
+            set_kernel("bot::spmm_bcast_pairs_kernel<%d,%d,%d,%d>", VEC, LN, NC, HB);                                         \
+            hipLaunchKernelGGL((spmm_bcast_pairs_kernel<VEC, LN, NC, HB>), dim3((unsigned)blocks), dim3(kBlock), 0, st, a, lp); \
+        } else {                                                                                                              \
+            set_kernel("bot::spmm_bcast_kernel<%d,%d,%d,%d>", VEC, LN, NC, HB);                                               \
+            hipLaunchKernelGGL((spmm_bcast_kernel<VEC, LN, NC, HB>), dim3((unsigned)blocks), dim3(kBlock), 0, st, a);         \
+        }                                                                                                                     \
     } while (0)
     if (L <= 16) BOT_BCAST(16, 1);
     else if (L <= 32) BOT_BCAST(32, 1);
@@ -805,13 +927,13 @@
 }
 
 template <bool DOT>
-static int run_bcast(SpmmArgs& a, int vec, int H, hipStream_t st) {
+static int run_bcast(SpmmArgs& a, int vec, int H, hipStream_t st, const LabelPairs& lp = LabelPairs{nullptr, 0}) {
 #define BOT_BCAST_H(V)                                \
     switch (H) {                                      \
-        case 1: dispatch_bcast<V, 1, DOT>(a, st); break; \
-        case 2: dispatch_bcast<V, 2, DOT>(a, st); break; \
-        case 3: dispatch_bcast<V, 3, DOT>(a, st); break; \
-        default: dispatch_bcast<V, 4, DOT>(a, st); break; \
+        case 1: dispatch_bcast<V, 1, DOT>(a, lp, st); break; \
+        case 2: dispatch_bcast<V, 2, DOT>(a, lp, st); break; \
+        case 3: dispatch_bcast<V, 3, DOT>(a, lp, st); break; \
+        default: dispatch_bcast<V, 4, DOT>(a, lp, st); break; \
     }
     if (vec == 4) { BOT_BCAST_H(4) } else if (vec == 2) { BOT_BCAST_H(2) } else { BOT_BCAST_H(1) }
 #undef BOT_BCAST_H
@@ -1091,12 +1213,11 @@
     return 0;
 }
 
-int bot_spmm_bcast_f32(const int32_t* indptr, const int32_t* indices, int64_t n_rows, int64_t nnz, const int32_t* items,
+static int spmm_bcast_f32_impl(const int32_t* indices, int64_t n_rows, int64_t nnz, const int32_t* items,
                        int64_t n_items, const int32_t* long_rows, const int32_t* long_ptr, int64_t n_long, const float* x,
-                       int64_t ldx, const float* w, const int32_t* wperm, int32_t H, int32_t D, float* out, int64_t ldo,
+                       int64_t ldx, const int32_t* pairs, int32_t F, const float* w, const int32_t* wperm, int32_t H, int32_t D, float* out, int64_t ldo,
                        int64_t hso, float* partial, bot_stream_t stream) {
     using namespace bot;
-    (void)indptr;
     BOT_REQUIRE(n_rows >= 0 && nnz >= 0 && n_items >= 0 && n_long >= 0 && nnz < INT32_MAX, BOT_E_RANGE, "spmm_bcast: bad size");
     BOT_REQUIRE(H >= 1 && H <= 4 && D >= 1 && D <= 1024, BOT_E_RANGE, "spmm_bcast: H=%d (1..4) D=%d (1..1024)", H, D);
     if (n_rows == 0) return 0;
@@ -1108,7 +1229,7 @@
                (int64_t)H * D, nullptr, 0, 0, nullptr, nullptr, 0, 0};
     const int vec = pick_vec(D, {ldx, ldo, hso}, {x, out, partial});
     BOT_REQUIRE(D <= vec * 256, BOT_E_RANGE, "spmm_bcast: D=%d exceeds one launch tile", D);
-    if (int rc = run_bcast<false>(a, vec, H, st)) return rc;
+    if (int rc = run_bcast<false>(a, vec, H, st, LabelPairs{reinterpret_cast<const int2*>(pairs), F})) return rc;
     if (n_long > 0) {
         const int64_t n = n_long * H * D;
         hipLaunchKernelGGL(spmm_combine_kernel, dim3((unsigned)((n + kBlock - 1) / kBlock)), dim3(kBlock), 0, st, long_rows,
@@ -1118,12 +1239,31 @@
     return 0;
 }
 
-int bot_spmm_bcast_halves_f16(const int32_t* indptr, const int32_t* indices, int64_t n_rows, int64_t nnz, const int32_t* items, int64_t n_items,
-                              const int32_t* long_rows, const int32_t* long_ptr, int64_t n_long, const float* x, int64_t ldx, const float* w,
+int bot_spmm_bcast_f32(const int32_t* indptr, const int32_t* indices, int64_t n_rows, int64_t nnz, const int32_t* items,
+                       int64_t n_items, const int32_t* long_rows, const int32_t* long_ptr, int64_t n_long, const float* x,
+                       int64_t ldx, const float* w, const int32_t* wperm, int32_t H, int32_t D, float* out, int64_t ldo,
+                       int64_t hso, float* partial, bot_stream_t stream) {
+    (void)indptr;
+    return spmm_bcast_f32_impl(indices, n_rows, nnz, items, n_items, long_rows, long_ptr, n_long, x, ldx, nullptr, 0, w, wperm, H, D, out, ldo, hso,
+                               partial, stream);
+}
+
+int bot_spmm_bcast_pairs_f32(const int32_t* indptr, const int32_t* indices, int64_t n_rows, int64_t nnz, const int32_t* items,
+                             int64_t n_items, const int32_t* long_rows, const int32_t* long_ptr, int64_t n_long, const float* x,
+                             int64_t ldx, const int32_t* pairs, int32_t F, const float* w, const int32_t* wperm, int32_t H, int32_t D, float* out,
+                             int64_t ldo, int64_t hso, float* partial, bot_stream_t stream) {
+    (void)indptr;
+    BOT_REQUIRE_PAIRS("spmm_bcast_pairs");
+    return spmm_bcast_f32_impl(indices, n_rows, nnz, items, n_items, long_rows, long_ptr, n_long, x, ldx, pairs, F, w, wperm, H, D, out, ldo, hso,
+                               partial, stream);
+}
+
+static int spmm_bcast_halves_f16_impl(const int32_t* indices, int64_t n_rows, int64_t nnz, const int32_t* items, int64_t n_items,
+                              const int32_t* long_rows, const int32_t* long_ptr, int64_t n_long, const float* x, int64_t ldx, const int32_t* pairs,
+                              int32_t F, const float* w,
                               const int32_t* wperm, int32_t H, int32_t D, const float* hscale, uint16_t* hout, int64_t ldh, int64_t hsh, int32_t h2_off,
                               int32_t hpiece, float* partial, bot_stream_t stream) {
     using namespace bot;
-    (void)indptr;
     BOT_REQUIRE(n_rows >= 0 && nnz >= 0 && n_items >= 0 && n_long >= 0 && nnz < INT32_MAX, BOT_E_RANGE, "spmm_bcast_halves: bad size");
     BOT_REQUIRE(H >= 1 && H <= 4 && D >= 1 && D <= 1024, BOT_E_RANGE, "spmm_bcast_halves: H=%d (1..4) D=%d (1..1024)", H, D);
     if (n_rows == 0) return 0;
@@ -1139,7 +1279,7 @@
     const int vec = pick_vec(D, {ldx}, {x, partial});
     BOT_REQUIRE(hpiece <= vec * 256, BOT_E_RANGE, "spmm_bcast_halves: hpiece=%d exceeds one launch tile", hpiece);
     a.D = D;
-    if (int rc = run_bcast<false>(a, vec, H, st)) return rc;
+    if (int rc = run_bcast<false>(a, vec, H, st, LabelPairs{reinterpret_cast<const int2*>(pairs), F})) return rc;
     if (n_long > 0) {
         const int64_t n = n_long * H * hpiece;
         hipLaunchKernelGGL(spmm_combine_halves_kernel, dim3((unsigned)((n + kBlock - 1) / kBlock)), dim3(kBlock), 0, st, long_rows, long_ptr, n_long, H, D,
@@ -1147,6 +1287,25 @@
         if (int rc = hip_status("spmm_bcast_halves combine launch")) return rc;
     }
     return 0;
+}
+
+int bot_spmm_bcast_halves_f16(const int32_t* indptr, const int32_t* indices, int64_t n_rows, int64_t nnz, const int32_t* items, int64_t n_items,
+                              const int32_t* long_rows, const int32_t* long_ptr, int64_t n_long, const float* x, int64_t ldx, const float* w,
+                              const int32_t* wperm, int32_t H, int32_t D, const float* hscale, uint16_t* hout, int64_t ldh, int64_t hsh, int32_t h2_off,
+                              int32_t hpiece, float* partial, bot_stream_t stream) {
+    (void)indptr;
+    return spmm_bcast_halves_f16_impl(indices, n_rows, nnz, items, n_items, long_rows, long_ptr, n_long, x, ldx, nullptr, 0, w, wperm, H, D, hscale, hout,
+                                      ldh, hsh, h2_off, hpiece, partial, stream);
+}
+
+int bot_spmm_bcast_halves_pairs_f16(const int32_t* indptr, const int32_t* indices, int64_t n_rows, int64_t nnz, const int32_t* items, int64_t n_items,
+                                    const int32_t* long_rows, const int32_t* long_ptr, int64_t n_long, const float* x, int64_t ldx,
+                                    const int32_t* pairs, int32_t F, const float* w, const int32_t* wperm, int32_t H, int32_t D, const float* hscale,
+                                    uint16_t* hout, int64_t ldh, int64_t hsh, int32_t h2_off, int32_t hpiece, float* partial, bot_stream_t stream) {
+    (void)indptr;
+    BOT_REQUIRE_PAIRS("spmm_bcast_halves_pairs");
+    return spmm_bcast_halves_f16_impl(indices, n_rows, nnz, items, n_items, long_rows, long_ptr, n_long, x, ldx, pairs, F, w, wperm, H, D, hscale, hout,
+                                      ldh, hsh, h2_off, hpiece, partial, stream);
 }
 
 int bot_spmm_dot_halves_fits(const float* x, int64_t ldx, int64_t hsx, const float* y, int64_t ldy, int64_t hsy, int32_t H, int32_t D, const uint16_t* hout,
diff --git a/bot_amd/csrc/step.hip b/bot_amd/csrc/step.hip
--- a/bot_amd/csrc/step.hip
+++ b/bot_amd/csrc/step.hip
@@ -48,8 +48,9 @@
     if (threadIdx.x == 0) count[0] = (float)t;
 }
 
-__global__ __launch_bounds__(256) void build_input_kernel(const float* feat, int64_t ldf, int64_t n, int F, int C, const int32_t* code, float p,
-                                                          uint64_t seed, const uint64_t* seed_offset, float* out, int64_t ldo) {
+template <bool PAIRS>
+__device__ __forceinline__ void build_input_rows(const float* feat, int64_t ldf, int64_t n, int F, int C, const int32_t* code, float p,
+                                                 uint64_t seed, const uint64_t* seed_offset, float* out, int64_t ldo, int2* pairs) {
     const int W = F + C, nquad = (W + 3) >> 2;
     const uint64_t s = eff_seed(seed, seed_offset);
     const float scale = p > 0.f ? 1.f / (1.f - p) : 1.f;
@@ -77,7 +78,25 @@
             for (int t = 0; t < 4; ++t)
                 if (c0 + t < W) o[t] = v[t];
         }
-    }
+        if constexpr (PAIRS) {
+            const bool has = lab >= 0 && lab < C;
+            if (!has) {
+                if (c0 == 0) pairs[r] = make_int2(-1, 0);
+            } else if (F + lab >= c0 && F + lab < c0 + 4) {
+                pairs[r] = make_int2(lab, __float_as_int(v[F + lab - c0]));
+            }
+        }
+    }
+}
+
+__global__ __launch_bounds__(256) void build_input_kernel(const float* feat, int64_t ldf, int64_t n, int F, int C, const int32_t* code, float p,
+                                                          uint64_t seed, const uint64_t* seed_offset, float* out, int64_t ldo) {
+    build_input_rows<false>(feat, ldf, n, F, C, code, p, seed, seed_offset, out, ldo, nullptr);
+}
+
+__global__ __launch_bounds__(256) void build_input_pairs_kernel(const float* feat, int64_t ldf, int64_t n, int F, int C, const int32_t* code, float p,
+                                                                uint64_t seed, const uint64_t* seed_offset, float* out, int64_t ldo, int2* pairs) {
+    build_input_rows<true>(feat, ldf, n, F, C, code, p, seed, seed_offset, out, ldo, pairs);
 }
 
 constexpr int kReuseMaxPerLane = 8;
@@ -286,6 +305,20 @@
     return hip_status("build_input");
 }
 
+extern "C" int bot_build_input_pairs_f32(const float* feat, int64_t ldf, int64_t n, int32_t F, int32_t C, const int32_t* code, float p, uint64_t seed,
+                                         const uint64_t* seed_offset, float* out, int64_t ldo, int32_t* pairs, bot_stream_t stream) {
+    using namespace bot;
+    BOT_REQUIRE(n >= 0 && F >= 0 && C >= 1 && ldo >= F + C && ldf >= F && p >= 0.f && p < 1.f, BOT_E_RANGE,
+                "build_input_pairs: n=%lld F=%d C=%d ldf=%lld ldo=%lld p=%f", (long long)n, (int)F, (int)C, (long long)ldf, (long long)ldo, (double)p);
+    BOT_REQUIRE(feat && out && code && pairs, BOT_E_NULL, "build_input_pairs: NULL pointer (feat, code, out, pairs)");
+    BOT_REQUIRE(aligned(pairs, 8), BOT_E_ALIGN, "build_input_pairs: pair table not 8-byte aligned");
+    if (n == 0) return 0;
+    const int64_t total = n * (int64_t)((F + C + 3) / 4);
+    hipLaunchKernelGGL(build_input_pairs_kernel, dim3((unsigned)std::min<int64_t>((total + 255) / 256, 65536)), dim3(256), 0, (hipStream_t)stream, feat, ldf, n,
+                       (int)F, (int)C, code, p, seed, seed_offset, out, ldo, reinterpret_cast<int2*>(pairs));
+    return hip_status("build_input_pairs");
+}
+
 extern "C" int bot_build_input_reuse_f32(const float* feat, int64_t ldf, int64_t n, int32_t F, int32_t C, const int32_t* code, const uint8_t* reuse,
                                          const float* pred, int64_t ldp, float p, uint64_t seed, const uint64_t* seed_offset, float* out, int64_t ldo,
                                          bot_stream_t stream) {
diff --git a/bot_amd/nn/fused.py b/bot_amd/nn/fused.py
--- a/bot_amd/nn/fused.py
+++ b/bot_amd/nn/fused.py
@@ -553,6 +553,7 @@
         else:
             xsrc = h
             el = out2[:, c:c + H].contiguous()
+        ctx.pairs_kw = pkw = _pairs_kw(h) if ext is None else {}
         er = out2[:Nd, c + H:c + 2 * H].contiguous() if has_er else None
         if sym:
             s_out, w_e = sym_scales(graph)
@@ -570,7 +571,7 @@
             xscale = _C.halves_scale(h) if ext is None else _C.halves_scale_from_slots(_C.absmax_into(xsrc, _C.absmax_slots(h.device)))
             A = torch.empty((Nd, 2 * KA), dtype=torch.float16, device=h.device)
             _C.halves_split_cols(h if Nd == N else h[:Nd], xscale, 2, A, KA, 0, FP)
-            _C.spmm_bcast_halves(csc, xsrc, a_d, None, xscale, A, FP, FP, KA, FP)
+            _C.spmm_bcast_halves(csc, xsrc, a_d, None, xscale, A, FP, FP, KA, FP, **pkw)
             Wres = (Wr.t()[:HD] if kp else Wr[:HD]).contiguous()
             slots = _C.absmax_slots(h.device)
             _C.absmax_into(Wres, slots)
@@ -587,7 +588,7 @@
             _C.gemm_halves3_nt_grouped(A, B, xscale, wscale, KA, 2 * FP, out2, g_fwd, FP // 32, stats=partials)
             return _finish_forward(ctx, x, bn, bn_w, bn_b, bn_training, drop_p, y_needed, partials, h=h, W=W, Wr=Wr, z=A,
                                    table=ext if ext is not None else h, el=el, er=er, a=a, a_d=a_d, xscale=xscale)
-        z = _C.spmm_bcast(csc, xsrc, a_d, None, head_outer=True)
+        z = _C.spmm_bcast(csc, xsrc, a_d, None, head_outer=True, **pkw)
         Wh = W.view(H, D, Fin)
         if has_res and skinny:
             _C.skinny_gemm(z, Wh, b_is_kn=False, out=out2, accumulate=True, batch=H, strides=(Nd * Fin, D * Fin, D), m=Nd, n=D, k=Fin)
@@ -674,7 +675,7 @@
         need_dh = ctx.needs_input_grad[0]
         if not need_dh:
             xsrc = table[:, :Fin] if halo else h
-            da = _C.sddmm_dot_bcast(g.csc, xsrc, dz)
+            da = _C.sddmm_dot_bcast(g.csc, xsrc, dz, **({} if halo else ctx.pairs_kw))
             dh_g = None
         elif halo:
             dext = torch.empty_like(table)
@@ -740,6 +741,39 @@
         return False
 
 
+L0_LABEL_PAIRS = os.environ.get("BOT_L0_LABEL_PAIRS", "1") != "0"
+_LABEL_PAIRS = [None]
+L0_PITCH_ALIGN = int(os.environ.get("BOT_L0_PITCH_ALIGN", "32"))
+
+
+def l0_row_pitch(width: int) -> int:
+    a = L0_PITCH_ALIGN
+    return width if a <= 0 else (width + a - 1) // a * a
+
+
+class label_pairs:
+
+    def __init__(self, operand, pairs, first_label_col):
+        self.entry = None if pairs is None else (operand, pairs, int(first_label_col), operand._version)
+
+    def __enter__(self):
+        self.prev, _LABEL_PAIRS[0] = _LABEL_PAIRS[0], self.entry
+        return self
+
+    def __exit__(self, *exc):
+        _LABEL_PAIRS[0] = self.prev
+        return False
+
+
+def _pairs_kw(h) -> dict:
+    e = _LABEL_PAIRS[0]
+    if not L0_LABEL_PAIRS or e is None:
+        return {}
+    t, pairs, F, version = e
+    same = h.data_ptr() == t.data_ptr() and h.shape == t.shape and h.stride() == t.stride() and h.dtype == t.dtype and h._version == version
+    return dict(pairs=pairs, label_col=F) if same else {}
+
+
 def take_input_dropped() -> bool:
     v = _INPUT_DROPPED[0]
     _INPUT_DROPPED[0] = False
@@ -913,7 +947,7 @@
     xscale = _C.halves_scale(h)
     A = torch.empty((N, 2 * KA), dtype=torch.float16, device=h.device)
     _C.halves_split_cols(h if N == h.shape[0] else h[:N], xscale, 2, A, KA, 0, FP)
-    _C.spmm_bcast_halves(csc, h, a, None, xscale, A, FP, FP, KA, FP)
+    _C.spmm_bcast_halves(csc, h, a, None, xscale, A, FP, FP, KA, FP, **_pairs_kw(h))
     scale, shift = eval_affine(epi)
     y = torch.empty((N, HD), dtype=h.dtype, device=h.device)
     slots = _C.absmax_slots(h.device) if (relu and ABSMAX_BYPRODUCT and gemm.enabled(h)) else None
diff --git a/bot_amd/train.py b/bot_amd/train.py
--- a/bot_amd/train.py
+++ b/bot_amd/train.py
@@ -119,7 +119,11 @@
     if use_labels:
         p = float(drop.p) if (drop is not None and model.training) else 0.0
         static = feat
-        feat = _C.build_input(static, code, n_classes, p, new_dropout_seed(p))
+        pairs = None
+        if fused.L0_LABEL_PAIRS and n_label_iters == 0 and static.is_cuda and isinstance(model, bnn.GAT):
+            feat, pairs = _C.build_input_pairs(static, code, n_classes, p, new_dropout_seed(p), pitch=fused.l0_row_pitch(static.shape[1] + n_classes))
+        else:
+            feat = _C.build_input(static, code, n_classes, p, new_dropout_seed(p))
         if n_label_iters > 0:
             reuse = _reuse_members(n, train_idx, val_idx, test_idx)
             with torch.no_grad():
@@ -130,7 +134,7 @@
                         DEBUG_PREDS.append(prev)
                     feat = _C.build_input_reuse(static, code, reuse, prev, n_classes, p, new_dropout_seed(p), out=feat)
                     del prev
-        with fused.input_already_dropped(drop is not None):
+        with fused.input_already_dropped(drop is not None), fused.label_pairs(feat, pairs, static.shape[1]):
             pred = _forward(model, graph, feat, edge_weight)
     else:
         pred = _forward(model, graph, feat, edge_weight)
@@ -234,11 +238,18 @@
              n_classes=None):
     import contextlib
     from .nn import fused
+    from . import _C
+    from . import nn as bnn
     model.eval()
     n_static = feat.shape[1]
-    if use_labels:
+    pairs = None
+    if use_labels and fused.L0_LABEL_PAIRS and feat.is_cuda and feat.dtype == torch.float32 and feat.stride(1) == 1 and isinstance(model, bnn.GAT):
+        code = torch.full((feat.shape[0],), -1, dtype=torch.int32, device=feat.device)
+        code[train_idx] = labels[train_idx, 0].to(torch.int32)
+        feat, pairs = _C.build_input_pairs(feat, code, n_classes, 0.0, 0, pitch=fused.l0_row_pitch(n_static + n_classes))
+    elif use_labels:
         feat = add_labels(feat, labels, train_idx, n_classes)
-    with (fused.label_reuse(n_static) if (use_labels and n_label_iters > 0) else contextlib.nullcontext()):
+    with (fused.label_reuse(n_static) if (use_labels and n_label_iters > 0) else contextlib.nullcontext()), fused.label_pairs(feat, pairs, n_static):
         pred = model(graph, feat)
         if n_label_iters > 0:
             unlabel_idx = torch.cat([val_idx, test_idx])
diff --git a/include/bot_gnn.h b/include/bot_gnn.h
--- a/include/bot_gnn.h
+++ b/include/bot_gnn.h
@@ -84,6 +84,18 @@
                               const float* x, int64_t ldx, const float* w, const int32_t* wperm,
                               int32_t H, int32_t D, const float* hscale, uint16_t* hout, int64_t ldh, int64_t hsh, int32_t h2_off,
                               int32_t hpiece, float* partial, bot_stream_t stream);
+int bot_spmm_bcast_pairs_f32(const int32_t* indptr, const int32_t* indices, int64_t n_rows, int64_t nnz,
+                             const int32_t* items, int64_t n_items,
+                             const int32_t* long_rows, const int32_t* long_ptr, int64_t n_long,
+                             const float* x, int64_t ldx, const int32_t* pairs, int32_t F, const float* w, const int32_t* wperm,
+                             int32_t H, int32_t D, float* out, int64_t ldo, int64_t hso,
+                             float* partial, bot_stream_t stream);
+int bot_spmm_bcast_halves_pairs_f16(const int32_t* indptr, const int32_t* indices, int64_t n_rows, int64_t nnz,
+                                    const int32_t* items, int64_t n_items,
+                                    const int32_t* long_rows, const int32_t* long_ptr, int64_t n_long,
+                                    const float* x, int64_t ldx, const int32_t* pairs, int32_t F, const float* w, const int32_t* wperm,
+                                    int32_t H, int32_t D, const float* hscale, uint16_t* hout, int64_t ldh, int64_t hsh, int32_t h2_off,
+                                    int32_t hpiece, float* partial, bot_stream_t stream);
 int bot_spmm_dot_bcast_f32(const int32_t* indptr, const int32_t* indices, int64_t n_rows, int64_t nnz,
                            const int32_t* items, int64_t n_items,
                            const int32_t* long_rows, const int32_t* long_ptr, int64_t n_long,
@@ -104,6 +116,12 @@
                             const float* y, int64_t ldy, int64_t hsy,
                             int32_t H, int32_t D,
                             float* out, const int32_t* operm, bot_stream_t stream);
+int bot_sddmm_dot_bcast_pairs_f32(const int32_t* indptr, const int32_t* indices, int64_t n_rows, int64_t nnz,
+                                  const int32_t* items, int64_t n_items,
+                                  const float* x, int64_t ldx, const int32_t* pairs, int32_t F,
+                                  const float* y, int64_t ldy, int64_t hsy,
+                                  int32_t H, int32_t D,
+                                  float* out, const int32_t* operm, bot_stream_t stream);
 
 int bot_sddmm_u_add_v_f32(const int32_t* src, const int32_t* dst, int64_t n_edges,
                           const float* x, const float* y, int32_t W, float* out, bot_stream_t stream);
@@ -412,6 +430,8 @@
                         bot_stream_t stream);
 int bot_build_input_f32(const float* feat, int64_t ldf, int64_t n, int32_t F, int32_t C, const int32_t* code, float p, uint64_t seed,
                         const uint64_t* seed_offset, float* out, int64_t ldo, bot_stream_t stream);
+int bot_build_input_pairs_f32(const float* feat, int64_t ldf, int64_t n, int32_t F, int32_t C, const int32_t* code, float p, uint64_t seed,
+                              const uint64_t* seed_offset, float* out, int64_t ldo, int32_t* pairs, bot_stream_t stream);
 int bot_build_input_reuse_f32(const float* feat, int64_t ldf, int64_t n, int32_t F, int32_t C, const int32_t* code, const uint8_t* reuse,
                               const float* pred, int64_t ldp, float p, uint64_t seed, const uint64_t* seed_offset, float* out, int64_t ldo,
                               bot_stream_t stream);
```

New measurement: 249.5 million, median of 4. About the same (+0.2%).
